# tinycrops/x-transformers-rl

Hardware: AMD Instinct MI355X
Metric: env-steps/s (rollout+update) (higher is better)
Workload: dtype f32; 1 GPU; C3: LunarLander-shaped VecSim (S=8, A=4, hazard 1/64), 1024 episodes x 128 steps per update per GPU, depth-4 d=256 4x16-head gated value-residual world-model policy, batch 128 episodes, 4 epochs, dropout 0.25; no EPO (BASELINE.json configs[2] names no gene pool: one policy, actor / critic heads on [embed | state embed], in = 2d); global_batch=1024, seq_len=128, parallelism=dp1, env_steps=1302236

## Files before the change

include/xtrl_hip.h:

```cpp
#ifndef XTRL_HIP_H
#define XTRL_HIP_H

#include <stdint.h>

#ifdef __cplusplus
extern "C" {
#endif

#define XTRL_OK 0
#define XTRL_E_ARG 1
#define XTRL_E_HIP 2

#define XTRL_ABI_VERSION 27

int xtrl_abi_version(void);
int64_t xtrl_struct_size(const char* name);
const char* xtrl_last_error(void);
const char* xtrl_source_hash(void);

#define XTRL_ACT_NONE 0
#define XTRL_ACT_GELU 1
#define XTRL_ACT_SILU 2
#define XTRL_ACT_RELU 3

int xtrl_gemm_f32(const float* X, int ldx, const float* W, int ldw, const float* bias, const float* ln_gamma,
                  const float* R, int ldr, float* Y, int ldy, const int32_t* t_dev, int64_t y_t_stride, int M,
                  int N, int K, int act, void* stream);

int xtrl_gemm_ex(int trans_a, int trans_b, const float* A, int lda, const float* B, int ldb, const float* bias,
                 float* C, int ldc, int M, int N, int K, float beta, void* stream);

int xtrl_gemm_wgrad(const float* dY, int ldy, const float* X, int ldx, float* dW, int ldw, int M, int N, int K,
                    float beta, float* ws, int64_t ws_floats, void* stream);
int xtrl_gemm_wgrad_db(const float* dY, int ldy, const float* X, int ldx, float* dW, int ldw, int M, int N, int K,
                       float beta, float* ws, int64_t ws_floats, float* db, int db_n0, void* stream);

int xtrl_layernorm_f32(const float* X, int ldx, const float* gamma, float* Y, int ldy, int M, int D, void* stream);

typedef struct XtrlDecodeLayer {
  const float* ln_attn;
  const float* w_qkv;
  const float* b_qkv;
  const float* w_out;
  const float* ln_ff;
  const float* w_ff1;
  const float* b_ff1;
  const float* w_ff2;
  const float* b_ff2;
  float* k_cache;
  float* v_cache;
  const float* w_out_t;
  const uint16_t* w_ff1x;
  const uint16_t* w_ff2x;
  const float* w_qkv_t;
  const float* w_ff1_t;
  const float* w_ff2_t;
  const float* w_ff1f;
  const float* w_ff2f;
  const float* mem_k;
  const float* mem_v;
} XtrlDecodeLayer;

typedef struct XtrlRngState {
  uint64_t seed;
  uint32_t update;
  uint32_t slot_offset;
} XtrlRngState;

typedef struct XtrlDecodeDesc {
  int E, S, A, B, d, L, H, dh, Tmax, G, ff, in_dim, n_qkv;
  int continuous, squash, evolutionary, gate_values, value_residual, learned_mix;
  int rotary_abs;
  int rot_dim;
  int sim_mode;
  int hazard_log2;
  int no_reward_cond;
  int state_only;
  float rs_eps;
  float clamp_lo, clamp_hi; int has_clamp;
  const float* w_pin; const float* b_pin;
  const float* act_emb; const float* act_emb_b;
  const float* reward_embed;
  const float* w_se; const float* b_se;
  const float* ln_final;
  const float* w_h1; const float* b_h1;
  const float* w_h2; const float* b_h2;
  const float* inv_freq;
  const XtrlDecodeLayer* layers;
  const float* rs_mean; const float* rs_var;
  float* state;
  int32_t* prev_action;
  float* prev_action_f;
  float* prev_reward;
  uint8_t* alive;
  int32_t* lens;
  double* cum_reward;
  const int32_t* episode_of_slot;
  const int32_t* slot_of_row;
  const XtrlRngState* rng;
  float* traj_states;
  int32_t* traj_actions;
  float* traj_actions_f;
  float* traj_logp;
  float* traj_rewards;
  uint8_t* traj_bounds;
  float* traj_values;
  float* x;
  float* qkv;
  float* att;
  float* hff;
  float* ac_in;
  float* logits;
  float* v1;
  float* xn;
  int32_t* live_rows;
  int32_t* live_count;
  float* mlp_part;
  uint32_t* mlp_cnt;
  const float* lat_embed;
  void** prof_events;
  const float* w_h1_t;
  const float* w_h2_t;
  const XtrlDecodeLayer* layers_dev;
  const uint16_t* w_h1x;
  float* heads_part;
  uint32_t* heads_cnt;
  float* row_part;
  uint32_t* row_cnt;
  int ff_glu;
  float* hglu;
  int qk_norm;
  float attn_scale;
  float xpos_base;
  int rms_norm;
  void* act_host;
  int attn_window;
  int Hkv;
  const float* alibi_slopes;
  int num_mem_kv;
  int add_zero_kv;
} XtrlDecodeDesc;

int xtrl_rollout_begin(const XtrlDecodeDesc* desc, void* stream);
int xtrl_decode_step(const XtrlDecodeDesc* desc, int t, void* stream);
int xtrl_decode_step_rows(const XtrlDecodeDesc* desc, int t, int max_rows, void* stream);
int xtrl_row_stamps(int on, uint64_t* out, int cap, int64_t* ticks_per_sec);
int xtrl_rollout_env_feedback(const XtrlDecodeDesc* desc, int t, const float* next_state, const float* reward,
                              const uint8_t* terminated, const uint8_t* truncated, int t_limit, int bootstrap,
                              void* stream);
int xtrl_host_decode(const XtrlDecodeDesc* desc, int t, int rows_max, void* act_host, void* stream);
int xtrl_host_feedback(const XtrlDecodeDesc* desc, int t, const void* host_stage, void* dev_stage, int t_limit,
                       int bootstrap, void* stream);
int xtrl_host_row_step(const XtrlDecodeDesc* desc, int t, const void* host_stage, int t_limit, int bootstrap,
                       uint32_t* gate, void* stream);
int xtrl_host_wait(const uint32_t* done, uint32_t value, double timeout_s);

int xtrl_dgemm(const float* A, int lda, const float* Wp, const float* bias, const float* ln_gamma, int ln_k,
               const float* R, int ldr, float* C, int ldc, const int32_t* row_map, const int32_t* m_dev, int M, int N,
               int K, int act, void* stream);
int64_t xtrl_dgemm_packed_floats(int N, int K);
int xtrl_dgemm_pack(const float* W, int ldw, int N, int K, float* Wp, void* stream);
int64_t xtrl_dgemm_packed_x6_elems(int N, int K);
int xtrl_dgemm_pack_x6(const float* W, int ldw, int N, int K, uint16_t* Wp, void* stream);
int64_t xtrl_dgemm_packed_f8_floats(int N, int K);
int xtrl_dgemm_pack_f8(const float* W, int ldw, int N, int K, float* Wp, void* stream);

typedef struct XtrlFractalLevel {
  const float* w_qkv;
  const float* w_out;
  const float* ln1_w; const float* ln1_b;
  const float* w_c;
  const float* ln2_w; const float* ln2_b;
  const float* w_ff1; const float* b_ff1;
  const float* w_ff2; const float* b_ff2;
  const float* ln3_w; const float* ln3_b;
  const float* w_pg; const float* b_pg;
  const float* level_emb;
  float* sums;
} XtrlFractalLevel;

typedef struct XtrlFractalDesc {
  int levels;
  float ln_eps;
  const XtrlFractalLevel* level;
  const float* g_init;
  const float* c0;
  const float* w_fa0; const float* b_fa0;
  const float* w_fa2; const float* b_fa2;
  float* g;
  float* c2;
  float* tmp;
  float* x2;
  float* mean;
  float* allf;
  float* hagg;
} XtrlFractalDesc;

int xtrl_fractal_decode_step(const XtrlDecodeDesc* desc, const XtrlFractalDesc* fd, int t, void* stream);

int xtrl_hlgauss_gae(const float* logits, int64_t ld_row, const float* rewards, const uint8_t* bounds,
                     int64_t ld_seq, const float* centers, float* values, float* returns, int E, int n, int B,
                     float gamma, float gamma_lam, const float* boot, const int32_t* lens, void* stream);

int xtrl_attn_fwd(const float* q, const float* k, const float* v, const int32_t* lens, float* o, float* lse,
                  int b, int H, int n, int dh, float scale, float dropout_p, uint64_t seed, uint32_t offset,
                  uint32_t sub, void* stream);
int xtrl_attn_bwd(const float* q, const float* k, const float* v, const int32_t* lens, const float* o,
                  const float* lse, const float* dout, float* dq, float* dk, float* dv, float* delta_ws, int b,
                  int H, int n, int dh, float scale, float dropout_p, uint64_t seed, uint32_t offset, uint32_t sub,
                  void* stream);
int64_t xtrl_attn_bwd_part_floats(int b, int H, int n, int dh);
int xtrl_attn_bwd_part(const float* q, const float* k, const float* v, const int32_t* lens, const float* o,
                       const float* lse, const float* dout, float* dq, float* dk, float* dv, float* delta_ws,
                       float* dq_part, int64_t dq_part_floats, int b, int H, int n, int dh, float scale,
                       float dropout_p, uint64_t seed, uint32_t offset, uint32_t sub, void* stream);
int xtrl_attn_fwd_win(const float* q, const float* k, const float* v, const int32_t* lens, float* o, float* lse,
                      int b, int H, int n, int dh, float scale, float dropout_p, uint64_t seed, uint32_t offset,
                      uint32_t sub, int window, void* stream);
int xtrl_attn_bwd_win(const float* q, const float* k, const float* v, const int32_t* lens, const float* o,
                      const float* lse, const float* dout, float* dq, float* dk, float* dv, float* delta_ws, int b,
                      int H, int n, int dh, float scale, float dropout_p, uint64_t seed, uint32_t offset,
                      uint32_t sub, int window, void* stream);
int xtrl_attn_bwd_part_win(const float* q, const float* k, const float* v, const int32_t* lens, const float* o,
                           const float* lse, const float* dout, float* dq, float* dk, float* dv, float* delta_ws,
                           float* dq_part, int64_t dq_part_floats, int b, int H, int n, int dh, float scale,
                           float dropout_p, uint64_t seed, uint32_t offset, uint32_t sub, int window, void* stream);
int xtrl_attn_fwd_gqa(const float* q, const float* k, const float* v, const int32_t* lens, float* o, float* lse,
                      int b, int H, int Hkv, int n, int dh, float scale, float dropout_p, uint64_t seed,
                      uint32_t offset, uint32_t sub, int window, void* stream);
int xtrl_attn_bwd_gqa(const float* q, const float* k, const float* v, const int32_t* lens, const float* o,
                      const float* lse, const float* dout, float* dq, float* dk, float* dv, float* delta_ws, int b,
                      int H, int Hkv, int n, int dh, float scale, float dropout_p, uint64_t seed, uint32_t offset,
                      uint32_t sub, int window, void* stream);
int xtrl_attn_bwd_part_gqa(const float* q, const float* k, const float* v, const int32_t* lens, const float* o,
                           const float* lse, const float* dout, float* dq, float* dk, float* dv, float* delta_ws,
                           float* dq_part, int64_t dq_part_floats, int b, int H, int Hkv, int n, int dh, float scale,
                           float dropout_p, uint64_t seed, uint32_t offset, uint32_t sub, int window, void* stream);
int64_t xtrl_attn_sink_ws_floats(int b, int H, int num_mem_kv, int dh);
int xtrl_attn_fwd_sink(const float* q, const float* k, const float* v, const int32_t* lens, float* o, float* lse,
                       const float* mem_k, const float* mem_v, int b, int H, int Hkv, int n, int dh, float scale,
                       float dropout_p, uint64_t seed, uint32_t offset, uint32_t sub, int window, int num_mem_kv,
                       int add_zero_kv, void* stream);
int xtrl_attn_bwd_sink(const float* q, const float* k, const float* v, const int32_t* lens, const float* o,
                       const float* lse, const float* dout, float* dq, float* dk, float* dv, float* delta_ws,
                       const float* mem_k, const float* mem_v, float* dmem_k, float* dmem_v, float* sink_ws,
                       int64_t sink_ws_floats, int b, int H, int Hkv, int n, int dh, float scale, float dropout_p,
                       uint64_t seed, uint32_t offset, uint32_t sub, int window, int num_mem_kv, int add_zero_kv,
                       void* stream);
int xtrl_attn_bwd_part_sink(const float* q, const float* k, const float* v, const int32_t* lens, const float* o,
                            const float* lse, const float* dout, float* dq, float* dk, float* dv, float* delta_ws,
                            float* dq_part, int64_t dq_part_floats, const float* mem_k, const float* mem_v,
                            float* dmem_k, float* dmem_v, float* sink_ws, int64_t sink_ws_floats, int b, int H, int Hkv,
                            int n, int dh, float scale, float dropout_p, uint64_t seed, uint32_t offset, uint32_t sub,
                            int window, int num_mem_kv, int add_zero_kv, void* stream);
int xtrl_attn_fwd_alibi(const float* q, const float* k, const float* v, const int32_t* lens, float* o, float* lse,
                        const float* mem_k, const float* mem_v, int b, int H, int Hkv, int n, int dh, float scale,
                        float dropout_p, uint64_t seed, uint32_t offset, uint32_t sub, int window, int num_mem_kv,
                        int add_zero_kv, const float* alibi_slopes, void* stream);
int xtrl_attn_bwd_alibi(const float* q, const float* k, const float* v, const int32_t* lens, const float* o,
                        const float* lse, const float* dout, float* dq, float* dk, float* dv, float* delta_ws,
                        const float* mem_k, const float* mem_v, float* dmem_k, float* dmem_v, float* sink_ws,
                        int64_t sink_ws_floats, int b, int H, int Hkv, int n, int dh, float scale, float dropout_p,
                        uint64_t seed, uint32_t offset, uint32_t sub, int window, int num_mem_kv, int add_zero_kv,
                        const float* alibi_slopes, void* stream);
int xtrl_attn_bwd_part_alibi(const float* q, const float* k, const float* v, const int32_t* lens, const float* o,
                             const float* lse, const float* dout, float* dq, float* dk, float* dv, float* delta_ws,
                             float* dq_part, int64_t dq_part_floats, const float* mem_k, const float* mem_v,
                             float* dmem_k, float* dmem_v, float* sink_ws, int64_t sink_ws_floats, int b, int H, int Hkv,
                             int n, int dh, float scale, float dropout_p, uint64_t seed, uint32_t offset, uint32_t sub,
                             int window, int num_mem_kv, int add_zero_kv, const float* alibi_slopes, void* stream);

typedef struct XtrlTrainLayer {
  int64_t ln_attn, w_proj, b_proj, w_out, ln_ff, w_ff1, b_ff1, w_ff2, b_ff2;
  int n_qkv;
  int mix;
  float* x_attn;
  float* x_ff;
  float* xn_attn;
  float* xn_ff;
  float* st_attn;
  float* st_ff;
  float* proj;
  float* qkv;
  float* o;
  float* og;
  float* lse;
  float* u;
  float* hd;
  int64_t mem_k, mem_v;
} XtrlTrainLayer;

typedef struct XtrlWimgEntry XtrlWimgEntry;

typedef struct XtrlTrainDesc {
  int b, n, S, A, d, L, H, dh, ff, B, in_dim, n_out, G;
  int continuous, evolutionary, gate_values, rot_dim;
  float dropout, frac_head_grad, reward_keep, attn_scale;
  uint64_t seed;
  uint32_t attn_offset, ff_offset;
  float* flat;
  float* grad;
  int64_t w_pin, act_emb, act_emb_b, reward_embed, w_se, b_se, ln_final;
  int64_t w_pd, b_pd;
  int64_t w_pred2, b_pred2, w_lat, b_lat, w_h1, b_h1, w_a2, b_a2, w_c2, b_c2;
  const float* inv_freq;
  const float* swr;
  const int32_t* prev_action;
  const int32_t* next_action;
  const float* prev_action_f;
  const float* next_action_f;
  const float* latent;
  const int32_t* lens;
  float* raw;
  float* values;
  float* pred;
  float* done;
  float* x_final;
  float* st_final;
  float* ac_in;
  float* ewa;
  float* zp;
  float* hp;
  float* z1;
  float* h1;
  float* lat_e;
  const float* d_raw;
  const float* d_values;
  const float* d_pred;
  const float* d_done;
  float* dx;
  float* dx2;
  float* dxn;
  float* dff;
  float* dproj;
  float* dog;
  float* dvfirst;
  float* dz1;
  float* dac;
  float* dzp;
  float* dewa;
  float* delta;
  float* part;
  int64_t part_floats;
  float* ws;
  int64_t ws_floats;
  const XtrlTrainLayer* layers;
  void** prof_events;
  double* prof_flops;
  int prof_cap;
  int* prof_n;
  void** grad_events;
  int ld_ff;
  int ff_glu;
  int ld_u2;
  float* glu_dh;
  int qk_norm;
  float xpos_base;
  int rms_norm;
  int Tv;
  int32_t* vrows;
  int32_t* vinv;
  float* ewa_v;
  float* hp_v;
  float* zp_v;
  float* pred_v;
  float* d_pred_v;
  float* dzp_v;
  float* dewa_v;
  float* dq_part;
  int64_t dq_part_floats;
  int packed;
  int32_t* ep_off;
  float* pack_ws;
  int64_t pack_ws_floats;
  int attn_window;
  int Hkv;
  void* wimg;
  int64_t wimg_bytes;
  const XtrlWimgEntry* wimg_tab;
  const XtrlWimgEntry* wimg_tab_host;
  int wimg_n;
  const float* alibi_slopes;
  int num_mem_kv;
  int add_zero_kv;
  float* sink_ws;
  int64_t sink_ws_floats;
} XtrlTrainDesc;

struct XtrlWimgEntry {
  int64_t w_off;
  int64_t img_off;
  int N, K, ld, trans_b, BN, blk0;
};
#define XTRL_WIMG_TILE_BYTES(BN) (3 * (BN) * 40 * 2)
int xtrl_train_wimg_plan(const XtrlTrainDesc* desc, XtrlWimgEntry* tab, int cap, int64_t* bytes);
int xtrl_wimg_build(const float* flat, const XtrlWimgEntry* tab_host, const XtrlWimgEntry* tab_dev, int n,
                    void* arena, int64_t arena_bytes, void* stream);

int64_t xtrl_wimg_launch_count(void);

int xtrl_train_forward(const XtrlTrainDesc* desc, void* stream);
int xtrl_train_backward(const XtrlTrainDesc* desc, void* stream);

typedef struct XtrlFractalTrainLevel {
  int64_t w_qkv;
  int64_t w_out, w_gv, w_go;
  int64_t ln1_w, ln1_b, ln2_w, ln2_b, ln3_w, ln3_b;
  int64_t w_ff1, b_ff1, w_ff2, b_ff2, w_proj, b_proj, level_embed;
  float* xin;
  float* qkv;
  float* o;
  float* lse;
  float* s1; float* x1; float* st1;
  float* g;
  float* gv;
  float* s2; float* x2; float* st2;
  float* h; float* u;
  float* s3; float* x3; float* st3;
  float* mean;
} XtrlFractalTrainLevel;

typedef struct XtrlFractalTrainDesc {
  int levels;
  int64_t b_in;
  int64_t g_init, w_gu, b_gu, w_fa0, b_fa0, w_fa2, b_fa2;
  const float* scale_embeds;
  float* le;
  float* bias0;
  float* cat;
  float* hfa;
  float* dxa; float* dxb; float* dmean;
  float* ds;
  float* dga;
  float* dgb;
  float* dgv;
  float* dz;
  float* dqkv;
  float* dob;
  float* dcat;
  float* dhfa;
  const XtrlFractalTrainLevel* level;
} XtrlFractalTrainDesc;

int xtrl_fractal_train_forward(const XtrlTrainDesc* base, const XtrlFractalTrainDesc* f, void* stream);
int xtrl_fractal_train_backward(const XtrlTrainDesc* base, const XtrlFractalTrainDesc* f, void* stream);
int xtrl_linear_gelu_drop(const float* X, int ldx, const float* W, const float* bias, float* Y, int ldy, float* deriv,
                          int ld_deriv, int M, int N, int K, float p, uint64_t seed, uint32_t offset, uint32_t layer,
                          void* stream);
int xtrl_ff_dropout_mask(uint8_t* mask, int M, int N, float p, uint64_t seed, uint32_t offset, uint32_t layer,
                         void* stream);
int xtrl_glu_drop_fwd(const float* u, int ldu, float* h, int ldh, int M, int ff, float p, uint64_t seed,
                      uint32_t offset, uint32_t layer, void* stream);
int xtrl_glu_drop_bwd(const float* dh, int lddh, const float* u, int ldu, float* du, int lddu, int M, int ff, float p,
                      uint64_t seed, uint32_t offset, uint32_t layer, void* stream);
int64_t xtrl_train_part_floats(int T, int b, int d, int A);
int64_t xtrl_train_pack_floats(int T, int S, int A, int n_out, int B);

typedef struct XtrlBatchDesc {
  int N, Tmax, n, b, S, A, B, continuous;
  const float* states;
  const int32_t* actions;
  const float* actions_f;
  const float* rewards;
  const float* logp;
  const uint8_t* bounds;
  const float* values;
  const float* returns;
  const int32_t* lens;
  const int64_t* idx;
  const float* rs_mean;
  const float* rs_var;
  float* swr;
  int32_t* prev_action;
  int32_t* action;
  float* prev_action_f;
  float* action_f;
  float* old_logp;
  float* mb_returns;
  float* old_values;
  uint8_t* dones;
  int32_t* mb_lens;
  float* rs_part;
  float* rs_m;
} XtrlBatchDesc;

int xtrl_minibatch_gather(const XtrlBatchDesc* desc, void* stream);
int xtrl_rsnorm_update(float* mean, float* var, const float* m, int D, int t, void* stream);

typedef struct XtrlLossDesc {
  int b, n, A, B, S1;
  int continuous, squash, hl_reduction_mean;
  float eps_clip, value_clip, entropy_weight, w_actor, w_critic, w_autoreg, lo, hi, sigma;
  const float* raw_actions;
  const float* values;
  const float* pred_raw;
  const float* done_logit;
  const int32_t* actions;
  const float* actions_f;
  const float* old_logp;
  const float* returns;
  const float* old_values;
  const uint8_t* dones;
  const int32_t* lens;
  const float* real;
  const float* support;
  const float* centers;
  float* tok;
  float* stats;
  float* d_raw_actions; float* d_values; float* d_pred_raw; float* d_done_logit;
} XtrlLossDesc;

#define XTRL_LOSS_TOK 30
#define XTRL_LOSS_STATS 32
#define XTRL_LS_LOSS 0
#define XTRL_LS_ACTOR 1
#define XTRL_LS_CRITIC 2
#define XTRL_LS_AUTOREG 3
#define XTRL_LS_DONE 4
#define XTRL_LS_ADV_MEAN 5
#define XTRL_LS_ADV_DEN 6
#define XTRL_LS_L 7
#define XTRL_LS_LC 8
#define XTRL_LS_NMASK 9
#define XTRL_LS_NWM 10
#define XTRL_LS_KCRIT 11
#define XTRL_LS_DL 12
#define XTRL_LS_DLC 13

int xtrl_loss_fwd(const XtrlLossDesc* desc, void* stream);
int xtrl_loss_bwd(const XtrlLossDesc* desc, float grad_scale, void* stream);

int xtrl_grad_norm(const float* g, int64_t n, double* ws, float max_norm, float* out, void* stream);
int xtrl_adopt_atan2(float* p, float* g, float* m, float* v, float* p_init, int64_t n, const int64_t* chunks,
                     int n_chunks, const int64_t* seg_start, int n_seg, int* seg_ws, const float* clip, float lr,
                     float init_lr, float beta1, float beta2, float a, float b, float weight_decay, float regen_rate,
                     float cautious, int first_step, void* stream);
int xtrl_ema_lerp(float* ema, const float* p, int64_t n, float weight, void* stream);

float xtrl_rng_uniform(uint64_t seed, uint32_t update, uint32_t slot, uint32_t t, uint32_t field, uint32_t sub);
float xtrl_rng_normal(uint64_t seed, uint32_t update, uint32_t slot, uint32_t t, uint32_t field, uint32_t sub);

int xtrl_sim_reset(float* state, int E, int S, uint64_t seed, uint32_t update, const int32_t* episode_of_slot,
                   void* stream);

int xtrl_attn_fwd_tokens(const float* q, int ldq, const float* k, int ldk, const float* v, int ldv,
                         const int32_t* lens, float* o, int ldo, float* lse, int b, int H, int n, int dh, float scale,
                         int causal, void* stream);
int xtrl_rows_add(const float* x, int ldx, const float* v, float* y, int ldy, int M, int D, void* stream);
int xtrl_add_layernorm(const float* x, int ldx, const float* r, int ldr, int r_rep, const float* gamma,
                       const float* beta, float* y, int ldy, int M, int D, float eps, void* stream);
int xtrl_seq_mean(const float* x, int ldx, int B, int n, int D, float* y, int ldy, void* stream);
int xtrl_safe_embed(const int32_t* actions, int M, const float* W, int D, float* y, int ldy, void* stream);
// ... 8 lines not shown
```

x-transformers-rl_amd/csrc/cabi.cpp:

```cpp
#include <hip/hip_runtime.h>
#include <stdarg.h>
#include <stdio.h>
#include <string.h>

#include "../../include/xtrl_hip.h"
#include "philox.h"

namespace xtrl {

static thread_local char g_err[512] = "";

void set_error(const char* fmt, ...) {
  va_list ap;
  va_start(ap, fmt);
  vsnprintf(g_err, sizeof(g_err), fmt, ap);
  va_end(ap);
}

int check_launch(const char* what) {
  const hipError_t e = hipGetLastError();
  if (e != hipSuccess) {
    set_error("%s: %s", what, hipGetErrorString(e));
    return XTRL_E_HIP;
  }
  return XTRL_OK;
}

}

extern "C" int xtrl_abi_version(void) { return XTRL_ABI_VERSION; }

#ifndef XTRL_SRC_HASH
#define XTRL_SRC_HASH "unknown"
#endif
extern "C" const char* xtrl_source_hash(void) { return XTRL_SRC_HASH; }

extern "C" int64_t xtrl_struct_size(const char* name) {
  static const struct {
    const char* name;
    int64_t size;
  } sizes[] = {{"XtrlDecodeLayer", sizeof(XtrlDecodeLayer)}, {"XtrlRngState", sizeof(XtrlRngState)},
               {"XtrlDecodeDesc", sizeof(XtrlDecodeDesc)},   {"XtrlTrainLayer", sizeof(XtrlTrainLayer)},
               {"XtrlTrainDesc", sizeof(XtrlTrainDesc)},     {"XtrlBatchDesc", sizeof(XtrlBatchDesc)},
               {"XtrlLossDesc", sizeof(XtrlLossDesc)},       {"XtrlFractalLevel", sizeof(XtrlFractalLevel)},
               {"XtrlFractalDesc", sizeof(XtrlFractalDesc)},     {"XtrlFractalTrainLevel", sizeof(XtrlFractalTrainLevel)},
               {"XtrlFractalTrainDesc", sizeof(XtrlFractalTrainDesc)}, {"XtrlWimgEntry", sizeof(XtrlWimgEntry)}};
  for (const auto& s : sizes)
    if (name && strcmp(name, s.name) == 0) return s.size;
  return -1;
}
extern "C" const char* xtrl_last_error(void) { return xtrl::g_err; }

extern "C" float xtrl_rng_uniform(uint64_t seed, uint32_t update, uint32_t slot, uint32_t t, uint32_t field,
                                  uint32_t sub) {
  return xtrl::rng_uniform(seed, update, slot, t, field, sub);
}
extern "C" float xtrl_rng_normal(uint64_t seed, uint32_t update, uint32_t slot, uint32_t t, uint32_t field,
                                 uint32_t sub) {
  return xtrl::rng_normal(seed, update, slot, t, field, sub);
}
```

x-transformers-rl_amd/csrc/gemm.hip:

```cpp
#include <cstdlib>
#include <type_traits>

#include "kernels.h"
#include "philox.h"
#include "x6.h"

namespace xtrl {

namespace {

__device__ __forceinline__ bool al16(const void* p) { return ((uintptr_t)p & 15u) == 0; }
__device__ __forceinline__ float f4c(const float4& v, int k) {
  return k == 0 ? v.x : (k == 1 ? v.y : (k == 2 ? v.z : v.w));
}

template <int EPI, bool RES>
__device__ __forceinline__ bool epi_v4_ok(const GemmArgs& a, const float* C) {
  constexpr bool AUX1 = (EPI == EPI_MUL_AUX || EPI == EPI_DGATE || EPI == EPI_MASK_POS), AUX2 = (EPI == EPI_DGATE);
  constexpr bool AOUT = (EPI == EPI_GELU_DROP || EPI == EPI_SILU_SAVE || EPI == EPI_DGATE);
  bool ok = (a.N & 3) == 0 && (a.ldc & 3) == 0 && al16(C);
  if constexpr (RES) ok = ok && (a.ldr & 3) == 0 && al16(a.R);
  if constexpr (AUX1) ok = ok && (a.ld_aux_in & 3) == 0 && al16(a.aux_in);
  if constexpr (AUX2) ok = ok && (a.ld_aux_in2 & 3) == 0 && al16(a.aux_in2);
  if constexpr (AOUT) ok = ok && (a.ld_aux_out & 3) == 0 && al16(a.aux_out);
// ... 649 lines not shown
  float4 gam = ld4(a.ln_g);
  if (!cok) gam = z4;
  const float inv_n = 1.0f / (float)N;
  if constexpr (EPI == EPI_RES_LN) {
    float4 bia = z4, beta = z4, add2 = z4;
    if (a.bias) bia = ld4(a.bias);
    if (a.ln_b) beta = ld4(a.ln_b);
    if (a.ln_b2) add2 = ld4(a.ln_b2);
    if (!cok) bia = beta = add2 = z4;
    float4 v[RPW], r[RPW];
#pragma unroll
    for (int rr = 0; rr < RPW; ++rr) {
      const int row = wave + 8 * rr, mc = min(m0 + row, M - 1);
      v[rr] = *reinterpret_cast<const float4*>(tile + row * LDT + cc);
      r[rr] = ld4(a.R + (int64_t)mc * a.ldr);
    }
#pragma unroll
    for (int rr = 0; rr < RPW; ++rr) {
      const int m = m0 + wave + 8 * rr;
      float4 x;
      x.x = (v[rr].x + bia.x) + r[rr].x; x.y = (v[rr].y + bia.y) + r[rr].y;
      x.z = (v[rr].z + bia.z) + r[rr].z; x.w = (v[rr].w + bia.w) + r[rr].w;
      if (!cok) x = z4;
      const float mean = a.ln_rms ? 0.f : wave_sum((x.x + x.y) + (x.z + x.w)) * inv_n;
      float4 dl = make_float4(x.x - mean, x.y - mean, x.z - mean, x.w - mean);
      if (!cok) dl = z4;
      const float sq = wave_sum((dl.x * dl.x + dl.y * dl.y) + (dl.z * dl.z + dl.w * dl.w));
      const float rstd = a.ln_rms ? norm_rstd(sq, (float)N, true) : 1.0f / sqrtf(sq * inv_n + 1e-5f);
      float4 y = make_float4((dl.x * rstd) * gam.x, (dl.y * rstd) * gam.y, (dl.z * rstd) * gam.z,
                             (dl.w * rstd) * gam.w);
      if (a.ln_b) y = make_float4(y.x + beta.x, y.y + beta.y, y.z + beta.z, y.w + beta.w);
      if (m < M) {
        if (cok) {
          *reinterpret_cast<float4*>(a.C + (int64_t)m * a.ldc + c) = x;
          *reinterpret_cast<float4*>(a.ln_y1 + (int64_t)m * a.ln_ld1 + c) = y;
          if (a.ln_y2)
            *reinterpret_cast<float4*>(a.ln_y2 + (int64_t)m * a.ln_ld2 + c) =
                make_float4(y.x + add2.x, y.y + add2.y, y.z + add2.z, y.w + add2.w);
        }
        if (lane == 0) *reinterpret_cast<float2*>(a.ln_stats + 2 * (int64_t)m) = make_float2(mean, rstd);
      }
    }
  } else {
    constexpr bool X = EPI == EPI_LN_BWD2;
    const int ps = X && a.ln_pstride ? a.ln_pstride : N;
    float4 g[RPW], xv[RPW], dr[RPW];
    float2 st[RPW];
#pragma unroll
    for (int rr = 0; rr < RPW; ++rr) {
      const int row = wave + 8 * rr, mc = min(m0 + row, M - 1);
      g[rr] = *reinterpret_cast<const float4*>(tile + row * LDT + cc);
      xv[rr] = ld4(a.ln_x + (int64_t)mc * N);
      if constexpr (X) dr[rr] = a.ln_gpre ? ld4(a.ln_gpre + (int64_t)mc * (a.ln_ldg ? a.ln_ldg : N)) : z4;
      else dr[rr] = a.ln_dres ? ld4(a.ln_dres + (int64_t)mc * N) : z4;
      st[rr] = *reinterpret_cast<const float2*>(a.ln_stats + 2 * (int64_t)mc);
      if constexpr (X) {
        const float gs = a.ln_gscale;
        g[rr] = make_float4(g[rr].x * gs + dr[rr].x, g[rr].y * gs + dr[rr].y, g[rr].z * gs + dr[rr].z,
                            g[rr].w * gs + dr[rr].w);
      }
      if (!cok) g[rr] = z4;
    }
    float4 dg = z4, db = z4;
#pragma unroll
    for (int rr = 0; rr < RPW; ++rr) {
      const int m = m0 + wave + 8 * rr;
      const float mu = st[rr].x, rs = st[rr].y;
      float4 xh = make_float4((xv[rr].x - mu) * rs, (xv[rr].y - mu) * rs, (xv[rr].z - mu) * rs, (xv[rr].w - mu) * rs);
      if (!cok) xh = z4;
      const float4 gm = make_float4(g[rr].x * gam.x, g[rr].y * gam.y, g[rr].z * gam.z, g[rr].w * gam.w);
      if (m < M) {
        dg.x += g[rr].x * xh.x; dg.y += g[rr].y * xh.y; dg.z += g[rr].z * xh.z; dg.w += g[rr].w * xh.w;
        if constexpr (X) { db.x += g[rr].x; db.y += g[rr].y; db.z += g[rr].z; db.w += g[rr].w; }
      }
      const float ma = a.ln_rms ? 0.f : wave_sum((gm.x + gm.y) + (gm.z + gm.w)) * inv_n;
      const float mb = wave_sum((gm.x * xh.x + gm.y * xh.y) + (gm.z * xh.z + gm.w * xh.w)) * inv_n;
      float4 o;
      o.x = rs * (gm.x - ma - xh.x * mb);
      o.y = rs * (gm.y - ma - xh.y * mb);
      o.z = rs * (gm.z - ma - xh.z * mb);
      o.w = rs * (gm.w - ma - xh.w * mb);
      if constexpr (!X) {
        o.x += dr[rr].x; o.y += dr[rr].y; o.z += dr[rr].z; o.w += dr[rr].w;
      }
      if (!cok) o = z4;
      if (m < M && cok) *reinterpret_cast<float4*>(a.C + (int64_t)m * a.ldc + c) = o;
      if constexpr (X) g[rr] = o;
    }
    float* red = tile + BM * LDT;
    const int t = threadIdx.x;
    auto tile_sum = [&](float4 v, float* dst) {
      __syncthreads();
      if (cok) *reinterpret_cast<float4*>(red + wave * BN + c) = v;
      __syncthreads();
      if (t < N) {
        float sum = 0.f;
#pragma unroll
        for (int w = 0; w < 8; ++w) sum += red[w * BN + t];
        dst[(int64_t)row_tile * ps + t] = sum;
      }
    };
    tile_sum(dg, a.ln_part);
    if constexpr (X) {
      if (a.ln_part_b) tile_sum(db, a.ln_part_b);
      if (a.ln2_out) {
        float4 gam2 = ld4(a.ln2_g);
        if (!cok) gam2 = z4;
#pragma unroll
        for (int rr = 0; rr < RPW; ++rr) {
          const int row = wave + 8 * rr, mc = min(m0 + row, M - 1);
          xv[rr] = ld4(a.ln2_x + (int64_t)mc * N);
          st[rr] = *reinterpret_cast<const float2*>(a.ln2_stats + 2 * (int64_t)mc);
        }
        dg = db = z4;
#pragma unroll
        for (int rr = 0; rr < RPW; ++rr) {
          const int m = m0 + wave + 8 * rr;
          const float mu = st[rr].x, rs = st[rr].y;
          float4 xh = make_float4((xv[rr].x - mu) * rs, (xv[rr].y - mu) * rs, (xv[rr].z - mu) * rs, (xv[rr].w - mu) * rs);
          if (!cok) xh = z4;
          const float4 gm = make_float4(g[rr].x * gam2.x, g[rr].y * gam2.y, g[rr].z * gam2.z, g[rr].w * gam2.w);
          if (m < M) {
            dg.x += g[rr].x * xh.x; dg.y += g[rr].y * xh.y; dg.z += g[rr].z * xh.z; dg.w += g[rr].w * xh.w;
            db.x += g[rr].x; db.y += g[rr].y; db.z += g[rr].z; db.w += g[rr].w;
          }
          const float ma = wave_sum((gm.x + gm.y) + (gm.z + gm.w)) * inv_n;
          const float mb = wave_sum((gm.x * xh.x + gm.y * xh.y) + (gm.z * xh.z + gm.w * xh.w)) * inv_n;
          const float4 o = make_float4(rs * (gm.x - ma - xh.x * mb), rs * (gm.y - ma - xh.y * mb),
                                       rs * (gm.z - ma - xh.z * mb), rs * (gm.w - ma - xh.w * mb));
          if (m < M && cok) *reinterpret_cast<float4*>(a.ln2_out + (int64_t)m * N + c) = o;
        }
        tile_sum(dg, a.ln2_part);
        tile_sum(db, a.ln2_part_b);
      }
    }
  }
}

#ifdef XTRL_WS_DIAG
__device__ uint64_t* g_ws_diag;
__device__ int g_ws_mode;
#define WS_STAMP(step, k)                                                                         \
  do {                                                                                            \
    if ((tid & 255) == 0)                                                                         \
      g_ws_diag[((int64_t)(blockIdx.x + gridDim.x * (blockIdx.y + gridDim.y * blockIdx.z)) * 2 +   \
                 (tid >> 8)) * 4096 + (step) * 4 + (k)] = __builtin_amdgcn_s_memtime();           \
  } while (0)
#else
#define WS_STAMP(step, k) do {} while (0)
#endif

typedef __attribute__((address_space(3))) void lds_void_t;

template <bool TA, bool TB, int EPI, bool RES, int BM = 128, int BN = 128, bool KT = false, bool WI = false>
__global__ __launch_bounds__(512, 1) void k_gemm_ws(const GemmArgs a) {
  constexpr int BK = 32, XRS = BK + 8, NP = 256, TM = 2, TN = 2, WN = BN / 64;
  constexpr bool LNE = (EPI == EPI_RES_LN || EPI == EPI_LN_BWD || EPI == EPI_LN_BWD2);
  static_assert(!WI || !TA, "weight images feed B of the A \"N\" launches");
  static_assert(XTRL_WIMG_TILE_BYTES(BN) == 3 * BN * XRS * 2, "image tile = the B part of a piece image");
  constexpr int A_F4 = BM * BK / 4 / NP, B_F4 = BN * BK / 4 / NP;
  constexpr int IMG = 3 * (BM + BN) * XRS;
  static_assert((BM == 128 && BN == 128) || (BM == 64 && BN == 256), "tile 128 x 128 or 64 x 256");
  static_assert(!TA || A_F4 == 4, "A \"T\": one 4 x 4 transposed group per producer thread");
  static_assert(!TB || B_F4 % 4 == 0, "B \"T\": whole 4 x 4 transposed groups per producer thread");
  constexpr int LDT = BN + 4;
  static_assert(!LNE || (BM * LDT + 8 * BN) * 4 <= 2 * IMG * 2, "LN tile exceeds the piece images");
  __shared__ __attribute__((aligned(16))) __bf16 smem[2 * IMG];

  const int tid = threadIdx.x, lane = tid & 63, wave = tid >> 6;
  const bool producer = wave >= 4;
  int bx = blockIdx.x, by = blockIdx.y, bz = blockIdx.z;
  if (a.xcd_remap) {
    const int nx = gridDim.x, ny = gridDim.y;
    const int total = nx * ny * gridDim.z;
    const int lin = bx + nx * (by + ny * bz);
    const int lg = (lin & 7) * (total >> 3) + (lin >> 3);
    bx = lg % nx;
    by = (lg / nx) % ny;
    bz = lg / (nx * ny);
  }
  const int m0 = by * BM, n0 = bx * BN;
  const int M = a.M, N = a.N;
  int K = a.K;
  const float* __restrict__ Ab = a.A;
  const float* __restrict__ Bb = a.B;
  if (a.kspan > 0) {
    const int kb = bz * a.kspan;
    K = min(a.kspan, a.K - kb);
    Ab += TA ? (int64_t)kb * a.lda : kb;
    Bb += TB ? (int64_t)kb * a.ldb : kb;
  }
  const int nk = (K + BK - 1) / BK;
  using I0 = std::integral_constant<int, 0>;
  using I1 = std::integral_constant<int, 1>;

  const int p = tid - 256;
  float4 ra[2][A_F4], rb[2][B_F4];
  const bool do_rs = a.rowsum != nullptr && bx == 0;
  float rs[4] = {0.f, 0.f, 0.f, 0.f};
  auto ld_n = [&](const float* base, int64_t ld, int row, int row_lim, int k) -> float4 {
    return *reinterpret_cast<const float4*>(base + (int64_t)min(row, row_lim - 1) * ld + (KT ? min(k, K - 4) : k));
  };
  auto ld_t = [&](const float* base, int64_t ld, int k, int col, int col_lim) -> float4 {
    return *reinterpret_cast<const float4*>(base + (int64_t)(KT ? min(k, K - 1) : k) * ld +
                                            min(col, ((col_lim + 3) & ~3) - 4));
  };
  auto kmask = [&](float4 f, int k) -> float4 {
    if constexpr (KT) {
      const bool ok = k < K;
      f = make_float4(ok ? f.x : 0.f, ok ? f.y : 0.f, ok ? f.z : 0.f, ok ? f.w : 0.f);
    }
    return f;
  };
  auto load = [&](auto S, int kt) {
    const int k0 = min(kt, nk - 1) * BK;
#pragma unroll
    for (int i = 0; i < A_F4; ++i) {
      if constexpr (!TA) {
        const int e = p + i * NP, r = e / (BK / 4), q = e % (BK / 4);
        ra[S][i] = ld_n(Ab, a.lda, m0 + r, M, k0 + 4 * q);
      } else {
        const int kq = p % (BK / 4), q = p / (BK / 4);
        ra[S][i] = ld_t(Ab, a.lda, k0 + 4 * kq + i, m0 + 4 * q, M);
      }
    }
    if constexpr (!WI) {
#pragma unroll
      for (int i = 0; i < B_F4; ++i) {
        if constexpr (!TB) {
          const int e = p + i * NP, r = e / (BK / 4), q = e % (BK / 4);
          rb[S][i] = ld_n(Bb, a.ldb, n0 + r, N, k0 + 4 * q);
        } else {
          const int kq = p % (BK / 4), q = p / (BK / 4) + 32 * (i >> 2);
          rb[S][i] = ld_t(Bb, a.ldb, k0 + 4 * kq + (i & 3), n0 + 4 * q, N);
        }
      }
    }
  };
  constexpr int WB = XTRL_WIMG_TILE_BYTES(BN), WCH = WB / 1024, WPW = (WCH + 3) / 4;
  static_assert(WB % 1024 == 0 && (3 * BM * XRS * 2) % 16 == 0, "whole wave-instructions, 16-byte aligned B part");
  auto dma_b = [&](int kt, __bf16* img) {
    const char* src = static_cast<const char*>(a.wimg) + ((int64_t)bx * nk + min(kt, nk - 1)) * WB + lane * 16;
    char* dst = reinterpret_cast<char*>(img + 3 * BM * XRS);
#pragma unroll
    for (int i = 0; i < WPW; ++i) {
      const int c = 4 * i + (wave - 4);
      if (WCH % 4 == 0 || c < WCH)
        __builtin_amdgcn_global_load_lds((const void*)(src + c * 1024), (lds_void_t*)(dst + c * 1024), 16, 0, 0);
    }
  };
  auto put = [&](__bf16* img, int rows, int row, int k, float4 v) {
    bf16x4 h, m, l;
#if defined(XTRL_WS_MODE) && XTRL_WS_MODE == 4
    h = __builtin_bit_cast(bf16x4, make_uint2(__float_as_uint(v.x), __float_as_uint(v.y)));
    m = __builtin_bit_cast(bf16x4, make_uint2(__float_as_uint(v.z), __float_as_uint(v.w)));
    l = __builtin_bit_cast(bf16x4, make_uint2(__float_as_uint(v.x), __float_as_uint(v.w)));
#else
    split3(v, h, m, l);
#endif
    __bf16* q = img + row * XRS + k;
    *reinterpret_cast<bf16x4*>(q) = h;
    *reinterpret_cast<bf16x4*>(q + rows * XRS) = m;
    *reinterpret_cast<bf16x4*>(q + 2 * rows * XRS) = l;
  };
  auto convert = [&](auto S, __bf16* img, int kt, bool live) {
    __bf16* xa = img;
    __bf16* xb = img + 3 * BM * XRS;
    const int k0 = min(kt, nk - 1) * BK;
    const int kq = p % (BK / 4), q = p / (BK / 4);
    if constexpr (!TA) {
#pragma unroll
      for (int i = 0; i < A_F4; ++i) {
        const int e = p + i * NP, r = e / (BK / 4), qq = e % (BK / 4);
        put(xa, BM, r, 4 * qq, kmask(ra[S][i], k0 + 4 * qq));
      }
    } else {
      const float4 k0v = kmask(ra[S][0], k0 + 4 * kq), k1v = kmask(ra[S][1], k0 + 4 * kq + 1),
                   k2v = kmask(ra[S][2], k0 + 4 * kq + 2), k3v = kmask(ra[S][3], k0 + 4 * kq + 3);
      put(xa, BM, 4 * q + 0, 4 * kq, make_float4(k0v.x, k1v.x, k2v.x, k3v.x));
      put(xa, BM, 4 * q + 1, 4 * kq, make_float4(k0v.y, k1v.y, k2v.y, k3v.y));
      put(xa, BM, 4 * q + 2, 4 * kq, make_float4(k0v.z, k1v.z, k2v.z, k3v.z));
      put(xa, BM, 4 * q + 3, 4 * kq, make_float4(k0v.w, k1v.w, k2v.w, k3v.w));
      if (do_rs) {
        float s4[4] = {(k0v.x + k1v.x) + (k2v.x + k3v.x), (k0v.y + k1v.y) + (k2v.y + k3v.y),
                       (k0v.z + k1v.z) + (k2v.z + k3v.z), (k0v.w + k1v.w) + (k2v.w + k3v.w)};
#pragma unroll
        for (int c = 0; c < 4; ++c) {
#pragma unroll
          for (int o = 1; o < BK / 4; o <<= 1) s4[c] += __shfl_xor(s4[c], o, kWave);
          rs[c] += live ? s4[c] : 0.f;
        }
      }
    }
    if constexpr (WI) {
    } else if constexpr (!TB) {
#pragma unroll
      for (int i = 0; i < B_F4; ++i) {
        const int e = p + i * NP, r = e / (BK / 4), qq = e % (BK / 4);
        put(xb, BN, r, 4 * qq, kmask(rb[S][i], k0 + 4 * qq));
      }
    } else {
#pragma unroll
      for (int gi = 0; gi < B_F4 / 4; ++gi) {
        const int qg = q + 32 * gi;
        const float4 k0v = kmask(rb[S][4 * gi], k0 + 4 * kq), k1v = kmask(rb[S][4 * gi + 1], k0 + 4 * kq + 1),
                     k2v = kmask(rb[S][4 * gi + 2], k0 + 4 * kq + 2), k3v = kmask(rb[S][4 * gi + 3], k0 + 4 * kq + 3);
        put(xb, BN, 4 * qg + 0, 4 * kq, make_float4(k0v.x, k1v.x, k2v.x, k3v.x));
        put(xb, BN, 4 * qg + 1, 4 * kq, make_float4(k0v.y, k1v.y, k2v.y, k3v.y));
        put(xb, BN, 4 * qg + 2, 4 * kq, make_float4(k0v.z, k1v.z, k2v.z, k3v.z));
        put(xb, BN, 4 * qg + 3, 4 * kq, make_float4(k0v.w, k1v.w, k2v.w, k3v.w));
      }
    }
  };

  const int wm = (wave & 3) / WN, wn = (wave & 3) % WN;
  f32x16 acc[TM][TN];
#pragma unroll
  for (int i = 0; i < TM; ++i)
#pragma unroll
    for (int j = 0; j < TN; ++j)
#pragma unroll
      for (int r = 0; r < 16; ++r) acc[i][j][r] = 0.f;
  auto compute = [&](const __bf16* img) {
    const int xi = wm * 32 * TM + (lane & 31), xj = wn * 32 * TN + (lane & 31), xk = 8 * (lane >> 5);
    const __bf16* xa = img;
    const __bf16* xb = img + 3 * BM * XRS;
    bf16x8 av[2][3][TM], bv[2][3][TN];
    auto rd = [&](int buf, int st) {
      auto ra_ = [&](int pc) {
#pragma unroll
        for (int i = 0; i < TM; ++i)
          av[buf][pc][i] = *reinterpret_cast<const bf16x8*>(xa + (pc * BM + xi + 32 * i) * XRS + 16 * st + xk);
      };
      auto rb_ = [&](int pc) {
#pragma unroll
        for (int j = 0; j < TN; ++j)
          bv[buf][pc][j] = *reinterpret_cast<const bf16x8*>(xb + (pc * BN + xj + 32 * j) * XRS + 16 * st + xk);
      };
      ra_(2); rb_(0); ra_(0); rb_(2); ra_(1); rb_(1);
    };
    rd(0, 0);
#pragma unroll
    for (int st = 0; st < BK / 16; ++st) {
      const int pb = st & 1;
      if (st + 1 < BK / 16) rd(pb ^ 1, st + 1);
      __builtin_amdgcn_sched_barrier(0);
      constexpr int PA[6] = {2, 0, 1, 1, 0, 0}, PB[6] = {0, 2, 1, 0, 1, 0};
#pragma unroll
      for (int t = 0; t < 6; ++t)
#pragma unroll
        for (int i = 0; i < TM; ++i)
#pragma unroll
          for (int j = 0; j < TN; ++j)
            acc[i][j] = __builtin_amdgcn_mfma_f32_32x32x16_bf16(av[pb][PA[t]][i], bv[pb][PB[t]][j], acc[i][j], 0, 0, 0);
      __builtin_amdgcn_sched_barrier(0);
    }
  };

  const int nsteps = 2 * ((nk + 1) / 2);
  auto wi_barrier = [&]() {
    static_assert(A_F4 <= 15, "vmcnt immediate");
    __builtin_amdgcn_sched_barrier(0);
    __builtin_amdgcn_s_waitcnt(A_F4 | 0x70);
    if constexpr (A_F4 == 2) asm volatile("s_waitcnt vmcnt(2) lgkmcnt(0)" ::: "memory");
    else asm volatile("s_waitcnt vmcnt(4) lgkmcnt(0)" ::: "memory");
    static_assert(A_F4 == 2 || A_F4 == 4, "vmcnt immediates above");
    __builtin_amdgcn_s_barrier();
    asm volatile("" ::: "memory");
    __builtin_amdgcn_sched_barrier(0);
  };
  if (producer) {
    load(I0{}, 0);
    load(I1{}, 1);
    convert(I0{}, smem, 0, true);
    if constexpr (WI) {
      __builtin_amdgcn_sched_barrier(0);
      dma_b(0, smem);
      __builtin_amdgcn_sched_barrier(0);
    }
    load(I0{}, 2);
    if constexpr (WI) wi_barrier();
    else __syncthreads();
#ifdef XTRL_WS_DIAG
    const int mode = g_ws_mode;
#elif defined(XTRL_WS_MODE)
    constexpr int mode = XTRL_WS_MODE;
#else
    constexpr int mode = 0;
#endif
    auto pstep = [&](auto C, int t) {
      if constexpr (WI) {
        __bf16* img = smem + ((t + 1) & 1) * IMG;
        convert(C, img, t + 1, t + 1 < nk);
        __builtin_amdgcn_sched_barrier(0);
        dma_b(t + 1, img);
        __builtin_amdgcn_sched_barrier(0);
        load(C, t + 3);
        wi_barrier();
        return;
      }
      WS_STAMP(t, 0);
      if (mode < 2 || mode == 4) convert(C, smem + ((t + 1) & 1) * IMG, t + 1, t + 1 < nk);
      else if (mode == 3) {
        float s = 0.f;
#pragma unroll
        for (int i = 0; i < 4; ++i) s += ra[decltype(C)::value][i % A_F4].x + rb[decltype(C)::value][i].y;
        if (s == 12345.f) smem[tid] = (__bf16)s;
      }
      WS_STAMP(t, 1);
      __builtin_amdgcn_sched_barrier(0);
      if (mode != 2) load(C, t + 3);
      WS_STAMP(t, 2);
      __builtin_amdgcn_sched_barrier(0);
      __syncthreads();
      __builtin_amdgcn_sched_barrier(0);
    };
    for (int t = 0; t < nsteps; t += 2) {
      pstep(I1{}, t);
      pstep(I0{}, t + 1);
    }
    if (TA && do_rs && (p % (BK / 4)) == 0) {
      const int q = p / (BK / 4);
#pragma unroll
      for (int c = 0; c < 4; ++c) {
        const int m = m0 + 4 * q + c;
        if (m < M && m >= a.rowsum_m0) {
          if (a.kspan > 0) a.rowsum_ws[(int64_t)bz * M + m] = rs[c];
          else a.rowsum[m - a.rowsum_m0] += rs[c];
        }
      }
    }
    if constexpr (!LNE) return;
  } else {
    __syncthreads();
    for (int t = 0; t < nsteps; ++t) {
      WS_STAMP(t, 0);
#ifdef XTRL_WS_DIAG
      if (t < nk && g_ws_mode != 1) compute(smem + (t & 1) * IMG);
#elif defined(XTRL_WS_MODE)
      if (t < nk && XTRL_WS_MODE != 1) compute(smem + (t & 1) * IMG);
#else
      if (t < nk) compute(smem + (t & 1) * IMG);
#endif
      WS_STAMP(t, 1);
      __syncthreads();
    }
    WS_STAMP(nsteps, 0);
    if constexpr (!LNE) {
      gemm_epilogue<TM, TN, EPI, RES, EPI == EPI_GELU_DROP>(a, acc, m0, n0, wm, wn, lane, bz);
      return;
    }
  }
  if constexpr (LNE) ln_epilogue<BM, BN, EPI>(a, acc, reinterpret_cast<float*>(smem), producer, m0, wm, wn, lane, wave,
                                              by);
}

__global__ __launch_bounds__(256) void k_layernorm(const float* X, int ldx, const float* gamma, float* Y, int ldy,
                                                   int M, int D) {
  const int lane = threadIdx.x & 63;
  const int m = blockIdx.x * 4 + (threadIdx.x >> 6);
  if (m >= M) return;
  const float* xr = X + (int64_t)m * ldx;
  float s = 0.f;
  for (int k = lane; k < D; k += 64) s += xr[k];
  const float mean = wave_sum(s) / (float)D;
  float q = 0.f;
  for (int k = lane; k < D; k += 64) {
    const float dlt = xr[k] - mean;
    q += dlt * dlt;
  }
  const float rstd = 1.0f / sqrtf(wave_sum(q) / (float)D + 1e-5f);
  for (int k = lane; k < D; k += 64) Y[(int64_t)m * ldy + k] = ((xr[k] - mean) * rstd) * gamma[k];
}

__device__ __forceinline__ float sum_splits(const float* p, int S, int64_t stride) {
  float acc = 0.f;
  int z = 0;
  for (; z + 16 <= S; z += 16) {
    float v[16];
#pragma unroll
    for (int u = 0; u < 16; ++u) v[u] = p[(int64_t)(z + u) * stride];
#pragma unroll
    for (int u = 0; u < 16; ++u) acc += v[u];
  }
  for (; z < S; ++z) acc += p[(int64_t)z * stride];
  return acc;
}

__global__ __launch_bounds__(256) void k_splitk_reduce(const float* ws, int S, int M, int N, float* C, int ldc,
                                                       float beta, const float* rws, float* rowsum, int m0) {
  const int64_t MN = (int64_t)M * N;
  const int64_t gtid = (int64_t)blockIdx.x * 256 + threadIdx.x, gsz = (int64_t)gridDim.x * 256;
  if (rowsum) {
    for (int64_t m = m0 + gtid; m < M; m += gsz) rowsum[m - m0] += sum_splits(rws + m, S, M);
  }
  if ((N & 3) == 0) {
    constexpr int G = 4, U = 8;
    const int64_t Q = MN >> 2;
    const int g = threadIdx.x & (G - 1);
    const float4* w4 = reinterpret_cast<const float4*>(ws);
    for (int64_t q = gtid / G; q < Q; q += gsz / G) {
      float4 a = make_float4(0.f, 0.f, 0.f, 0.f);
      for (int z0 = g; z0 < S; z0 += G * U) {
        float4 p[U];
#pragma unroll
        for (int u = 0; u < U; ++u) {
          const int z = z0 + G * u;
          p[u] = z < S ? w4[(int64_t)z * Q + q] : make_float4(0.f, 0.f, 0.f, 0.f);
        }
#pragma unroll
        for (int u = 0; u < U; ++u) {
          a.x += p[u].x; a.y += p[u].y; a.z += p[u].z; a.w += p[u].w;
        }
      }
      float4 b;
      b.x = __shfl_xor(a.x, 1); b.y = __shfl_xor(a.y, 1); b.z = __shfl_xor(a.z, 1); b.w = __shfl_xor(a.w, 1);
      if (g & 1) { const float4 t = a; a = b; b = t; }
      a.x += b.x; a.y += b.y; a.z += b.z; a.w += b.w;
      b.x = __shfl_xor(a.x, 2); b.y = __shfl_xor(a.y, 2); b.z = __shfl_xor(a.z, 2); b.w = __shfl_xor(a.w, 2);
      if (g & 2) { const float4 t = a; a = b; b = t; }
      a.x += b.x; a.y += b.y; a.z += b.z; a.w += b.w;
      if (g == 0) {
        const int64_t i = q << 2;
        const int m = (int)(i / N), n = (int)(i - (int64_t)m * N);
        float* dst = C + (int64_t)m * ldc + n;
        if (beta != 0.f) {
          a.x += beta * dst[0]; a.y += beta * dst[1]; a.z += beta * dst[2]; a.w += beta * dst[3];
        }
        dst[0] = a.x; dst[1] = a.y; dst[2] = a.z; dst[3] = a.w;
      }
    }
    return;
  }
  for (int64_t i = gtid; i < MN; i += gsz) {
    const float acc = sum_splits(ws + i, S, MN);
    const int m = (int)(i / N), n = (int)(i - (int64_t)m * N);
    float* dst = C + (int64_t)m * ldc + n;
    *dst = (beta != 0.f) ? beta * (*dst) + acc : acc;
  }
}

struct SplitKJobs {
  SplitKJob job[kMaxSplitKJobs];
  int n;
  int64_t total_q, total_r;
};
__global__ __launch_bounds__(256) void k_splitk_reduce_multi(const SplitKJobs J) {
  const int64_t gsz = (int64_t)gridDim.x * 256;
  for (int64_t u = (int64_t)blockIdx.x * 256 + threadIdx.x; u < J.total_q + J.total_r; u += gsz) {
    if (u < J.total_q) {
      int j = 0;
      while (j + 1 < J.n && J.job[j + 1].q0 <= u) ++j;
      const SplitKJob& b = J.job[j];
      const int64_t q = u - b.q0, MN4 = (int64_t)b.M * b.N / 4;
      const float4* w4 = reinterpret_cast<const float4*>(b.ws);
      float4 a = make_float4(0.f, 0.f, 0.f, 0.f);
      int z = 0;
      for (; z + 8 <= b.S; z += 8) {
        float4 p[8];
#pragma unroll
        for (int k = 0; k < 8; ++k) p[k] = w4[(int64_t)(z + k) * MN4 + q];
#pragma unroll
        for (int k = 0; k < 8; ++k) {
          a.x += p[k].x; a.y += p[k].y; a.z += p[k].z; a.w += p[k].w;
        }
      }
      for (; z < b.S; ++z) {
        const float4 p = w4[(int64_t)z * MN4 + q];
        a.x += p.x; a.y += p.y; a.z += p.z; a.w += p.w;
      }
      const int64_t i = q << 2;
      const int m = (int)(i / b.N), n = (int)(i - (int64_t)m * b.N);
      float4* dst = reinterpret_cast<float4*>(b.C + (int64_t)m * b.ldc + n);
      if (b.beta != 0.f) {
        const float4 o = *dst;
        a.x += b.beta * o.x; a.y += b.beta * o.y; a.z += b.beta * o.z; a.w += b.beta * o.w;
      }
      *dst = a;
    } else {
      const int64_t r = u - J.total_q;
      int j = 0;
      while (j + 1 < J.n && J.job[j + 1].r0 <= r) ++j;
      const SplitKJob& b = J.job[j];
      const int m = b.m0 + (int)(r - b.r0);
      b.rowsum[m - b.m0] += sum_splits(b.rws + m, b.S, b.M);
    }
  }
}

template <int WM, int WN, int WK, int TM, int TN, bool TA, bool TB, int EPI, bool LN, bool RES, bool VEC,
          bool X6 = false>
void launch(const GemmArgs& a, hipStream_t s) {
  constexpr int BM = 32 * WM * TM, BN = 32 * WN * TN;
  const int splits = a.kspan > 0 ? (a.K + a.kspan - 1) / a.kspan : 1;
  dim3 grid((a.N + BN - 1) / BN, (a.M + BM - 1) / BM, splits);
  if constexpr (X6) {
    if ((int64_t)grid.x * grid.y * grid.z % 8 == 0) {
      GemmArgs r = a;
      r.xcd_remap = 1;
      hipLaunchKernelGGL((k_gemm<WM, WN, WK, TM, TN, TA, TB, EPI, LN, RES, VEC, X6>), grid, dim3(64 * WM * WN * WK), 0,
                         s, r);
      return;
    }
  }
  hipLaunchKernelGGL((k_gemm<WM, WN, WK, TM, TN, TA, TB, EPI, LN, RES, VEC, X6>), grid, dim3(64 * WM * WN * WK), 0, s,
                     a);
}

bool ws_ok(const GemmArgs& a, bool ta, bool ln) {
  if (!(!ln && (a.K % 32 == 0 || ta) && (a.kspan == 0 || a.kspan % 32 == 0) && (!a.rowsum || ta)))
    return false;
  const int splits = a.kspan > 0 ? (a.K + a.kspan - 1) / a.kspan : 1;
  const int64_t wgs = (int64_t)((a.N + 127) / 128) * ((a.M + 127) / 128) * splits;
  return wgs <= 256 && (a.kspan > 0 ? a.kspan : a.K) >= (ta ? 64 : 512);
}

int64_t g_wimg_launches = 0;

bool wimg_on() {
  static const bool on = [] {
    const char* e = getenv("XTRL_WIMG");
    return !(e && atoi(e) == 0);
  }();
  return on;
}

template <bool TA, bool TB, int EPI, bool RES, int BM = 128, int BN = 128, bool KT = false>
void launch_ws(const GemmArgs& a, hipStream_t s) {
  const int splits = a.kspan > 0 ? (a.K + a.kspan - 1) / a.kspan : 1;
  dim3 grid((a.N + BN - 1) / BN, (a.M + BM - 1) / BM, splits);
  GemmArgs r = a;
  r.xcd_remap = (int64_t)grid.x * grid.y * grid.z % 8 == 0 ? 1 : 0;
  if constexpr (!TA && (EPI == EPI_NONE || EPI == EPI_RES_LN || EPI == EPI_LN_BWD || EPI == EPI_LN_BWD2)) {
    if (a.wimg && a.wimg_bn == BN && a.kspan == 0 && wimg_on()) {
      ++g_wimg_launches;
      hipLaunchKernelGGL((k_gemm_ws<TA, TB, EPI, RES, BM, BN, KT, true>), grid, dim3(512), 0, s, r);
      return;
    }
  }
  hipLaunchKernelGGL((k_gemm_ws<TA, TB, EPI, RES, BM, BN, KT>), grid, dim3(512), 0, s, r);
}

int ln_gemm_run(const GemmArgs& a, int trans_a, int trans_b, int epi, bool vec, hipStream_t s) {
  const bool res = a.R != nullptr;
  XTRL_REQUIRE(!trans_a && vec && a.kspan == 0 && a.N <= 256 && a.N % 4 == 0 && a.K % 4 == 0 && a.ln_g &&
                   a.ln_stats && a.ldc % 4 == 0 && ((uintptr_t)a.C & 15u) == 0 && ((uintptr_t)a.ln_g & 15u) == 0,
               "gemm: LayerNorm epilogue needs one row tile (N=%d <= 256), float4 operands, K %% 4 == 0", a.N);
  const bool kt = a.K % 32 != 0, narrow = a.N <= 128;
  if (epi == EPI_RES_LN) {
    XTRL_REQUIRE(!trans_b && res && a.ln_y1 && a.ldr % 4 == 0 && a.ln_ld1 % 4 == 0 && (!a.ln_y2 || a.ln_ld2 % 4 == 0) &&
                     (!a.bias || ((uintptr_t)a.bias & 15u) == 0) && (!a.ln_b || ((uintptr_t)a.ln_b & 15u) == 0) &&
                     (!a.ln_b2 || (a.ln_y2 && ((uintptr_t)a.ln_b2 & 15u) == 0)),
                 "gemm: residual + LayerNorm epilogue arguments");
    if (narrow) {
      if (kt) launch_ws<false, false, EPI_RES_LN, true, 128, 128, true>(a, s);
      else launch_ws<false, false, EPI_RES_LN, true, 128, 128, false>(a, s);
    } else {
      if (kt) launch_ws<false, false, EPI_RES_LN, true, 64, 256, true>(a, s);
      else launch_ws<false, false, EPI_RES_LN, true, 64, 256, false>(a, s);
    }
  } else if (epi == EPI_LN_BWD) {
    XTRL_REQUIRE(trans_b && !res && a.ln_x && a.ln_part, "gemm: LayerNorm-backward epilogue arguments");
    if (narrow) launch_ws<false, true, EPI_LN_BWD, false, 128, 128, true>(a, s);
    else launch_ws<false, true, EPI_LN_BWD, false, 64, 256, true>(a, s);
  } else {
    XTRL_REQUIRE(trans_b && !res && a.ln_x && a.ln_part && (!a.ln_gpre || ((uintptr_t)a.ln_gpre & 15u) == 0) &&
                     a.ln_ldg % 4 == 0 &&
                     (!a.ln2_out || (a.ln2_g && a.ln2_x && a.ln2_stats && a.ln2_part && a.ln2_part_b &&
                                     ((uintptr_t)a.ln2_out & 15u) == 0 && ((uintptr_t)a.ln2_g & 15u) == 0)) &&
                     a.ldc == a.N,
                 "gemm: post-norm LayerNorm-backward epilogue arguments");
    if (narrow) launch_ws<false, true, EPI_LN_BWD2, false, 128, 128, true>(a, s);
    else launch_ws<false, true, EPI_LN_BWD2, false, 64, 256, true>(a, s);
  }
  XTRL_LAUNCHED("gemm_ln");
  return XTRL_OK;
}

bool use_x6() {
  static const bool x6 = [] {
    const char* e = getenv("XTRL_GEMM_F32");
    return !(e && atoi(e) != 0);
  }();
  return x6;
}

template <bool TA, bool TB, int EPI, bool LN, bool RES>
void dispatch_geom(const GemmArgs& a, bool vec, hipStream_t s) {
  const int64_t tiles128 = (int64_t)((a.M + 127) / 128) * ((a.N + 127) / 128);
  const int64_t tiles64 = (int64_t)((a.M + 63) / 64) * ((a.N + 63) / 64);
  if (!vec) launch<2, 2, 1, 1, 1, TA, TB, EPI, LN, RES, false>(a, s);
  else if (!TA && a.N <= 32 && a.M >= 4096) launch<2, 1, 2, 1, 1, TA, TB, EPI, LN, RES, true>(a, s);
  else if (tiles128 >= 192 && a.K > 64) {
    bool done = false;
    if constexpr (EPI != EPI_DGATE && !LN) {
      if (use_x6() && ws_ok(a, TA, LN) && a.K % 32 == 0) {
        launch_ws<TA, TB, EPI, RES>(a, s);
        done = true;
      }
    }
    if (done) {
    } else if (use_x6()) launch<2, 2, 1, 2, 2, TA, TB, EPI, LN, RES, true, true>(a, s);
    else launch<2, 2, 1, 2, 2, TA, TB, EPI, LN, RES, true>(a, s);
  }
  else if (tiles64 >= 256 && a.K <= 512) {
    bool done = false;
    if constexpr (!TA && !TB && EPI != EPI_DGATE) {
      if (use_x6()) {
        launch<2, 2, 1, 1, 1, TA, TB, EPI, LN, RES, true, true>(a, s);
        done = true;
      }
    }
    if (!done) launch<2, 2, 1, 1, 1, TA, TB, EPI, LN, RES, true>(a, s);
  }
  else if (a.K <= 256) launch<2, 1, 2, 1, 1, TA, TB, EPI, LN, RES, true>(a, s);
  else launch<1, 1, 4, 1, 1, TA, TB, EPI, LN, RES, true>(a, s);
}

bool aligned16(const void* p) { return ((uintptr_t)p & 15u) == 0; }

bool gelu_drop_v4_host(const GemmArgs& a) {
  return (a.N & 3) == 0 && (a.ldc & 3) == 0 && aligned16(a.C) && (a.ld_aux_out & 3) == 0 && aligned16(a.aux_out) &&
         !a.t_dev && a.kspan == 0;
}
int round4(int x) { return (x + 3) & ~3; }

}

int gemm_ln_rows(int N) { return N <= 128 ? 128 : 64; }

int gemm_run(const GemmArgs& a, int trans_a, int trans_b, int epi, hipStream_t s) {
  XTRL_REQUIRE(a.A && a.B && a.C, "gemm: null operand");
  XTRL_REQUIRE(a.M >= 0 && a.N >= 0 && a.K > 0, "gemm: bad shape M=%d N=%d K=%d", a.M, a.N, a.K);
  XTRL_REQUIRE(a.lda >= (trans_a ? a.M : a.K) && a.ldb >= (trans_b ? a.N : a.K) && a.ldc >= a.N,
               "gemm: leading dims too small");
  XTRL_REQUIRE(!(a.gamma && trans_a), "gemm: LayerNorm prologue needs a row-major A");
  XTRL_REQUIRE(!((epi == EPI_GELU_DROP || epi == EPI_SILU_SAVE || epi == EPI_DGATE) && !a.aux_out),
               "gemm: epilogue %d needs aux_out", epi);
  XTRL_REQUIRE(!((epi == EPI_MUL_AUX || epi == EPI_DGATE || epi == EPI_MASK_POS) && !a.aux_in),
               "gemm: epilogue %d needs aux_in", epi);
  XTRL_REQUIRE(!(epi == EPI_DGATE && !a.aux_in2), "gemm: gate epilogue needs aux_in2");
  if (a.M == 0 || a.N == 0) return XTRL_OK;
  const bool vec = aligned16(a.A) && aligned16(a.B) && (a.lda % 4 == 0) && (a.ldb % 4 == 0) &&
                   a.lda >= round4(trans_a ? a.M : a.K) && a.ldb >= round4(trans_b ? a.N : a.K);
  const bool ln = a.gamma != nullptr, res = a.R != nullptr;
  if (epi == EPI_RES_LN || epi == EPI_LN_BWD || epi == EPI_LN_BWD2) return ln_gemm_run(a, trans_a, trans_b, epi, vec, s);
  const bool vec_k = vec && (epi != EPI_GELU_DROP || gelu_drop_v4_host(a));
#define XG(TA_, TB_, E_, L_, R_)                                                                   \
  if (trans_a == TA_ && trans_b == TB_ && epi == E_ && ln == L_ && res == R_) {                    \
    dispatch_geom<TA_, TB_, E_, L_, R_>(a, vec_k, s);                                              \
    XTRL_LAUNCHED("gemm_f32");                                                                     \
    return XTRL_OK;                                                                                \
  }
  XG(0, 0, EPI_NONE, false, false)
  XG(0, 0, EPI_NONE, false, true)
  XG(0, 0, EPI_NONE, true, false)
  XG(0, 0, EPI_GELU, true, false)
  XG(0, 0, EPI_GELU, false, false)
  XG(0, 0, EPI_SILU, false, false)
  XG(0, 0, EPI_RELU, false, false)
  XG(0, 0, EPI_GELU_DROP, false, false)
  XG(0, 0, EPI_SILU_SAVE, false, false)
  XG(0, 1, EPI_NONE, false, false)
  XG(0, 1, EPI_NONE, false, true)
  XG(0, 1, EPI_MASK_POS, false, false)
  XG(0, 1, EPI_MUL_AUX, false, false)
  XG(0, 1, EPI_DGATE, false, false)
  XG(1, 1, EPI_NONE, false, false)
#undef XG
  set_error("gemm: unsupported combination ta=%d tb=%d epi=%d ln=%d residual=%d", trans_a, trans_b, epi, (int)ln,
            (int)res);
  return XTRL_E_ARG;
}

int gemm_ex(int trans_a, int trans_b, const float* A, int lda, const float* B, int ldb, const float* bias,
            const float* ln_gamma, const float* R, int ldr, float* C, int ldc, const int32_t* t_dev,
            int64_t c_t_stride, int M, int N, int K, int act, float beta, hipStream_t s) {
  XTRL_REQUIRE(act >= 0 && act <= 3, "gemm: bad activation %d", act);
  if (act == 3) act = EPI_RELU;
  GemmArgs a;
  a.A = A; a.B = B; a.bias = bias; a.gamma = ln_gamma; a.R = R; a.C = C; a.t_dev = t_dev;
  a.c_t_stride = c_t_stride; a.lda = lda; a.ldb = ldb; a.ldr = ldr; a.ldc = ldc; a.M = M; a.N = N; a.K = K;
  a.beta = beta;
  return gemm_run(a, trans_a, trans_b, act, s);
}

constexpr int SKW_R = 64;
template <bool TALL, int S, int LJ>
__global__ __launch_bounds__(256) void k_wgrad_skinny(const float* __restrict__ dY, int ldy, const float* __restrict__ X,
                                                      int ldx, int M, int N, int K, int bias, int span,
                                                      float* __restrict__ P, float* __restrict__ PR) {
  constexpr int R = SKW_R / LJ;
  extern __shared__ float skw_lds[];
  const int tid = threadIdx.x, Kx = K + bias;
  const int YS = (N + 3) & ~3, XS = (Kx + 3) & ~3;
  float* Ys = skw_lds;
  float* Xs = skw_lds + R * YS + (TALL ? 0 : 256 * LJ);
  const int t_lo = blockIdx.x * span, t_hi = min(M, t_lo + span);
  auto stage = [&](int t0) {
    const float* Lg = TALL ? dY : X;
    const int ldl = TALL ? ldy : ldx, Ln = TALL ? N : Kx, LSd = TALL ? YS : XS;
    float* Ld = TALL ? Ys : Xs;
#pragma unroll
    for (int j = 0; j < LJ; ++j) {
      const int c = tid + 256 * j;
      const bool in = c < Ln, ld = in && (TALL || c < K);
      float v[R];
#pragma unroll
      for (int r = 0; r < R; ++r) v[r] = (t0 + r < t_hi && ld) ? Lg[(int64_t)(t0 + r) * ldl + c] : 0.f;
      if (!TALL && c == K)
#pragma unroll
        for (int r = 0; r < R; ++r) v[r] = t0 + r < t_hi ? 1.f : 0.f;
      if (in)
#pragma unroll
        for (int r = 0; r < R; ++r) Ld[r * LSd + c] = v[r];
    }
    const float* Sg = TALL ? X : dY;
    const int lds_ = TALL ? ldx : ldy, Sn = TALL ? Kx : N, SSd = TALL ? XS : YS;
    float* Sd = TALL ? Xs : Ys;
    for (int e = tid; e < R * Sn; e += 256) {
      const int r = e / Sn, c = e - r * Sn, t = t0 + r;
      float v = 0.f;
      if (t < t_hi) v = (!TALL || c < K) ? Sg[(int64_t)t * lds_ + c] : 1.f;
      Sd[r * SSd + c] = v;
    }
  };
// ... 194 lines not shown
    }
  if (deferred && (defer->n == kMaxSplitKJobs || defer->used + need(splits) > ws_floats)) {
    if (int rc = splitk_flush(*defer, s)) return rc;
  }
  if (defer && !deferred && splits > 1 && defer->n > 0)
    if (int rc = splitk_flush(*defer, s)) return rc;
  if (deferred) {
    ws += defer->used;
    ws_floats -= defer->used;
  }
  while (splits > 1 && need(splits) > ws_floats) {
    splits = std::max(1, splits / 2);
    kspan = ((M + splits - 1) / splits + 31) / 32 * 32;
    splits = (M + kspan - 1) / kspan;
  }
  const bool vec = aligned16(dY) && aligned16(X) && (ldy % 4 == 0) && (ldx % 4 == 0) && ldy >= round4(N) &&
                   ldx >= round4(K);
  GemmArgs a;
  a.A = dY; a.B = X; a.C = dW; a.lda = ldy; a.ldb = ldx; a.ldc = ldw; a.M = N; a.N = K; a.K = M; a.beta = beta;
  a.rowsum = db;
  a.rowsum_m0 = db_n0;
  if (splits > 1) {
    XTRL_REQUIRE(ws && need(splits) <= ws_floats, "gemm_wgrad: workspace too small");
    a.C = ws;
    a.ldc = K;
    a.beta = 0.f;
    a.kspan = kspan;
    a.c_split = (int64_t)N * K;
    a.rowsum_ws = ws + (int64_t)splits * N * K;
  }
  if (!vec) launch<2, 2, 1, 1, 1, true, true, EPI_NONE, false, false, false>(a, s);
  else if (big) {
    const bool timed = prof && prof->events && *prof->n < prof->cap;
    if (timed) (void)hipEventRecord((hipEvent_t)prof->events[2 * *prof->n], s);
    if (use_x6() && ws_ok(a, true, false)) {
      if (a.K % 32 == 0) launch_ws<true, true, EPI_NONE, false>(a, s);
      else launch_ws<true, true, EPI_NONE, false, 128, 128, true>(a, s);
    }
    else if (use_x6()) launch<2, 2, 1, 2, 2, true, true, EPI_NONE, false, false, true, true>(a, s);
    else launch<2, 2, 1, 2, 2, true, true, EPI_NONE, false, false, true>(a, s);
    if (timed) {
      (void)hipEventRecord((hipEvent_t)prof->events[2 * *prof->n + 1], s);
      prof->flops[*prof->n] = 2.0 * (double)M * (double)N * (double)K;
      ++*prof->n;
    }
  } else launch<2, 2, 1, 1, 1, true, true, EPI_NONE, false, false, true>(a, s);
  if (splits > 1 && deferred) {
    SplitKJob& j = defer->job[defer->n++];
    j.ws = ws; j.C = dW; j.rws = a.rowsum_ws; j.rowsum = db; j.S = splits; j.M = N; j.N = K; j.ldc = ldw;
    j.m0 = db_n0; j.beta = beta; j.q0 = j.r0 = 0;
    defer->used += need(splits);
  } else if (splits > 1) {
    const int64_t MN = (int64_t)N * K;
    const int64_t units = MN;
    hipLaunchKernelGGL(k_splitk_reduce, dim3((unsigned)std::max<int64_t>(1, std::min<int64_t>((units + 255) / 256, 4096))),
                       dim3(256), 0, s, ws, splits, N, K, dW, ldw, beta, a.rowsum_ws, db, db_n0);
  }
  XTRL_LAUNCHED("gemm_wgrad");
  return XTRL_OK;
}

int gemm_f32(const float* X, int ldx, const float* W, int ldw, const float* bias, const float* ln_gamma,
             const float* R, int ldr, float* Y, int ldy, const int32_t* t_dev, int64_t y_t_stride, int M, int N,
             int K, int act, hipStream_t s) {
  return gemm_ex(0, 0, X, ldx, W, ldw, bias, ln_gamma, R, ldr, Y, ldy, t_dev, y_t_stride, M, N, K, act, 0.f, s);
}

int layernorm_f32(const float* X, int ldx, const float* gamma, float* Y, int ldy, int M, int D, hipStream_t s) {
  XTRL_REQUIRE(X && gamma && Y && M >= 0 && D > 0, "layernorm: bad arguments");
  if (M == 0) return XTRL_OK;
  hipLaunchKernelGGL(k_layernorm, dim3((M + 3) / 4), dim3(256), 0, s, X, ldx, gamma, Y, ldy, M, D);
  XTRL_LAUNCHED("layernorm_f32");
  return XTRL_OK;
}

namespace {
__global__ __launch_bounds__(256) void k_wimg_build(const float* __restrict__ flat, const XtrlWimgEntry* __restrict__ tab,
                                                    int n, char* __restrict__ arena) {
  constexpr int BK = 32, XRS = BK + 8;
  int e = 0;
  while (e + 1 < n && tab[e + 1].blk0 <= (int)blockIdx.x) ++e;
  const XtrlWimgEntry E = tab[e];
  const int BN = E.BN, nkt = (E.K + BK - 1) / BK, blk = (int)blockIdx.x - E.blk0, j = blk / nkt, s = blk % nkt;
  __bf16* out = reinterpret_cast<__bf16*>(arena + E.img_off + (int64_t)blk * XTRL_WIMG_TILE_BYTES(BN));
  const float* W = flat + E.w_off;
  for (int u = threadIdx.x; u < BN * (BK / 4); u += 256) {
    const int r = E.trans_b ? u % BN : u / (BK / 4), q = E.trans_b ? u / BN : u % (BK / 4);
    const int row = j * BN + r, k0 = s * BK + 4 * q;
    float v[4];
#pragma unroll
    for (int c = 0; c < 4; ++c) {
      const bool ok = row < E.N && k0 + c < E.K;
      const int64_t at = E.trans_b ? (int64_t)(k0 + c) * E.ld + row : (int64_t)row * E.ld + k0 + c;
      const float x = W[ok ? at : 0];
      v[c] = ok ? x : 0.f;
    }
    bf16x4 h, m, l;
    split3(make_float4(v[0], v[1], v[2], v[3]), h, m, l);
    __bf16* o = out + r * XRS + 4 * q;
    *reinterpret_cast<bf16x4*>(o) = h;
    *reinterpret_cast<bf16x4*>(o + BN * XRS) = m;
    *reinterpret_cast<bf16x4*>(o + 2 * BN * XRS) = l;
    if (q == 0) {
#pragma unroll
      for (int pc = 0; pc < 3; ++pc)
        *reinterpret_cast<uint4*>(out + (pc * BN + r) * XRS + BK) = make_uint4(0u, 0u, 0u, 0u);
    }
  }
}
}

bool wimg_enabled() { return wimg_on(); }

int wimg_tile_bn(int N, int epi) {
  const bool lne = epi == EPI_RES_LN || epi == EPI_LN_BWD || epi == EPI_LN_BWD2;
  return lne && N > 128 ? 256 : 128;
}

void wimg_find(GemmArgs& g, int trans_b, int epi, const float* flat, const XtrlWimgEntry* tab, int n,
               const void* arena) {
  if (!tab || !arena || n <= 0 || !wimg_on()) return;
  const int bn = wimg_tile_bn(g.N, epi);
  for (int i = 0; i < n; ++i) {
    const XtrlWimgEntry& E = tab[i];
    if (flat + E.w_off == g.B && E.trans_b == trans_b && E.N == g.N && E.K == g.K && E.ld == g.ldb && E.BN == bn) {
      g.wimg = static_cast<const char*>(arena) + E.img_off;
      g.wimg_bn = bn;
      return;
    }
  }
}

int wimg_build(const float* flat, const XtrlWimgEntry* tab_host, const XtrlWimgEntry* tab_dev, int n, void* arena,
               int64_t arena_bytes, hipStream_t s) {
  XTRL_REQUIRE(flat && tab_host && tab_dev && arena && n > 0, "wimg: null table / arena");
  XTRL_REQUIRE(((uintptr_t)arena & 15u) == 0, "wimg: the arena must be 16-byte aligned");
  int blocks = 0;
  for (int i = 0; i < n; ++i) {
    const XtrlWimgEntry& E = tab_host[i];
    XTRL_REQUIRE((E.BN == 128 || E.BN == 256) && E.N > 0 && E.K > 0 && E.w_off >= 0 && E.img_off >= 0 &&
                     E.img_off % 16 == 0 && E.blk0 == blocks && (E.trans_b == 0 || E.trans_b == 1) &&
                     E.ld >= (E.trans_b ? E.N : E.K),
                 "wimg: bad table entry %d", i);
    const int64_t tiles = (int64_t)((E.N + E.BN - 1) / E.BN) * ((E.K + 31) / 32);
    XTRL_REQUIRE(E.img_off + tiles * XTRL_WIMG_TILE_BYTES(E.BN) <= arena_bytes,
                 "wimg: entry %d ends past the arena (%lld bytes)", i, (long long)arena_bytes);
    blocks += (int)tiles;
  }
  hipLaunchKernelGGL(k_wimg_build, dim3(blocks), dim3(256), 0, s, flat, tab_dev, n, static_cast<char*>(arena));
  XTRL_LAUNCHED("wimg_build");
  return XTRL_OK;
}

}

extern "C" int64_t xtrl_wimg_launch_count(void) { return xtrl::g_wimg_launches; }

extern "C" int xtrl_wimg_build(const float* flat, const XtrlWimgEntry* tab_host, const XtrlWimgEntry* tab_dev, int n,
                               void* arena, int64_t arena_bytes, void* stream) {
  return xtrl::wimg_build(flat, tab_host, tab_dev, n, arena, arena_bytes, xtrl::as_stream(stream));
}

extern "C" int xtrl_gemm_f32(const float* X, int ldx, const float* W, int ldw, const float* bias,
                             const float* ln_gamma, const float* R, int ldr, float* Y, int ldy,
                             const int32_t* t_dev, int64_t y_t_stride, int M, int N, int K, int act, void* stream) {
  return xtrl::gemm_f32(X, ldx, W, ldw, bias, ln_gamma, R, ldr, Y, ldy, t_dev, y_t_stride, M, N, K, act,
                        xtrl::as_stream(stream));
}

extern "C" int xtrl_gemm_ex(int trans_a, int trans_b, const float* A, int lda, const float* B, int ldb,
                            const float* bias, float* C, int ldc, int M, int N, int K, float beta, void* stream) {
  return xtrl::gemm_ex(trans_a, trans_b, A, lda, B, ldb, bias, nullptr, nullptr, 0, C, ldc, nullptr, 0, M, N, K,
                       XTRL_ACT_NONE, beta, xtrl::as_stream(stream));
}

extern "C" int xtrl_gemm_wgrad(const float* dY, int ldy, const float* X, int ldx, float* dW, int ldw, int M, int N,
                               int K, float beta, float* ws, int64_t ws_floats, void* stream) {
  return xtrl::gemm_wgrad(dY, ldy, X, ldx, dW, ldw, M, N, K, beta, ws, ws_floats, xtrl::as_stream(stream), nullptr, 0);
}

extern "C" int xtrl_gemm_wgrad_db(const float* dY, int ldy, const float* X, int ldx, float* dW, int ldw, int M,
                                  int N, int K, float beta, float* ws, int64_t ws_floats, float* db, int db_n0,
                                  void* stream) {
  return xtrl::gemm_wgrad(dY, ldy, X, ldx, dW, ldw, M, N, K, beta, ws, ws_floats, xtrl::as_stream(stream), db, db_n0);
}

extern "C" int xtrl_layernorm_f32(const float* X, int ldx, const float* gamma, float* Y, int ldy, int M, int D,
                                  void* stream) {
  return xtrl::layernorm_f32(X, ldx, gamma, Y, ldy, M, D, xtrl::as_stream(stream));
}
```

x-transformers-rl_amd/csrc/kernels.h:

```cpp
#pragma once
#include "common.h"

namespace xtrl {

enum GemmEpi : int {
  EPI_NONE = 0,
  EPI_GELU = 1,
  EPI_SILU = 2,
  EPI_GELU_DROP = 3,
  EPI_SILU_SAVE = 4,
  EPI_MUL_AUX = 5,
  EPI_RELU = 8,
  EPI_DGATE = 7,
  EPI_RES_LN = 9,
  EPI_LN_BWD = 10,
  EPI_MASK_POS = 11,
  EPI_LN_BWD2 = 12,
};

struct GemmArgs {
  const float* A = nullptr;
  const float* B = nullptr;
  const float* bias = nullptr;
  const float* gamma = nullptr;
  const float* R = nullptr;
  float* C = nullptr;
  const int32_t* t_dev = nullptr;
  int64_t c_t_stride = 0;
  int lda = 0, ldb = 0, ldr = 0, ldc = 0, M = 0, N = 0, K = 0;
  float beta = 0.f;
  int kspan = 0;
  int64_t c_split = 0;
  int bias_col0 = 0;
  int act_cols = 1 << 30;
  const float* aux_in = nullptr;  int ld_aux_in = 0;
  const float* aux_in2 = nullptr; int ld_aux_in2 = 0;
  float* aux_out = nullptr;       int ld_aux_out = 0;
  uint64_t seed = 0;
  uint32_t drop_off = 0;
  uint32_t drop_layer = 0;
  uint32_t drop_thresh = 0;
  uint32_t drop_thresh8 = 0;
  float inv_keep = 1.f;
  const uint8_t* row_mask = nullptr;
  float* rowsum = nullptr;
  int rowsum_m0 = 0;
  float* rowsum_ws = nullptr;
  int xcd_remap = 0;
  const float* ln_g = nullptr;
  int ln_rms = 0;
  const float* ln_b = nullptr;
  const float* ln_b2 = nullptr;
  float* ln_y1 = nullptr; int ln_ld1 = 0;
  float* ln_y2 = nullptr; int ln_ld2 = 0;
  float* ln_stats = nullptr;
  const float* ln_x = nullptr;
  const float* ln_dres = nullptr;
  float* ln_part = nullptr;
  const float* ln_gpre = nullptr;
  int ln_ldg = 0;
  float ln_gscale = 1.f;
  float* ln_part_b = nullptr;
  int ln_pstride = 0;
  const float* ln2_g = nullptr;
  const float* ln2_x = nullptr;
  const float* ln2_stats = nullptr;
  float* ln2_out = nullptr;
  float* ln2_part = nullptr;
  float* ln2_part_b = nullptr;
  const void* wimg = nullptr;
  int wimg_bn = 0;
};
void wimg_find(GemmArgs& g, int trans_b, int epi, const float* flat, const XtrlWimgEntry* tab, int n,
               const void* arena);
int wimg_tile_bn(int N, int epi);
bool wimg_enabled();
int wimg_build(const float* flat, const XtrlWimgEntry* tab_host, const XtrlWimgEntry* tab_dev, int n, void* arena,
               int64_t arena_bytes, hipStream_t s);
int gemm_ln_rows(int N);

int gemm_run(const GemmArgs& a, int trans_a, int trans_b, int epi, hipStream_t s);
struct GemmProfile {
  void** events;
  double* flops;
  int cap;
  int* n;
};
struct SplitKJob {
  const float* ws;
  float* C;
  const float* rws;
  float* rowsum;
  int S, M, N, ldc, m0;
  float beta;
  int64_t q0, r0;
};
constexpr int kMaxSplitKJobs = 24;
struct SplitKQueue {
  SplitKJob job[kMaxSplitKJobs];
  int n = 0;
  int64_t used = 0;
};
int splitk_flush(SplitKQueue& q, hipStream_t s);

int gemm_wgrad(const float* dY, int ldy, const float* X, int ldx, float* dW, int ldw, int M, int N, int K, float beta,
               float* ws, int64_t ws_floats, hipStream_t s, float* db = nullptr, int db_n0 = 0,
               const GemmProfile* prof = nullptr, SplitKQueue* defer = nullptr);
int gemm_f32(const float* X, int ldx, const float* W, int ldw, const float* bias, const float* ln_gamma,
             const float* R, int ldr, float* Y, int ldy, const int32_t* t_dev, int64_t y_t_stride, int M, int N,
             int K, int act, hipStream_t s);
int layernorm_f32(const float* X, int ldx, const float* gamma, float* Y, int ldy, int M, int D, hipStream_t s);

struct DGemmArgs {
  const float* A = nullptr; int lda = 0;
  const float* W = nullptr; int ldw = 0;
  const float* bias = nullptr;
  const float* gamma = nullptr; int ln_k = 0;
  int ln_rms = 0;
  const float* R = nullptr; int ldr = 0;
  float* C = nullptr; int ldc = 0;
  const int32_t* row_map = nullptr;
  const int32_t* m_dev = nullptr;
  int M = 0, N = 0, K = 0;
  int n_split = 1 << 30;
  float* C2 = nullptr; int ldc2 = 0;
  const int32_t* row_map2 = nullptr;
};
int dgemm_run(const DGemmArgs& a, int rows, int epi, hipStream_t s);
int dg_ks(int N, int K);
int64_t dgemm_packed_floats(int N, int K);
int dgemm_pack(const float* W, int ldw, int N, int K, float* Wp, hipStream_t s);

void rows_add_launch(const float* x, int ldx, const float* v, float* y, int ldy, int M, int D, hipStream_t s);
void add_layernorm_launch(const float* x, int ldx, const float* r, int ldr, const float* g, const float* b, float* y,
                          int ldy, int M, int D, float eps, hipStream_t s);

inline uint32_t dropout_thresh8(float p) {
  const double t = (double)p * 256.0;
  return (t >= 1.0 && t <= 255.0 && t == (double)(int)t) ? (uint32_t)t : 0u;
}

inline uint32_t dropout_thresh(float p) {
  if (!(p > 0.f)) return 0u;
  const double th = (double)p * 4294967296.0;
  const uint32_t t = (uint32_t)fmin(th, 4294967295.0);
  return t ? t : 1u;
}

struct AttnLayout {
  int64_t sb, sh;
  int si;
};
inline AttnLayout attn_layout_bhnd(int H, int n, int dh) {
  return AttnLayout{(int64_t)H * n * dh, (int64_t)n * dh, dh};
}
inline AttnLayout attn_layout_tokens(int n, int ld, int dh) {
  return AttnLayout{(int64_t)n * ld, (int64_t)dh, ld};
}

struct AttnProblem {
  int b, H, n, dh;
  const int32_t* lens;
  float scale, dropout;
  uint64_t seed;
  uint32_t offset;
  AttnLayout in, out, grad;
  AttnLayout gate;
  int causal = 1;
  uint32_t sub = 0;
  float* dq_part = nullptr;
  int64_t dq_part_floats = 0;
  const int32_t* ep_off = nullptr;
  int window = 0;
  int Hkv = 0;
  AttnLayout kv = {}, kvgrad = {};
  const float *mem_k = nullptr, *mem_v = nullptr;
  int mem_kv = 0, zero_kv = 0;
  float *dmem_k = nullptr, *dmem_v = nullptr;
  int dmem_accum = 0;
  float* sink_ws = nullptr;
  int64_t sink_ws_floats = 0;
  const float* alibi = nullptr;
};
constexpr int kMaxMemKV = 16;
inline bool attn_has_sinks(const AttnProblem& p) { return p.mem_kv > 0 || p.zero_kv != 0; }
int64_t attn_sink_ws_floats(int b, int H, int mem_kv, int dh);
__host__ __device__ inline int kv_head_of(int h, int Hkv) { return h % Hkv; }
__host__ __device__ inline bool kv_head_owner(int h, int Hkv) {
  for (int x = 0; x < h; ++x)
    if (kv_head_of(x, Hkv) == kv_head_of(h, Hkv)) return false;
  return true;
}
int64_t attn_dq_part_floats(int b, int H, int n, int dh);

int attn_fwd_ex(const AttnProblem& p, const float* q, const float* k, const float* v, float* o, float* lse,
                const float* gate, float* og, hipStream_t s);
int attn_bwd_ex(const AttnProblem& p, const float* q, const float* k, const float* v, const float* o,
                const float* lse, const float* dout, float* dq, float* dk, float* dv, float* delta_ws,
                hipStream_t s);

}
```

x-transformers-rl_amd/csrc/train.hip:

```cpp
#include <cstdlib>
#include <vector>

#include <hip/hip_ext.h>

#include "kernels.h"
#include "philox.h"

namespace xtrl {
namespace {

constexpr int kMaxDPerLane = 8;

__device__ __forceinline__ float ldg(const float* p) { return __builtin_nontemporal_load(p); }

struct EmbedArgs {
  const float *swr, *w_pin, *act_emb, *act_emb_b, *reward_embed, *w_se, *b_se, *lat_e, *prev_af, *next_af;
  const int32_t *prev_a, *next_a;
  float *x0, *ac_in, *ewa;
  int T, n, S, A, d, in_dim, continuous, evolutionary;
  float keep;
  const float* ln_g;
  float *xn, *st;
  int rms;
  const int32_t* rows;
// ... 640 lines not shown
  const int r = blockIdx.x * blockDim.x + threadIdx.x;
  if (r < rows) dst[(int64_t)r * lddst] = src[(int64_t)r * ld];
}

__device__ __forceinline__ bool ff_keep(int m, int n, uint32_t thresh, uint32_t thresh8, uint64_t seed, uint32_t off,
                                        uint32_t layer) {
  if (thresh8) {
    const u32x4_t r = philox4x32_10((uint32_t)n, (uint32_t)(((m >> 5) << 1) | ((m >> 2) & 1)), off,
                                    rng_c3(FIELD_FF_DROPOUT, 2 * layer + 1), seed);
    const int g = (m >> 3) & 3;
    const uint32_t w = g == 0 ? r.x : (g == 1 ? r.y : (g == 2 ? r.z : r.w));
    return ((w >> (8 * (m & 3))) & 0xFFu) >= thresh8;
  }
  if (thresh == 0) return true;
  const u32x4_t r = philox4x32_10((uint32_t)n, (uint32_t)(m >> 2), off, rng_c3(FIELD_FF_DROPOUT, 2 * layer), seed);
  const int q = m & 3;
  const uint32_t w = q == 0 ? r.x : (q == 1 ? r.y : (q == 2 ? r.z : r.w));
  return w >= thresh;
}

__global__ void k_ff_mask(uint8_t* mask, int M, int N, uint32_t thresh, uint32_t thresh8, uint64_t seed,
                          uint32_t off, uint32_t layer) {
  const int64_t i = (int64_t)blockIdx.x * blockDim.x + threadIdx.x;
  if (i >= (int64_t)M * N) return;
  const int m = (int)(i / N), n = (int)(i - (int64_t)m * N);
  mask[i] = (uint8_t)ff_keep(m, n, thresh, thresh8, seed, off, layer);
}

__device__ __forceinline__ float gelu_deriv_erf(float x) {
  const float cdf = 0.5f * (1.0f + erff(x * 0.70710678118654752f));
  return cdf + x * (0.39894228040143268f * expf(-0.5f * x * x));
}
__global__ void k_glu_fwd(const float* u, int ldu, float* h, int ldh, int M, int ff, uint32_t thresh, uint32_t thresh8,
                          float inv_keep, uint64_t seed, uint32_t off, uint32_t layer) {
  const int64_t i = (int64_t)blockIdx.x * blockDim.x + threadIdx.x;
  if (i >= (int64_t)M * ff) return;
  const int m = (int)(i / ff), j = (int)(i - (int64_t)m * ff);
  const float a = u[(int64_t)m * ldu + j], g = u[(int64_t)m * ldu + ff + j];
  const bool keep = ff_keep(m, j, thresh, thresh8, seed, off, layer);
  h[(int64_t)m * ldh + j] = keep ? (a * geluf_(g)) * inv_keep : 0.f;
}
__global__ void k_glu_bwd(const float* dh, int lddh, const float* u, int ldu, float* du, int lddu, int M, int ff,
                          uint32_t thresh, uint32_t thresh8, float inv_keep, uint64_t seed, uint32_t off,
                          uint32_t layer) {
  const int64_t i = (int64_t)blockIdx.x * blockDim.x + threadIdx.x;
  if (i >= (int64_t)M * ff) return;
  const int m = (int)(i / ff), j = (int)(i - (int64_t)m * ff);
  const float a = u[(int64_t)m * ldu + j], g = u[(int64_t)m * ldu + ff + j];
  const bool keep = ff_keep(m, j, thresh, thresh8, seed, off, layer);
  const float dk = keep ? dh[(int64_t)m * lddh + j] * inv_keep : 0.f;
  du[(int64_t)m * lddu + j] = dk * geluf_(g);
  du[(int64_t)m * lddu + ff + j] = (dk * a) * gelu_deriv_erf(g);
}

int glu_fwd(const float* u, int ldu, float* h, int ldh, int M, int ff, float p, uint64_t seed, uint32_t off,
            uint32_t layer, hipStream_t s) {
  if ((int64_t)M * ff == 0) return XTRL_OK;
  hipLaunchKernelGGL(k_glu_fwd, dim3((unsigned)(((int64_t)M * ff + 255) / 256)), dim3(256), 0, s, u, ldu, h, ldh, M, ff,
                     dropout_thresh(p), dropout_thresh8(p), p > 0.f ? 1.f / (1.f - p) : 1.f, seed, off, layer);
  XTRL_LAUNCHED("glu_fwd");
  return XTRL_OK;
}
int glu_bwd(const float* dh, int lddh, const float* u, int ldu, float* du, int lddu, int M, int ff, float p,
            uint64_t seed, uint32_t off, uint32_t layer, hipStream_t s) {
  if ((int64_t)M * ff == 0) return XTRL_OK;
  hipLaunchKernelGGL(k_glu_bwd, dim3((unsigned)(((int64_t)M * ff + 255) / 256)), dim3(256), 0, s, dh, lddh, u, ldu, du,
                     lddu, M, ff, dropout_thresh(p), dropout_thresh8(p), p > 0.f ? 1.f / (1.f - p) : 1.f, seed, off,
                     layer);
  XTRL_LAUNCHED("glu_bwd");
  return XTRL_OK;
}

constexpr int CM_G = 16;
template <int REV>
__global__ __launch_bounds__(64 * CM_G) void k_causal_mean(const float* src, int lds, const float* add, int ldadd,
                                                          float* dst, int ldd, int n, int d) {
  __shared__ float tot[CM_G][64];
  const int e = blockIdx.x, cl = threadIdx.x & 63, grp = threadIdx.x >> 6;
  const int c = blockIdx.y * 64 + cl;
  const int per = (n + CM_G - 1) / CM_G, t0 = min(n, grp * per), t1 = min(n, t0 + per);
  const bool ok = c < d;
  const int64_t base = (int64_t)e * n;
  float s = 0.f;
  if (ok)
    for (int t = t0; t < t1; ++t) {
      const float v = src[(base + t) * lds + c];
      s += REV ? v / (float)(t + 1) : v;
    }
  tot[grp][cl] = s;
  __syncthreads();
  float carry = 0.f;
  if (REV) {
    for (int j = CM_G - 1; j > grp; --j) carry += tot[j][cl];
  } else {
    for (int j = 0; j < grp; ++j) carry += tot[j][cl];
  }
  if (!ok) return;
  if (REV) {
    for (int t = t1 - 1; t >= t0; --t) {
      carry += src[(base + t) * lds + c] / (float)(t + 1);
      dst[(base + t) * ldd + c] = (add ? add[(base + t) * ldadd + c] : 0.f) + carry;
    }
  } else {
    for (int t = t0; t < t1; ++t) {
      carry += src[(base + t) * lds + c];
      dst[(base + t) * ldd + c] = carry / (float)(t + 1);
    }
  }
}

__global__ void k_vec_add(const float* a, const float* b, float* out, int n) {
  const int i = blockIdx.x * 256 + threadIdx.x;
  if (i < n) out[i] = a[i] + b[i];
}

__global__ void k_rows_axpb(const float* a, int lda, float alpha, const float* b, int ldb, float* dst, int ldd,
                            int rows, int cols) {
  const int64_t i = (int64_t)blockIdx.x * 256 + threadIdx.x;
  if (i >= (int64_t)rows * cols) return;
  const int64_t r = i / cols;
  const int c = (int)(i - r * cols);
  float v = alpha * a[r * lda + c];
  if (b) v += b[r * ldb + c];
  dst[r * ldd + c] = v;
}

__global__ void k_action_rows(const int32_t* act, const float* W, int A, float* out, int ldo, int rows, int d) {
  const int64_t i = (int64_t)blockIdx.x * 256 + threadIdx.x;
  if (i >= (int64_t)rows * d) return;
  const int64_t r = i / d;
  const int c = (int)(i - r * d), a = act[r];
  out[r * ldo + c] = (a >= 0 && a < A) ? W[(int64_t)a * d + c] : 0.f;
}

__global__ void k_rows_bcast_ep(const float* src, float* dst, int ldd, int rows, int n, int d) {
  const int64_t i = (int64_t)blockIdx.x * 256 + threadIdx.x;
  if (i >= (int64_t)rows * d) return;
  const int64_t r = i / d;
  const int c = (int)(i - r * d);
  dst[r * ldd + c] = src[(r / n) * d + c];
}

inline unsigned blocks(int64_t n, int per) { return (unsigned)((n + per - 1) / per); }

struct Ctx {
  const XtrlTrainDesc* D;
  hipStream_t s;
  int T;
  SplitKQueue* q = nullptr;
  const float* P(int64_t off) const { return off >= 0 ? D->flat + off : nullptr; }
  float* G(int64_t off) const { return off >= 0 ? D->grad + off : nullptr; }
  void img(GemmArgs& g, int trans_b, int epi) const {
    wimg_find(g, trans_b, epi, D->flat, D->wimg_tab_host, D->wimg_n, D->wimg);
  }
};

inline int ld_ff(const XtrlTrainDesc* D) { return D->ld_ff > 0 ? D->ld_ff : D->ff; }

struct SideStream {
  hipStream_t s = nullptr;
  std::vector<hipEvent_t> ev;
  bool ok = false;
  bool ensure(size_t n) {
    constexpr unsigned flags = hipEventDisableTiming | hipEventReleaseToDevice;
    while (ok && ev.size() < n) {
      hipEvent_t e = nullptr;
      if (hipEventCreateWithFlags(&e, flags) != hipSuccess) return false;
      ev.push_back(e);
    }
    return ok;
  }
};
SideStream& side_stream() {
  static SideStream S = [] {
    SideStream x;
    int least = 0, greatest = 0;
    if (hipDeviceGetStreamPriorityRange(&least, &greatest) != hipSuccess) least = 0;
    x.ok = hipStreamCreateWithPriority(&x.s, hipStreamNonBlocking, least) == hipSuccess;
    return x;
  }();
  return S;
}
constexpr size_t side_events_needed(int L) { return 8 * (size_t)L + 6; }

struct Fork {
  hipStream_t main, side;
  SideStream* S;
  int next = 0;
  bool failed = false;
  bool on() const { return S != nullptr; }
  hipEvent_t take() {
    if ((size_t)next >= S->ev.size()) return nullptr;
    return S->ev[next++];
  }
  int fork() {
    if (!on()) return XTRL_OK;
    hipEvent_t e = take();
    if (!e || hipEventRecord(e, main) != hipSuccess || hipStreamWaitEvent(side, e, 0) != hipSuccess) {
      set_error("train: side-stream fork failed");
      return XTRL_E_HIP;
    }
    return XTRL_OK;
  }
  hipEvent_t mark() {
    if (!on()) return nullptr;
    hipEvent_t e = take();
    if (!e || hipEventRecord(e, side) != hipSuccess) {
      failed = true;
      return nullptr;
    }
    return e;
  }
  int wait(hipEvent_t e) {
    if (!on() || !e) return XTRL_OK;
    if (hipStreamWaitEvent(main, e, 0) != hipSuccess) {
      set_error("train: side-stream join failed");
      return XTRL_E_HIP;
    }
    return XTRL_OK;
  }
};

int linear_fwd(const Ctx& c, const float* A, int lda, const float* W, const float* bias, float* C, int ldc, int M,
               int N, int K, int epi, const float* R = nullptr, float* aux_out = nullptr, int ld_aux = 0,
               int act_cols = 1 << 30, int bias_col0 = 0, uint32_t drop_off = 0, uint32_t drop_layer = 0) {
  GemmArgs g;
  g.A = A; g.lda = lda; g.B = W; g.ldb = K; g.bias = bias; g.C = C; g.ldc = ldc; g.M = M; g.N = N; g.K = K;
  g.R = R; g.ldr = ldc; g.aux_out = aux_out; g.ld_aux_out = ld_aux; g.act_cols = act_cols; g.bias_col0 = bias_col0;
  if (epi == EPI_GELU_DROP) {
    g.seed = c.D->seed;
    g.drop_off = drop_off;
    g.drop_layer = drop_layer;
    g.drop_thresh = dropout_thresh(c.D->dropout);
    g.drop_thresh8 = dropout_thresh8(c.D->dropout);
    g.inv_keep = c.D->dropout > 0.f ? 1.f / (1.f - c.D->dropout) : 1.f;
  }
  c.img(g, 0, epi);
  return gemm_run(g, 0, 0, epi, c.s);
}

int linear_dgrad(const Ctx& c, const float* dY, int ldy, const float* W, float* dX, int ldx, int M, int N, int K,
                 int epi, const float* aux_in = nullptr, int ld_aux = 0, int act_cols = 1 << 30,
                 const float* aux_in2 = nullptr, int ld_aux2 = 0, float* aux_out = nullptr, int ld_aux_out = 0) {
  GemmArgs g;
  g.A = dY; g.lda = ldy; g.B = W; g.ldb = K; g.C = dX; g.ldc = ldx; g.M = M; g.N = K; g.K = N;
  g.aux_in = aux_in; g.ld_aux_in = ld_aux; g.act_cols = act_cols;
  g.aux_in2 = aux_in2; g.ld_aux_in2 = ld_aux2; g.aux_out = aux_out; g.ld_aux_out = ld_aux_out;
  c.img(g, 1, epi);
  return gemm_run(g, 0, 1, epi, c.s);
}

int wgrad(const Ctx& c, const float* dY, int ldy, const float* X, int ldx, float* dW, int M, int N, int K,
          float* db = nullptr, int db_n0 = 0) {
  const GemmProfile prof{c.D->prof_events, c.D->prof_flops, c.D->prof_cap, c.D->prof_n};
  return gemm_wgrad(dY, ldy, X, ldx, dW, K, M, N, K, 1.f, c.D->ws, c.D->ws_floats, c.s, db, db_n0,
                    c.D->prof_events && c.D->prof_n ? &prof : nullptr, c.q);
}

int colsum(const Ctx& c, const float* src, int ld, int rows, int cols, float* dst, const float* rw = nullptr,
           int ld_rw = 0, float rw_scale = 1.f) {
  if (!dst || cols <= 0) return XTRL_OK;
  int chunks = std::min(1024, std::max(1, rows / 16));
  const int chunk_rows = (rows + chunks - 1) / chunks;
  chunks = (rows + chunk_rows - 1) / chunk_rows;
  XTRL_REQUIRE((int64_t)chunks * cols <= c.D->part_floats, "train: partial-sum workspace too small");
  hipLaunchKernelGGL(k_colsum_part, dim3(blocks(cols, 256), chunks), dim3(256), 0, c.s, src, ld, rows, cols,
                     chunk_rows, rw, ld_rw, rw_scale, c.D->part);
  hipLaunchKernelGGL(k_colsum_final, dim3(blocks(cols, CS_COLS)), dim3(64 * CS_WAVES), 0, c.s, c.D->part, chunks, cols, dst);
  XTRL_LAUNCHED("train colsum");
  return XTRL_OK;
}

struct Backward {
  const XtrlTrainDesc* D;
  const char* what;
  size_t events_needed;
  Fork F;
  SplitKQueue skq;
  ColsumQueue csq;
  Ctx c, cw;
  int bucket = 0;
  bool wpin_on_main = false;
  Backward(const Ctx& main, size_t events, const char* what_)
      : D(main.D), what(what_), events_needed(events), F{main.s, nullptr, nullptr}, c(main), cw(main) {
    SideStream& side = side_stream();
    if (side.ok && side.ensure(events)) {
      F.side = side.s;
      F.S = &side;
      cw.s = side.s;
    }
    cw.q = &skq;
  }
  Backward(const Backward&) = delete;
  int bucket_done() {
    if (!D->grad_events) return XTRL_OK;
    if (int rc = csq.flush(c.s)) return rc;
    if (int rc = splitk_flush(skq, cw.s)) return rc;
    if (hipEventRecord((hipEvent_t)D->grad_events[2 * bucket], c.s) != hipSuccess ||
        hipEventRecord((hipEvent_t)D->grad_events[2 * bucket + 1], cw.s) != hipSuccess) {
      set_error("%s: gradient bucket event record failed", what);
      return XTRL_E_HIP;
    }
    ++bucket;
    return XTRL_OK;
  }
  int embed_grad(const float* g1, int ld1, const int32_t* prev, const float* g2, int ld2, const int32_t* next,
// ... 218 lines not shown
  const int cv = cols / V;
  const int64_t i = (int64_t)blockIdx.x * 256 + threadIdx.x;
  if (i >= (int64_t)nr * cv) return;
  const int r = (int)(i / cv), c = V * (int)(i - (int64_t)r * cv);
  const float* sp = src + (int64_t)rows[r] * lds + c;
  float* dp = dst + (int64_t)r * ldd + c;
  if constexpr (V == 4) *reinterpret_cast<float4*>(dp) = *reinterpret_cast<const float4*>(sp);
  else *dp = *sp;
}
template <int V>
__global__ void k_scatter_rows(const float* src, int lds, const int32_t* inv, int T, int cols, float* dst, int ldd) {
  const int cv = cols / V;
  const int64_t i = (int64_t)blockIdx.x * 256 + threadIdx.x;
  if (i >= (int64_t)T * cv) return;
  const int r = (int)(i / cv), c = V * (int)(i - (int64_t)r * cv);
  const int j = inv[r];
  float* dp = dst + (int64_t)r * ldd + c;
  if constexpr (V == 4)
    *reinterpret_cast<float4*>(dp) = j >= 0 ? *reinterpret_cast<const float4*>(src + (int64_t)j * lds + c)
                                            : make_float4(0.f, 0.f, 0.f, 0.f);
  else
    *dp = j >= 0 ? src[(int64_t)j * lds + c] : 0.f;
}
bool vec4_ok(const float* a, int lda, const float* b, int ldb, int cols) {
  return cols % 4 == 0 && lda % 4 == 0 && ldb % 4 == 0 && ((uintptr_t)a % 16) == 0 && ((uintptr_t)b % 16) == 0;
}
void gather_rows(const float* src, int lds, const int32_t* rows, int nr, int cols, float* dst, int ldd, hipStream_t s) {
  const bool v4 = vec4_ok(src, lds, dst, ldd, cols);
  const int64_t units = (int64_t)nr * (v4 ? cols / 4 : cols);
  if (v4) hipLaunchKernelGGL(k_gather_rows<4>, dim3(blocks(units, 256)), dim3(256), 0, s, src, lds, rows, nr, cols, dst, ldd);
  else hipLaunchKernelGGL(k_gather_rows<1>, dim3(blocks(units, 256)), dim3(256), 0, s, src, lds, rows, nr, cols, dst, ldd);
}
void scatter_rows(const float* src, int lds, const int32_t* inv, int T, int cols, float* dst, int ldd, hipStream_t s) {
  const bool v4 = vec4_ok(src, lds, dst, ldd, cols);
  const int64_t units = (int64_t)T * (v4 ? cols / 4 : cols);
  if (v4) hipLaunchKernelGGL(k_scatter_rows<4>, dim3(blocks(units, 256)), dim3(256), 0, s, src, lds, inv, T, cols, dst, ldd);
  else hipLaunchKernelGGL(k_scatter_rows<1>, dim3(blocks(units, 256)), dim3(256), 0, s, src, lds, inv, T, cols, dst, ldd);
}
bool heads_compact(const Ctx& c) {
  const XtrlTrainDesc* D = c.D;
  return D->Tv > 0 && D->Tv < c.T && D->b <= VR_MAXB && D->vrows && D->vinv && D->ewa_v && D->hp_v &&
         D->zp_v && D->pred_v && D->d_pred_v && D->dzp_v && D->dewa_v;
}
}

int heads_forward(const Ctx& c) {
  const XtrlTrainDesc* D = c.D;
  const int T = c.T, d = D->d, ldp = d + 4;
  const hipStream_t s = c.s;
  int rc;
  const int S1x2 = 2 * (D->S + 1);
  if (heads_compact(c)) {
    const int Tv = D->Tv;
    hipLaunchKernelGGL(k_valid_rows, dim3(1), dim3(1024), 0, s, D->lens, D->b, D->n, D->Tv, D->vrows, D->vinv);
    gather_rows(D->ewa, 2 * d, D->vrows, Tv, 2 * d, D->ewa_v, 2 * d, s);
    if ((rc = linear_fwd(c, D->ewa_v, 2 * d, c.P(D->w_pd), c.P(D->b_pd), D->hp_v, ldp, Tv, d + 1, 2 * d, EPI_SILU_SAVE,
                         nullptr, D->zp_v, ldp, d)))
      return rc;
    if ((rc = linear_fwd(c, D->hp_v, ldp, c.P(D->w_pred2), c.P(D->b_pred2), D->pred_v, S1x2, Tv, S1x2, d, EPI_NONE)))
      return rc;
    scatter_rows(D->pred_v, S1x2, D->vinv, T, S1x2, D->pred, S1x2, s);
    scatter_rows(D->hp_v + d, ldp, D->vinv, T, 1, D->done, 1, s);
  } else {
    if ((rc = linear_fwd(c, D->ewa, 2 * d, c.P(D->w_pd), c.P(D->b_pd), D->hp, ldp, T, d + 1, 2 * d, EPI_SILU_SAVE,
                         nullptr, D->zp, ldp, d)))
      return rc;
    if ((rc = linear_fwd(c, D->hp, ldp, c.P(D->w_pred2), c.P(D->b_pred2), D->pred, S1x2, T, S1x2, d, EPI_NONE)))
      return rc;
    hipLaunchKernelGGL(k_copy_col, dim3(blocks(T, 256)), dim3(256), 0, s, D->hp + d, ldp, D->done, 1, T);
  }
  if ((rc = linear_fwd(c, D->ac_in, D->in_dim, c.P(D->w_h1), c.P(D->b_h1), D->h1, 4 * d, T, 4 * d, D->in_dim,
                       EPI_SILU_SAVE, nullptr, D->z1, 4 * d)))
    return rc;
  if ((rc = linear_fwd(c, D->h1, 4 * d, c.P(D->w_a2), c.P(D->b_a2), D->raw, D->n_out, T, D->n_out, 2 * d, EPI_NONE)))
    return rc;
  if ((rc = linear_fwd(c, D->h1 + 2 * d, 4 * d, c.P(D->w_c2), c.P(D->b_c2), D->values, D->B, T, D->B, 2 * d,
                       EPI_NONE)))
    return rc;
  XTRL_LAUNCHED("train heads");
  return XTRL_OK;
}

int heads_backward(const Ctx& c, const Ctx& cw, Fork& F, bool embed_cols = true) {
  const XtrlTrainDesc* D = c.D;
  const int T = c.T, d = D->d, ldp = d + 4, S1x2 = 2 * (D->S + 1);
  const hipStream_t s = c.s;
  int rc;
  const bool cmp = heads_compact(c);
  if (cmp) {
    gather_rows(D->d_pred, S1x2, D->vrows, D->Tv, S1x2, D->d_pred_v, S1x2, s);
    gather_rows(D->d_done, 1, D->vrows, D->Tv, 1, D->dzp_v + d, ldp, s);
  }
  if ((rc = F.fork())) return rc;
  if ((rc = wgrad(cw, D->d_raw, D->n_out, D->h1, 4 * d, c.G(D->w_a2), T, D->n_out, 2 * d, c.G(D->b_a2)))) return rc;
  if ((rc = wgrad(cw, D->d_values, D->B, D->h1 + 2 * d, 4 * d, c.G(D->w_c2), T, D->B, 2 * d, c.G(D->b_c2)))) return rc;
  if ((rc = linear_dgrad(c, D->d_raw, D->n_out, c.P(D->w_a2), D->dz1, 4 * d, T, D->n_out, 2 * d, EPI_MUL_AUX, D->z1,
                         4 * d)))
    return rc;
  if ((rc = linear_dgrad(c, D->d_values, D->B, c.P(D->w_c2), D->dz1 + 2 * d, 4 * d, T, D->B, 2 * d, EPI_MUL_AUX,
                         D->z1 + 2 * d, 4 * d)))
    return rc;
  if ((rc = F.fork())) return rc;
  if ((rc = wgrad(cw, D->dz1, 4 * d, D->ac_in, D->in_dim, c.G(D->w_h1), T, 4 * d, D->in_dim, c.G(D->b_h1)))) return rc;
  if (embed_cols) {
    if ((rc = linear_dgrad(c, D->dz1, 4 * d, c.P(D->w_h1), D->dac, D->in_dim, T, 4 * d, D->in_dim, EPI_NONE))) return rc;
  } else {
    GemmArgs g;
    g.A = D->dz1; g.lda = 4 * d; g.B = c.P(D->w_h1) + d; g.ldb = D->in_dim; g.C = D->dac + d; g.ldc = D->in_dim;
    g.M = T; g.N = D->in_dim - d; g.K = 4 * d;
    c.img(g, 1, EPI_NONE);
    if ((rc = gemm_run(g, 0, 1, EPI_NONE, c.s))) return rc;
  }
  if ((rc = F.fork())) return rc;
  if ((rc = wgrad(cw, D->dac + d, D->in_dim, D->swr, D->S + 1, c.G(D->w_se), T, d, D->S, c.G(D->b_se)))) return rc;
  if (D->evolutionary) {
    XTRL_REQUIRE((int64_t)D->b * d <= D->part_floats, "train: partial-sum workspace too small");
    hipLaunchKernelGGL(k_latent_grad, dim3(D->b, (d + 63) / 64), dim3(64 * LG_G), 0, s, D->dac, D->in_dim, 2 * d,
                       D->b, D->n, d, D->part, D->packed ? D->ep_off : nullptr);
    hipLaunchKernelGGL(k_latent_wgrad, dim3(blocks(d * (D->G + 1), 256)), dim3(256), 0, s, D->part, D->latent, D->b,
                       d, D->G, c.G(D->w_lat), c.G(D->b_lat));
    XTRL_LAUNCHED("train latent grad");
  }
  if (cmp) {
    const int Tv = D->Tv;
    if ((rc = wgrad(cw, D->d_pred_v, S1x2, D->hp_v, ldp, c.G(D->w_pred2), Tv, S1x2, d, c.G(D->b_pred2)))) return rc;
    if ((rc = linear_dgrad(c, D->d_pred_v, S1x2, c.P(D->w_pred2), D->dzp_v, ldp, Tv, S1x2, d, EPI_MUL_AUX, D->zp_v,
                           ldp)))
      return rc;
    if ((rc = F.fork())) return rc;
    if ((rc = wgrad(cw, D->dzp_v, ldp, D->ewa_v, 2 * d, c.G(D->w_pd), Tv, d + 1, 2 * d, c.G(D->b_pd)))) return rc;
    if ((rc = linear_dgrad(c, D->dzp_v, ldp, c.P(D->w_pd), D->dewa_v, 2 * d, Tv, d + 1, 2 * d, EPI_NONE))) return rc;
    scatter_rows(D->dewa_v, 2 * d, D->vinv, T, 2 * d, D->dewa, 2 * d, s);
    XTRL_LAUNCHED("train heads backward (compact)");
    return XTRL_OK;
  }
  if ((rc = wgrad(cw, D->d_pred, S1x2, D->hp, ldp, c.G(D->w_pred2), T, S1x2, d, c.G(D->b_pred2)))) return rc;
  if ((rc = linear_dgrad(c, D->d_pred, S1x2, c.P(D->w_pred2), D->dzp, ldp, T, S1x2, d, EPI_MUL_AUX, D->zp, ldp))) return rc;
  hipLaunchKernelGGL(k_copy_col, dim3(blocks(T, 256)), dim3(256), 0, s, D->d_done, 1, D->dzp + d, ldp, T);
  if ((rc = F.fork())) return rc;
  if ((rc = wgrad(cw, D->dzp, ldp, D->ewa, 2 * d, c.G(D->w_pd), T, d + 1, 2 * d, c.G(D->b_pd)))) return rc;
  if ((rc = linear_dgrad(c, D->dzp, ldp, c.P(D->w_pd), D->dewa, 2 * d, T, d + 1, 2 * d, EPI_NONE))) return rc;
  return XTRL_OK;
}

int train_forward_rows(const XtrlTrainDesc* D, int Trows, hipStream_t s) {
  if (int rc = validate(D)) return rc;
  const Ctx c{D, s, Trows};
  const int32_t* rows = D->packed ? D->vrows : nullptr;
  const int T = c.T, d = D->d, I = D->H * D->dh, ff = D->ff, lf = ld_ff(D);
  const int Ikv = kv_inner(D), nq3 = I + 2 * Ikv;
  int rc;
  if (D->wimg && D->wimg_tab && D->wimg_tab_host && D->wimg_n > 0 && wimg_enabled())
    if ((rc = wimg_build(D->flat, D->wimg_tab_host, D->wimg_tab, D->wimg_n, D->wimg, D->wimg_bytes, s))) return rc;
  if (D->evolutionary) {
    hipLaunchKernelGGL(k_latent_embed, dim3(blocks(D->b * d, 256)), dim3(256), 0, s, D->latent, c.P(D->w_lat),
                       c.P(D->b_lat), D->lat_e, D->b, D->G, d);
  }
  EmbedArgs ea{D->swr, c.P(D->w_pin), c.P(D->act_emb), c.P(D->act_emb_b), c.P(D->reward_embed), c.P(D->w_se),
               c.P(D->b_se), D->lat_e, D->prev_action_f, D->next_action_f, D->prev_action, D->next_action,
               D->layers[0].x_attn, D->ac_in, D->ewa, T, D->n, D->S, D->A, d, D->in_dim, D->continuous,
               D->evolutionary, D->reward_keep, nullptr, nullptr, nullptr, D->rms_norm, rows};
  const bool fuse = ln_fusable(D);
  if (fuse) {
    const XtrlTrainLayer& L0 = D->layers[0];
    ea.ln_g = c.P(L0.ln_attn);
    ea.xn = L0.xn_attn;
    ea.st = L0.st_attn;
    if (D->S == 8) hipLaunchKernelGGL(k_embed_ln<8>, dim3(blocks(T, EMB_LN_TOK)), dim3(256), 0, s, ea);
    else hipLaunchKernelGGL(k_embed_ln<0>, dim3(blocks(T, EMB_LN_TOK)), dim3(256), 0, s, ea);
  } else if (D->S == 8) {
    hipLaunchKernelGGL(k_embed<8>, dim3(blocks(T, EMB_TOK)), dim3(256), 0, s, ea);
  } else {
    hipLaunchKernelGGL(k_embed<0>, dim3(blocks(T, EMB_TOK)), dim3(256), 0, s, ea);
  }
  XTRL_LAUNCHED("train embed");
  for (int li = 0; li < D->L; ++li) {
    const XtrlTrainLayer& Ly = D->layers[li];
    if (!fuse)
      if ((rc = ln_fwd(c, Ly.x_attn, c.P(Ly.ln_attn), Ly.xn_attn, d, nullptr, 0, Ly.st_attn))) return rc;
    if ((rc = linear_fwd(c, Ly.xn_attn, d, c.P(Ly.w_proj), c.P(Ly.b_proj), Ly.proj, Ly.n_qkv, T, Ly.n_qkv, d,
                         EPI_NONE, nullptr, nullptr, 0, 1 << 30, nq3)))
      return rc;
    const int mix_col = Ly.mix ? nq3 + (D->gate_values ? I : 0) : -1;
    PrepArgs pa{Ly.proj, D->layers[0].proj, Ly.qkv, D->inv_freq, T, D->n, D->H, D->dh, I, Ly.n_qkv,
                D->layers[0].n_qkv, D->rot_dim, mix_col, D->qk_norm, D->xpos_base, rows, Ikv};
    const dim3 pg = rows ? dim3(blocks(nq3 / 2, PREP_T), T) : dim3(blocks(nq3 / 2, PREP_T), D->n, D->b);
    hipLaunchKernelGGL(k_qkv_prep, pg, dim3(PREP_T), 0, s, pa);
    XTRL_LAUNCHED("train qkv_prep");
    const AttnProblem ap = attn_problem(c, Ly, li);
    if ((rc = attn_fwd_ex(ap, Ly.qkv, Ly.qkv + I, Ly.qkv + I + Ikv, Ly.o, Ly.lse,
                          D->gate_values ? Ly.proj + nq3 : nullptr, D->gate_values ? Ly.og : nullptr, s)))
      return rc;
    if (fuse) {
      if ((rc = linear_res_ln(c, D->gate_values ? Ly.og : Ly.o, I, c.P(Ly.w_out), nullptr, Ly.x_attn, Ly.x_ff, I,
                              c.P(Ly.ln_ff), Ly.xn_ff, d, nullptr, 0, Ly.st_ff)))
        return rc;
    } else {
      if ((rc = linear_fwd(c, D->gate_values ? Ly.og : Ly.o, I, c.P(Ly.w_out), nullptr, Ly.x_ff, d, T, d, I, EPI_NONE,
                           Ly.x_attn)))
        return rc;
      if ((rc = ln_fwd(c, Ly.x_ff, c.P(Ly.ln_ff), Ly.xn_ff, d, nullptr, 0, Ly.st_ff))) return rc;
    }
    if (D->ff_glu) {
      if ((rc = linear_fwd(c, Ly.xn_ff, d, c.P(Ly.w_ff1), c.P(Ly.b_ff1), Ly.u, D->ld_u2, T, 2 * ff, d, EPI_NONE)))
        return rc;
      if ((rc = glu_fwd(Ly.u, D->ld_u2, Ly.hd, lf, T, ff, D->dropout, D->seed, D->ff_offset, (uint32_t)li, s)))
        return rc;
    } else if ((rc = linear_fwd(c, Ly.xn_ff, d, c.P(Ly.w_ff1), c.P(Ly.b_ff1), Ly.hd, lf, T, ff, d, EPI_GELU_DROP,
                                nullptr, Ly.u, lf, 1 << 30, 0, D->ff_offset, (uint32_t)li))) {
      return rc;
    }
    float* x_out = li + 1 < D->L ? D->layers[li + 1].x_attn : D->x_final;
    if (fuse && li + 1 < D->L) {
      const XtrlTrainLayer& Ln = D->layers[li + 1];
      if ((rc = linear_res_ln(c, Ly.hd, lf, c.P(Ly.w_ff2), c.P(Ly.b_ff2), Ly.x_ff, x_out, ff, c.P(Ln.ln_attn),
                              Ln.xn_attn, d, nullptr, 0, Ln.st_attn)))
        return rc;
    } else if (fuse) {
      if ((rc = linear_res_ln(c, Ly.hd, lf, c.P(Ly.w_ff2), c.P(Ly.b_ff2), Ly.x_ff, x_out, ff, c.P(D->ln_final),
                              D->ac_in, D->in_dim, D->ewa, 2 * d, D->st_final)))
        return rc;
    } else {
      if ((rc = linear_fwd(c, Ly.hd, lf, c.P(Ly.w_ff2), c.P(Ly.b_ff2), x_out, d, T, d, ff, EPI_NONE, Ly.x_ff))) return rc;
    }
  }
  if (!fuse)
    if ((rc = ln_fwd(c, D->x_final, c.P(D->ln_final), D->ac_in, D->in_dim, D->ewa, 2 * d, D->st_final))) return rc;
  if ((rc = heads_forward(c))) return rc;
  XTRL_LAUNCHED("train forward");
  return XTRL_OK;
}

int train_backward_rows(const XtrlTrainDesc* D, int Trows, hipStream_t s) {
  if (int rc = validate(D)) return rc;
  XTRL_REQUIRE(D->d_raw && D->d_values && D->d_pred && D->d_done, "train: missing loss gradients");
  Backward B(Ctx{D, s, Trows}, side_events_needed(D->L), "train");
  const Ctx &c = B.c, &cw = B.cw;
  Fork& F = B.F;
  ColsumQueue& csq = B.csq;
  const int32_t* rows = D->packed ? D->vrows : nullptr;
  const int T = c.T, d = D->d, I = D->H * D->dh, ff = D->ff, lf = ld_ff(D);
  const int Ikv = kv_inner(D), nq3 = I + 2 * Ikv;
  int rc;
  const bool fuse = ln_fusable(D);
  XTRL_REQUIRE(!fuse || D->dx2, "train: fused LayerNorm backward needs dx2");
  if (fuse) {
    csq.base = D->part;
    csq.cap = D->part_floats;
  }
  const int64_t Td = (int64_t)T * d;
  float* dx_top = fuse ? D->dx + D->L * Td : D->dx;
  if ((rc = heads_backward(c, cw, F, !fuse))) return rc;
  if (fuse) {
    const int nb = (T + gemm_ln_rows(d) - 1) / gemm_ln_rows(d);
    XTRL_REQUIRE((int64_t)nb * d <= D->part_floats, "train: partial-sum workspace too small");
    GemmArgs g;
    g.A = D->dz1; g.lda = 4 * d; g.B = c.P(D->w_h1); g.ldb = D->in_dim; g.C = dx_top; g.ldc = d;
    g.M = T; g.N = d; g.K = 4 * d;
    g.ln_g = c.P(D->ln_final); g.ln_x = D->x_final; g.ln_stats = D->st_final; g.ln_rms = D->rms_norm;
    float* P = csq.take_or_flush(nb, d, c.G(D->ln_final), s, &rc);
    if (rc) return rc;
    g.ln_gpre = D->dewa; g.ln_ldg = 2 * d; g.ln_gscale = D->frac_head_grad; g.ln_part = P ? P : D->part;
    c.img(g, 1, EPI_LN_BWD2);
    if ((rc = gemm_run(g, 0, 1, EPI_LN_BWD2, s))) return rc;
    if (!P)
      hipLaunchKernelGGL(k_colsum_final, dim3(blocks(d, CS_COLS)), dim3(64 * CS_WAVES), 0, s, D->part, nb, d,
                         c.G(D->ln_final));
    XTRL_LAUNCHED("train final-norm backward");
  } else if ((rc = ln_bwd(c, D->dac, D->in_dim, D->frac_head_grad, D->dewa, 2 * d, D->x_final, D->st_final,
                          c.P(D->ln_final), nullptr, dx_top, c.G(D->ln_final)))) {
    return rc;
  }
  if ((rc = B.bucket_done())) return rc;
  int maxq = 0;
  for (int li = 0; li < D->L; ++li) maxq = std::max(maxq, D->layers[li].n_qkv);
  auto Gx = [&](int slot) { return fuse ? D->dx + slot * Td : D->dx; };
  auto Gx2 = [&](int li) { return fuse ? D->dx2 + li * Td : D->dx2; };
  const int f1 = D->ff_glu ? 2 * ff : ff, ld_f1 = D->ff_glu ? D->ld_u2 : lf;
  auto Gff = [&](int li) { return fuse ? D->dff + (int64_t)li * T * ld_f1 : D->dff; };
  auto Gpr = [&](int li) { return fuse ? D->dproj + (int64_t)li * T * maxq : D->dproj; };
  const bool any_mix = [&] {
    for (int j = 1; j < D->L; ++j)
      if (D->layers[j].mix) return true;
    return false;
  }();
  hipEvent_t e_ff1 = nullptr, e_proj = nullptr;
  for (int li = D->L - 1; li >= 0; --li) {
    const XtrlTrainLayer& Ly = D->layers[li];
    float* gout = Gx(li + 1);
    float* dff = Gff(li);
    float* dproj = Gpr(li);
    if ((rc = F.fork())) return rc;
    if ((rc = wgrad(cw, gout, d, Ly.hd, lf, c.G(Ly.w_ff2), T, d, ff, c.G(Ly.b_ff2)))) return rc;
    hipEvent_t e_ff2 = F.mark();
    if (!fuse && (rc = F.wait(e_ff1))) return rc;
    if (D->ff_glu) {
      if ((rc = linear_dgrad(c, gout, d, c.P(Ly.w_ff2), D->glu_dh, lf, T, d, ff, EPI_NONE))) return rc;
      if ((rc = glu_bwd(D->glu_dh, lf, Ly.u, D->ld_u2, dff, ld_f1, T, ff, D->dropout, D->seed, D->ff_offset,
                        (uint32_t)li, s)))
        return rc;
    } else if ((rc = linear_dgrad(c, gout, d, c.P(Ly.w_ff2), dff, lf, T, d, ff, EPI_MUL_AUX, Ly.u, lf))) {
      return rc;
    }
    if ((rc = F.fork())) return rc;
    if ((rc = wgrad(cw, dff, ld_f1, Ly.xn_ff, d, c.G(Ly.w_ff1), T, f1, d, c.G(Ly.b_ff1)))) return rc;
    e_ff1 = F.mark();
// ... 327 lines not shown

int fractal_train_backward(const XtrlTrainDesc* D, const XtrlFractalTrainDesc* F, hipStream_t s) {
  if (int rc = validate_fractal(D, F)) return rc;
  XTRL_REQUIRE(D->d_raw && D->d_values && D->d_pred && D->d_done, "fractal train: missing loss gradients");
  XTRL_REQUIRE(F->dxa && F->dxb && F->ds && F->dmean && F->dga && F->dgv && F->dz && F->dqkv && F->dob && F->dcat &&
                   F->dhfa,
               "fractal train: missing backward scratch");
  const int Lv = F->levels;
  Backward B(Ctx{D, s, D->b * D->n}, fractal_events_needed(Lv), "fractal train");
  const Ctx &c = B.c, &cw = B.cw;
  Fork& Fk = B.F;
  const int T = c.T, d = D->d, I = D->H * D->dh, ff = D->ff, lf = ld_ff(D), ldcat = (Lv + 1) * d;
  const int64_t Td = (int64_t)T * d;
  int rc;
  if ((rc = heads_backward(c, cw, Fk))) return rc;
  float* dfeat = F->ds + 3 * (int64_t)Lv * Td;
  if ((rc = rows_axpb(c, D->dac, D->in_dim, D->frac_head_grad, D->dewa, 2 * d, dfeat, d, T, d))) return rc;
  if (D->continuous) {
    if ((rc = Fk.fork())) return rc;
    if ((rc = wgrad(cw, D->dewa + d, 2 * d, D->next_action_f, D->A, c.G(D->act_emb), T, d, D->A, c.G(D->act_emb_b))))
      return rc;
  } else {
    if ((rc = B.embed_grad(nullptr, 0, nullptr, D->dewa + d, 2 * d, D->next_action, c.G(D->act_emb)))) return rc;
    if ((rc = Fk.fork())) return rc;
  }
  if ((rc = wgrad(cw, dfeat, d, F->hfa, 2 * d, c.G(F->w_fa2), T, d, 2 * d, c.G(F->b_fa2)))) return rc;
  if ((rc = linear_dgrad(c, dfeat, d, c.P(F->w_fa2), F->dhfa, 2 * d, T, d, 2 * d, EPI_MASK_POS, F->hfa, 2 * d))) return rc;
  if ((rc = Fk.fork())) return rc;
  if ((rc = wgrad(cw, F->dhfa, 2 * d, F->cat, ldcat, c.G(F->w_fa0), T, 2 * d, ldcat, c.G(F->b_fa0)))) return rc;
  if ((rc = linear_dgrad(c, F->dhfa, 2 * d, c.P(F->w_fa0), F->dcat, ldcat, T, 2 * d, ldcat, EPI_NONE))) return rc;
  if ((rc = B.bucket_done())) return rc;
  const bool post2 = ln_fusable_fractal(D);
  const float* dgn = F->dcat + Lv * d;
  int lddgn = ldcat;
  const float* dxn = nullptr;
  for (int l = Lv - 1; l >= 0; --l) {
    const XtrlFractalTrainLevel& V = F->level[l];
    float* ds1 = F->ds + 3 * (int64_t)l * Td;
    float* ds2 = ds1 + Td;
    float* ds3 = ds1 + 2 * Td;
    float* dz = F->dz + (int64_t)l * T * lf;
    float* dgv = F->dgv + (int64_t)l * T * I;
    float* dqkv = F->dqkv + (int64_t)l * T * 3 * I;
    float* dgc = F->dga + (int64_t)l * Td;
    if ((rc = Fk.fork())) return rc;
    if ((rc = wgrad(cw, dgn, lddgn, V.mean, d, c.G(F->w_gu), T, d, d, c.G(F->b_gu)))) return rc;
    if ((rc = wgrad(cw, F->dcat + l * d, ldcat, V.mean, d, c.G(V.w_proj), T, d, d, c.G(V.b_proj)))) return rc;
    if ((rc = linear_dgrad(c, dgn, lddgn, c.P(F->w_gu), F->dmean, d, T, d, d, EPI_NONE))) return rc;
    if ((rc = dgrad_res(c, F->dcat + l * d, ldcat, c.P(V.w_proj), d, d, F->dmean, d, F->dmean, d))) return rc;
    if ((rc = causal_mean(c, F->dmean, d, dxn, d, F->dxa, d, true))) return rc;
    if ((rc = ln_bwd(c, F->dxa, d, 1.f, nullptr, 0, V.s3, V.st3, c.P(V.ln3_w), nullptr, ds3, c.G(V.ln3_w),
                     c.G(V.ln3_b))))
      return rc;
    if ((rc = Fk.fork())) return rc;
    if ((rc = wgrad(cw, ds3, d, V.h, lf, c.G(V.w_ff2), T, d, ff, c.G(V.b_ff2)))) return rc;
    if ((rc = linear_dgrad(c, ds3, d, c.P(V.w_ff2), dz, lf, T, d, ff, EPI_MUL_AUX, V.u, lf))) return rc;
    if ((rc = Fk.fork())) return rc;
    if ((rc = wgrad(cw, dz, lf, V.x2, d, c.G(V.w_ff1), T, ff, d, c.G(V.b_ff1)))) return rc;
    if (post2) {
      if ((rc = dgrad_post_ln2(c, dz, lf, c.P(V.w_ff1), ds3, V, ds2, ds1))) return rc;
    } else {
      if ((rc = dgrad_res(c, dz, lf, c.P(V.w_ff1), ff, d, ds3, d, F->dxb, d))) return rc;
      if ((rc = ln_bwd(c, F->dxb, d, 1.f, nullptr, 0, V.s2, V.st2, c.P(V.ln2_w), nullptr, ds2, c.G(V.ln2_w),
                       c.G(V.ln2_b))))
        return rc;
      if ((rc = ln_bwd(c, ds2, d, 1.f, nullptr, 0, V.s1, V.st1, c.P(V.ln1_w), nullptr, ds1, c.G(V.ln1_w),
                       c.G(V.ln1_b))))
        return rc;
    }
    if ((rc = Fk.fork())) return rc;
    if ((rc = wgrad(cw, ds2, d, V.gv, I, c.G(V.w_go), T, d, I))) return rc;
    if ((rc = linear_dgrad(c, ds2, d, c.P(V.w_go), dgv, I, T, d, I, EPI_NONE))) return rc;
    if ((rc = Fk.fork())) return rc;
    if ((rc = wgrad(cw, dgv, I, V.g, d, c.G(V.w_gv), T, I, d))) return rc;
    if ((rc = dgrad_res(c, dgv, I, c.P(V.w_gv), I, d, dgn, lddgn, dgc, d))) return rc;
    if ((rc = Fk.fork())) return rc;
    if ((rc = wgrad(cw, ds1, d, V.o, I, c.G(V.w_out), T, d, I))) return rc;
    if ((rc = linear_dgrad(c, ds1, d, c.P(V.w_out), F->dob, I, T, d, I, EPI_NONE))) return rc;
    const AttnProblem ap = fractal_attn(c, l);
    if ((rc = attn_bwd_ex(ap, V.qkv, V.qkv + I, V.qkv + 2 * I, V.o, V.lse, F->dob, dqkv, dqkv + I, dqkv + 2 * I,
                          D->delta, s)))
      return rc;
    if ((rc = Fk.fork())) return rc;
    if ((rc = wgrad(cw, dqkv, 3 * I, V.xin, d, c.G(V.w_qkv), T, 3 * I, d))) return rc;
    if ((rc = dgrad_res(c, dqkv, 3 * I, c.P(V.w_qkv), 3 * I, d, ds1, d, F->dxa, d))) return rc;
    if ((rc = colsum(c, F->dxa, d, T, d, c.G(V.level_embed)))) return rc;
    dxn = F->dxa;
    dgn = dgc;
    lddgn = d;
    if ((rc = B.bucket_done())) return rc;
  }
  if ((rc = B.input_proj_wgrad(F->dxa, c.G(F->b_in), true))) return rc;
  if ((rc = colsum(c, dgn, lddgn, T, d, c.G(F->g_init)))) return rc;
  return B.finish();
}

}

extern "C" int xtrl_train_forward(const XtrlTrainDesc* desc, void* stream) {
  return xtrl::train_forward(desc, xtrl::as_stream(stream));
}

extern "C" int xtrl_train_backward(const XtrlTrainDesc* desc, void* stream) {
  return xtrl::train_backward(desc, xtrl::as_stream(stream));
}

extern "C" int xtrl_fractal_train_forward(const XtrlTrainDesc* base, const XtrlFractalTrainDesc* f, void* stream) {
  return xtrl::fractal_train_forward(base, f, xtrl::as_stream(stream));
}

extern "C" int xtrl_fractal_train_backward(const XtrlTrainDesc* base, const XtrlFractalTrainDesc* f, void* stream) {
  return xtrl::fractal_train_backward(base, f, xtrl::as_stream(stream));
}

extern "C" int64_t xtrl_train_part_floats(int T, int b, int d, int A) {
  if (T <= 0 || d <= 0) return 0;
  const int64_t ln = (int64_t)((T + xtrl::LN_ROWS - 1) / xtrl::LN_ROWS) * d;
  const int64_t cs = (int64_t)std::min(1024, std::max(1, T / 16)) * d;
  const int64_t lat = (int64_t)std::max(b, 1) * d;
  const int64_t emb = (int64_t)std::max(A, 1) * d;
  return std::max(std::max(ln, cs), std::max(lat, emb));
}

extern "C" int xtrl_train_wimg_plan(const XtrlTrainDesc* D, XtrlWimgEntry* tab, int cap, int64_t* bytes) {
  int n = 0, blk = 0;
  int64_t at = 0;
  auto add = [&](int64_t w_off, int trans_b, int N, int K, int ld, int epi) {
    if (w_off < 0 || N <= 0 || K <= 0) return;
    XtrlWimgEntry E{};
    E.w_off = w_off; E.img_off = at; E.N = N; E.K = K; E.ld = ld; E.trans_b = trans_b;
    E.BN = xtrl::wimg_tile_bn(N, epi); E.blk0 = blk;
    const int64_t tiles = (int64_t)((N + E.BN - 1) / E.BN) * ((K + 31) / 32);
    if (tab && n < cap) tab[n] = E;
    ++n;
    blk += (int)tiles;
    at += tiles * XTRL_WIMG_TILE_BYTES(E.BN);
  };
  if (D && D->layers && D->L > 0 && D->d > 0 && xtrl::ln_fusable(D)) {
    const int d = D->d, I = D->H * D->dh, f1 = D->ff_glu ? 2 * D->ff : D->ff;
    for (int li = 0; li < D->L; ++li) {
      const XtrlTrainLayer& Ly = D->layers[li];
      add(Ly.w_out, 0, d, I, I, xtrl::EPI_RES_LN);
      add(Ly.w_ff2, 0, d, D->ff, D->ff, xtrl::EPI_RES_LN);
      add(Ly.w_ff1, 1, d, f1, d, xtrl::EPI_LN_BWD);
      add(Ly.w_proj, 1, d, Ly.n_qkv, d, xtrl::EPI_LN_BWD);
    }
    add(D->w_h1, 1, d, 4 * d, D->in_dim, xtrl::EPI_LN_BWD2);
    if (D->w_h1 >= 0) add(D->w_h1 + d, 1, D->in_dim - d, 4 * d, D->in_dim, xtrl::EPI_NONE);
  }
  if (bytes) *bytes = at;
  return n;
}

extern "C" int64_t xtrl_train_pack_floats(int T, int S, int A, int n_out, int B) {
  if (T <= 0) return 0;
  return xtrl::pack_bufs(nullptr, T, S, A, n_out, B).floats;
}

extern "C" int xtrl_linear_gelu_drop(const float* X, int ldx, const float* W, const float* bias, float* Y, int ldy,
                                     float* deriv, int ld_deriv, int M, int N, int K, float p, uint64_t seed,
                                     uint32_t offset, uint32_t layer, void* stream) {
  XTRL_REQUIRE(layer < (1u << 22), "linear_gelu_drop: layer %u out of range", layer);
  XTRL_REQUIRE(X && W && Y && deriv && M >= 0 && N > 0 && K > 0 && p >= 0.f && p < 1.f && ldx >= K && ldy >= N &&
                   ld_deriv >= N,
               "linear_gelu_drop: bad arguments");
  if (M == 0) return XTRL_OK;
  xtrl::GemmArgs g;
  g.A = X; g.lda = ldx; g.B = W; g.ldb = K; g.bias = bias; g.C = Y; g.ldc = ldy; g.M = M; g.N = N; g.K = K;
  g.aux_out = deriv; g.ld_aux_out = ld_deriv;
  g.seed = seed; g.drop_off = offset; g.drop_layer = layer;
  g.drop_thresh = xtrl::dropout_thresh(p);
  g.drop_thresh8 = xtrl::dropout_thresh8(p);
  g.inv_keep = p > 0.f ? 1.f / (1.f - p) : 1.f;
  return xtrl::gemm_run(g, 0, 0, xtrl::EPI_GELU_DROP, xtrl::as_stream(stream));
}

extern "C" int xtrl_glu_drop_fwd(const float* u, int ldu, float* h, int ldh, int M, int ff, float p, uint64_t seed,
                                 uint32_t offset, uint32_t layer, void* stream) {
  XTRL_REQUIRE(layer < (1u << 22), "glu_drop_fwd: layer %u out of range", layer);
  XTRL_REQUIRE(u && h && M >= 0 && ff > 0 && ldu >= 2 * ff && ldh >= ff && p >= 0.f && p < 1.f,
               "glu_drop_fwd: bad arguments");
  return xtrl::glu_fwd(u, ldu, h, ldh, M, ff, p, seed, offset, layer, xtrl::as_stream(stream));
}

extern "C" int xtrl_glu_drop_bwd(const float* dh, int lddh, const float* u, int ldu, float* du, int lddu, int M, int ff,
                                 float p, uint64_t seed, uint32_t offset, uint32_t layer, void* stream) {
  XTRL_REQUIRE(layer < (1u << 22), "glu_drop_bwd: layer %u out of range", layer);
  XTRL_REQUIRE(dh && u && du && M >= 0 && ff > 0 && lddh >= ff && ldu >= 2 * ff && lddu >= 2 * ff && p >= 0.f && p < 1.f,
               "glu_drop_bwd: bad arguments");
  return xtrl::glu_bwd(dh, lddh, u, ldu, du, lddu, M, ff, p, seed, offset, layer, xtrl::as_stream(stream));
}

extern "C" int xtrl_ff_dropout_mask(uint8_t* mask, int M, int N, float p, uint64_t seed, uint32_t offset,
                                    uint32_t layer, void* stream) {
  XTRL_REQUIRE(layer < (1u << 22), "ff_dropout_mask: layer %u out of range", layer);
  XTRL_REQUIRE(mask && M >= 0 && N >= 0 && p >= 0.f && p < 1.f, "ff_dropout_mask: bad arguments");
  if ((int64_t)M * N == 0) return XTRL_OK;
  hipLaunchKernelGGL(xtrl::k_ff_mask, dim3((unsigned)(((int64_t)M * N + 255) / 256)), dim3(256), 0,
                     xtrl::as_stream(stream), mask, M, N, xtrl::dropout_thresh(p), xtrl::dropout_thresh8(p), seed, offset, layer);
  XTRL_LAUNCHED("ff_dropout_mask");
  return XTRL_OK;
}
```

x-transformers-rl_amd/xtrl_amd/_lib.py:

```python
from __future__ import annotations

import ctypes as C
import os
from pathlib import Path

import torch

LIB_PATH = Path(os.environ.get('XTRL_LIB', Path(__file__).resolve().parent / 'libxtrl_hip.so'))
ABI_VERSION = 27

P = C.c_void_p
I32, I64, U32, U64, F32 = C.c_int, C.c_int64, C.c_uint32, C.c_uint64, C.c_float

ACT_NONE, ACT_GELU, ACT_SILU, ACT_RELU = 0, 1, 2, 3

LS = dict(loss=0, actor=1, critic=2, autoreg=3, done=4, adv_mean=5, adv_den=6, L=7, Lc=8, nmask=9, nwm=10,
          kcrit=11, dL=12, dLc=13)
LOSS_TOK, LOSS_STATS = 30, 32


class DecodeLayer(C.Structure):
    _fields_ = [(n, P) for n in ('ln_attn', 'w_qkv', 'b_qkv', 'w_out', 'ln_ff', 'w_ff1', 'b_ff1', 'w_ff2', 'b_ff2',
                                 'k_cache', 'v_cache', 'w_out_t', 'w_ff1x', 'w_ff2x', 'w_qkv_t', 'w_ff1_t', 'w_ff2_t',
                                 'w_ff1f', 'w_ff2f', 'mem_k', 'mem_v')]


class RngState(C.Structure):
    _fields_ = [('seed', U64), ('update', U32), ('slot_offset', U32)]


class DecodeDesc(C.Structure):
    _fields_ = ([(n, I32) for n in ('E', 'S', 'A', 'B', 'd', 'L', 'H', 'dh', 'Tmax', 'G', 'ff', 'in_dim', 'n_qkv',
                                    'continuous', 'squash', 'evolutionary', 'gate_values', 'value_residual',
                                    'learned_mix', 'rotary_abs', 'rot_dim', 'sim_mode', 'hazard_log2', 'no_reward_cond',
                                    'state_only')]
                + [('rs_eps', F32), ('clamp_lo', F32), ('clamp_hi', F32), ('has_clamp', I32)]
                + [(n, P) for n in ('w_pin', 'b_pin', 'act_emb', 'act_emb_b', 'reward_embed', 'w_se', 'b_se',
                                    'ln_final', 'w_h1', 'b_h1', 'w_h2', 'b_h2', 'inv_freq')]
                + [('layers', C.POINTER(DecodeLayer))]
                + [(n, P) for n in ('rs_mean', 'rs_var', 'state', 'prev_action', 'prev_action_f', 'prev_reward',
                                    'alive', 'lens', 'cum_reward', 'episode_of_slot', 'slot_of_row', 'rng', 'traj_states',
                                    'traj_actions', 'traj_actions_f', 'traj_logp', 'traj_rewards', 'traj_bounds',
                                    'traj_values', 'x', 'qkv', 'att', 'hff', 'ac_in', 'logits', 'v1', 'xn', 'live_rows', 'live_count',
                                    'mlp_part', 'mlp_cnt', 'lat_embed')]
                + [('prof_events', C.POINTER(C.c_void_p))]
                + [(n, P) for n in ('w_h1_t', 'w_h2_t')]
                + [('layers_dev', C.POINTER(DecodeLayer))]
                + [(n, P) for n in ('w_h1x', 'heads_part', 'heads_cnt', 'row_part', 'row_cnt')]
                + [('ff_glu', I32), ('hglu', P), ('qk_norm', I32), ('attn_scale', F32), ('xpos_base', F32),
                   ('rms_norm', I32), ('act_host', P), ('attn_window', I32), ('Hkv', I32),
                   ('alibi_slopes', P), ('num_mem_kv', I32), ('add_zero_kv', I32)])


class FractalLevel(C.Structure):
    _fields_ = [(n, P) for n in ('w_qkv', 'w_out', 'ln1_w', 'ln1_b', 'w_c', 'ln2_w', 'ln2_b', 'w_ff1', 'b_ff1',
                                 'w_ff2', 'b_ff2', 'ln3_w', 'ln3_b', 'w_pg', 'b_pg', 'level_emb', 'sums')]


class FractalDesc(C.Structure):
    _fields_ = ([('levels', I32), ('ln_eps', F32), ('level', C.POINTER(FractalLevel))]
                + [(n, P) for n in ('g_init', 'c0', 'w_fa0', 'b_fa0', 'w_fa2', 'b_fa2', 'g', 'c2', 'tmp', 'x2', 'mean',
                                    'allf', 'hagg')])


class LossDesc(C.Structure):
    _fields_ = ([(n, I32) for n in ('b', 'n', 'A', 'B', 'S1', 'continuous', 'squash', 'hl_reduction_mean')]
                + [(n, F32) for n in ('eps_clip', 'value_clip', 'entropy_weight', 'w_actor', 'w_critic', 'w_autoreg',
                                      'lo', 'hi', 'sigma')]
                + [(n, P) for n in ('raw_actions', 'values', 'pred_raw', 'done_logit', 'actions', 'actions_f',
                                    'old_logp', 'returns', 'old_values', 'dones', 'lens', 'real', 'support', 'centers',
                                    'tok', 'stats', 'd_raw_actions', 'd_values', 'd_pred_raw', 'd_done_logit')])


class TrainLayer(C.Structure):
    _fields_ = ([(n, I64) for n in ('ln_attn', 'w_proj', 'b_proj', 'w_out', 'ln_ff', 'w_ff1', 'b_ff1', 'w_ff2',
                                    'b_ff2')]
                + [('n_qkv', I32), ('mix', I32)]
                + [(n, P) for n in ('x_attn', 'x_ff', 'xn_attn', 'xn_ff', 'st_attn', 'st_ff', 'proj', 'qkv', 'o', 'og',
                                    'lse', 'u', 'hd')]
                + [('mem_k', I64), ('mem_v', I64)])


class WimgEntry(C.Structure):
    _fields_ = [('w_off', I64), ('img_off', I64), ('N', I32), ('K', I32), ('ld', I32), ('trans_b', I32), ('BN', I32),
                ('blk0', I32)]


WIMG_XRS = 40


def wimg_tile_bytes(bn: int) -> int:
    return 3 * bn * WIMG_XRS * 2


class TrainDesc(C.Structure):
    _fields_ = ([(n, I32) for n in ('b', 'n', 'S', 'A', 'd', 'L', 'H', 'dh', 'ff', 'B', 'in_dim', 'n_out', 'G',
                                    'continuous', 'evolutionary', 'gate_values', 'rot_dim')]
                + [(n, F32) for n in ('dropout', 'frac_head_grad', 'reward_keep', 'attn_scale')]
                + [('seed', U64), ('attn_offset', U32), ('ff_offset', U32), ('flat', P), ('grad', P)]
                + [(n, I64) for n in ('w_pin', 'act_emb', 'act_emb_b', 'reward_embed', 'w_se', 'b_se', 'ln_final',
                                      'w_pd', 'b_pd', 'w_pred2', 'b_pred2', 'w_lat', 'b_lat', 'w_h1', 'b_h1', 'w_a2',
                                      'b_a2', 'w_c2', 'b_c2')]
                + [(n, P) for n in ('inv_freq', 'swr', 'prev_action', 'next_action', 'prev_action_f',
                                    'next_action_f', 'latent', 'lens', 'raw', 'values', 'pred', 'done', 'x_final',
                                    'st_final', 'ac_in', 'ewa', 'zp', 'hp', 'z1', 'h1', 'lat_e', 'd_raw', 'd_values',
                                    'd_pred', 'd_done', 'dx', 'dx2', 'dxn', 'dff', 'dproj', 'dog', 'dvfirst', 'dz1', 'dac',
                                    'dzp', 'dewa', 'delta', 'part')]
                + [('part_floats', I64), ('ws', P), ('ws_floats', I64), ('layers', C.POINTER(TrainLayer)),
                   ('prof_events', C.POINTER(C.c_void_p)), ('prof_flops', P), ('prof_cap', I32), ('prof_n', P),
                   ('grad_events', C.POINTER(C.c_void_p)), ('ld_ff', I32),
                   ('ff_glu', I32), ('ld_u2', I32), ('glu_dh', P),
                   ('qk_norm', I32), ('xpos_base', F32), ('rms_norm', I32),
                   ('Tv', I32), ('vrows', P), ('vinv', P), ('ewa_v', P), ('hp_v', P), ('zp_v', P), ('pred_v', P),
                   ('d_pred_v', P), ('dzp_v', P), ('dewa_v', P), ('dq_part', P), ('dq_part_floats', I64),
                   ('packed', I32), ('ep_off', P), ('pack_ws', P), ('pack_ws_floats', I64), ('attn_window', I32),
                   ('Hkv', I32), ('wimg', P), ('wimg_bytes', I64), ('wimg_tab', P),
                   ('wimg_tab_host', C.POINTER(WimgEntry)), ('wimg_n', I32), ('alibi_slopes', P),
                   ('num_mem_kv', I32), ('add_zero_kv', I32), ('sink_ws', P), ('sink_ws_floats', I64)])


class FractalTrainLevel(C.Structure):
    _fields_ = ([(n, I64) for n in ('w_qkv', 'w_out', 'w_gv', 'w_go', 'ln1_w', 'ln1_b', 'ln2_w', 'ln2_b', 'ln3_w',
                                    'ln3_b', 'w_ff1', 'b_ff1', 'w_ff2', 'b_ff2', 'w_proj', 'b_proj', 'level_embed')]
                + [(n, P) for n in ('xin', 'qkv', 'o', 'lse', 's1', 'x1', 'st1', 'g', 'gv', 's2', 'x2', 'st2', 'h', 'u',
                                    's3', 'x3', 'st3', 'mean')])


class FractalTrainDesc(C.Structure):
    _fields_ = ([('levels', I32)]
                + [(n, I64) for n in ('b_in', 'g_init', 'w_gu', 'b_gu', 'w_fa0', 'b_fa0', 'w_fa2', 'b_fa2')]
                + [(n, P) for n in ('scale_embeds', 'le', 'bias0', 'cat', 'hfa', 'dxa', 'dxb', 'dmean', 'ds',
                                    'dga', 'dgb', 'dgv', 'dz', 'dqkv', 'dob', 'dcat', 'dhfa')]
                + [('level', C.POINTER(FractalTrainLevel))])


class BatchDesc(C.Structure):
    _fields_ = ([(n, I32) for n in ('N', 'Tmax', 'n', 'b', 'S', 'A', 'B', 'continuous')]
                + [(n, P) for n in ('states', 'actions', 'actions_f', 'rewards', 'logp', 'bounds', 'values', 'returns',
                                    'lens', 'idx', 'rs_mean', 'rs_var', 'swr', 'prev_action', 'action',
                                    'prev_action_f', 'action_f', 'old_logp', 'mb_returns', 'old_values', 'dones',
                                    'mb_lens', 'rs_part', 'rs_m')])


SIGNATURES = {
    'xtrl_abi_version': (I32, []),
    'xtrl_struct_size': (C.c_int64, [C.c_char_p]),
    'xtrl_last_error': (C.c_char_p, []),
    'xtrl_gemm_f32': (I32, [P, I32, P, I32, P, P, P, I32, P, I32, P, I64, I32, I32, I32, I32, P]),
    'xtrl_gemm_ex': (I32, [I32, I32, P, I32, P, I32, P, P, I32, I32, I32, I32, F32, P]),
    'xtrl_gemm_wgrad': (I32, [P, I32, P, I32, P, I32, I32, I32, I32, F32, P, I64, P]),
    'xtrl_gemm_wgrad_db': (I32, [P, I32, P, I32, P, I32, I32, I32, I32, F32, P, I64, P, I32, P]),
    'xtrl_linear_gelu_drop': (I32, [P, I32, P, P, P, I32, P, I32, I32, I32, I32, F32, U64, U32, U32, P]),
    'xtrl_layernorm_f32': (I32, [P, I32, P, P, I32, I32, I32, P]),
    'xtrl_rollout_begin': (I32, [C.POINTER(DecodeDesc), P]),
    'xtrl_decode_step': (I32, [C.POINTER(DecodeDesc), I32, P]),
    'xtrl_decode_step_rows': (I32, [C.POINTER(DecodeDesc), I32, I32, P]),
    'xtrl_row_stamps': (I32, [I32, P, I32, P]),
    'xtrl_host_decode': (I32, [C.POINTER(DecodeDesc), I32, I32, P, P]),
    'xtrl_host_feedback': (I32, [C.POINTER(DecodeDesc), I32, P, P, I32, I32, P]),
    'xtrl_rollout_env_feedback': (I32, [C.POINTER(DecodeDesc), I32, P, P, P, P, I32, I32, P]),
    'xtrl_host_row_step': (I32, [C.POINTER(DecodeDesc), I32, P, I32, I32, P, P]),
    'xtrl_host_wait': (I32, [P, C.c_uint32, C.c_double]),
    'xtrl_dgemm': (I32, [P, I32, P, P, P, I32, P, I32, P, I32, P, P, I32, I32, I32, I32, P]),
    'xtrl_dgemm_pack': (I32, [P, I32, I32, I32, P, P]),
    'xtrl_fractal_decode_step': (I32, [C.POINTER(DecodeDesc), C.POINTER(FractalDesc), I32, P]),
    'xtrl_dgemm_packed_floats': (I64, [I32, I32]),
    'xtrl_dgemm_pack_x6': (I32, [P, I32, I32, I32, P, P]),
    'xtrl_dgemm_packed_x6_elems': (I64, [I32, I32]),
    'xtrl_dgemm_pack_f8': (I32, [P, I32, I32, I32, P, P]),
    'xtrl_glu_drop_fwd': (I32, [P, I32, P, I32, I32, I32, F32, U64, U32, U32, P]),
    'xtrl_glu_drop_bwd': (I32, [P, I32, P, I32, P, I32, I32, I32, F32, U64, U32, U32, P]),
    'xtrl_dgemm_packed_f8_floats': (I64, [I32, I32]),
    'xtrl_hlgauss_gae': (I32, [P, I64, P, P, I64, P, P, P, I32, I32, I32, F32, F32, P, P, P]),
    'xtrl_attn_fwd': (I32, [P, P, P, P, P, P, I32, I32, I32, I32, F32, F32, U64, U32, U32, P]),
    'xtrl_attn_bwd': (I32, [P, P, P, P, P, P, P, P, P, P, P, I32, I32, I32, I32, F32, F32, U64, U32, U32, P]),
    'xtrl_attn_bwd_part_floats': (I64, [I32, I32, I32, I32]),
    'xtrl_train_pack_floats': (I64, [I32, I32, I32, I32, I32]),
    'xtrl_attn_bwd_part': (I32, [P, P, P, P, P, P, P, P, P, P, P, P, I64, I32, I32, I32, I32, F32, F32, U64, U32, U32,
                                  P]),
    'xtrl_attn_fwd_win': (I32, [P, P, P, P, P, P, I32, I32, I32, I32, F32, F32, U64, U32, U32, I32, P]),
    'xtrl_attn_bwd_win': (I32, [P, P, P, P, P, P, P, P, P, P, P, I32, I32, I32, I32, F32, F32, U64, U32, U32, I32, P]),
    'xtrl_attn_bwd_part_win': (I32, [P, P, P, P, P, P, P, P, P, P, P, P, I64, I32, I32, I32, I32, F32, F32, U64, U32,
                                      U32, I32, P]),
    'xtrl_attn_fwd_gqa': (I32, [P, P, P, P, P, P, I32, I32, I32, I32, I32, F32, F32, U64, U32, U32, I32, P]),
    'xtrl_attn_bwd_gqa': (I32, [P, P, P, P, P, P, P, P, P, P, P, I32, I32, I32, I32, I32, F32, F32, U64, U32, U32, I32,
                                 P]),
    'xtrl_attn_bwd_part_gqa': (I32, [P, P, P, P, P, P, P, P, P, P, P, P, I64, I32, I32, I32, I32, I32, F32, F32, U64,
                                      U32, U32, I32, P]),
    'xtrl_attn_sink_ws_floats': (I64, [I32, I32, I32, I32]),
    'xtrl_attn_fwd_sink': (I32, [P, P, P, P, P, P, P, P, I32, I32, I32, I32, I32, F32, F32, U64, U32, U32, I32, I32, I32,
                                 P]),
    'xtrl_attn_bwd_sink': (I32, [P, P, P, P, P, P, P, P, P, P, P, P, P, P, P, P, I64, I32, I32, I32, I32, I32, F32, F32,
                                 U64, U32, U32, I32, I32, I32, P]),
    'xtrl_attn_bwd_part_sink': (I32, [P, P, P, P, P, P, P, P, P, P, P, P, I64, P, P, P, P, P, I64, I32, I32, I32, I32,
                                      I32, F32, F32, U64, U32, U32, I32, I32, I32, P]),
    'xtrl_attn_fwd_alibi': (I32, [P, P, P, P, P, P, P, P, I32, I32, I32, I32, I32, F32, F32, U64, U32, U32, I32, I32, I32,
                                  P, P]),
    'xtrl_attn_bwd_alibi': (I32, [P, P, P, P, P, P, P, P, P, P, P, P, P, P, P, P, I64, I32, I32, I32, I32, I32, F32, F32,
                                  U64, U32, U32, I32, I32, I32, P, P]),
    'xtrl_attn_bwd_part_alibi': (I32, [P, P, P, P, P, P, P, P, P, P, P, P, I64, P, P, P, P, P, I64, I32, I32, I32, I32,
                                       I32, F32, F32, U64, U32, U32, I32, I32, I32, P, P]),
    'xtrl_loss_fwd': (I32, [C.POINTER(LossDesc), P]),
    'xtrl_loss_bwd': (I32, [C.POINTER(LossDesc), F32, P]),
    'xtrl_grad_norm': (I32, [P, I64, P, F32, P, P]),
    'xtrl_adopt_atan2': (I32, [P, P, P, P, P, I64, P, I32, P, I32, P, P, F32, F32, F32, F32, F32, F32, F32, F32, F32,
                               I32, P]),
    'xtrl_ema_lerp': (I32, [P, P, I64, F32, P]),
    'xtrl_sim_reset': (I32, [P, I32, I32, U64, U32, P, P]),
    'xtrl_train_forward': (I32, [C.POINTER(TrainDesc), P]),
    'xtrl_train_backward': (I32, [C.POINTER(TrainDesc), P]),
    'xtrl_ff_dropout_mask': (I32, [P, I32, I32, F32, U64, U32, U32, P]),
    'xtrl_train_part_floats': (C.c_int64, [I32, I32, I32, I32]),
    'xtrl_train_wimg_plan': (I32, [C.POINTER(TrainDesc), C.POINTER(WimgEntry), I32, C.POINTER(I64)]),
    'xtrl_wimg_launch_count': (I64, []),
    'xtrl_wimg_build': (I32, [P, C.POINTER(WimgEntry), P, I32, P, I64, P]),
    'xtrl_minibatch_gather': (I32, [C.POINTER(BatchDesc), P]),
    'xtrl_rsnorm_update': (I32, [P, P, P, I32, I32, P]),
    'xtrl_attn_fwd_tokens': (I32, [P, I32, P, I32, P, I32, P, P, I32, P, I32, I32, I32, I32, F32, I32, P]),
    'xtrl_rows_add': (I32, [P, I32, P, P, I32, I32, I32, P]),
    'xtrl_add_layernorm': (I32, [P, I32, P, I32, I32, P, P, P, I32, I32, I32, F32, P]),
    'xtrl_seq_mean': (I32, [P, I32, I32, I32, I32, P, I32, P]),
    'xtrl_safe_embed': (I32, [P, I32, P, I32, P, I32, P]),
    'xtrl_wm_post': (I32, [P, I32, I32, I32, P, P, I32, P, P]),
    'xtrl_rng_uniform': (F32, [U64, U32, U32, U32, U32, U32]),
    'xtrl_rng_normal': (F32, [U64, U32, U32, U32, U32, U32]),
    'xtrl_source_hash': (C.c_char_p, []),
    'xtrl_fractal_train_forward': (I32, [C.POINTER(TrainDesc), C.POINTER(FractalTrainDesc), P]),
    'xtrl_fractal_train_backward': (I32, [C.POINTER(TrainDesc), C.POINTER(FractalTrainDesc), P]),
}

STRUCTS = {'XtrlDecodeLayer': DecodeLayer, 'XtrlRngState': RngState, 'XtrlDecodeDesc': DecodeDesc,
           'XtrlTrainLayer': TrainLayer, 'XtrlTrainDesc': TrainDesc, 'XtrlBatchDesc': BatchDesc,
           'XtrlLossDesc': LossDesc, 'XtrlFractalLevel': FractalLevel, 'XtrlFractalDesc': FractalDesc,
           'XtrlFractalTrainLevel': FractalTrainLevel, 'XtrlFractalTrainDesc': FractalTrainDesc,
           'XtrlWimgEntry': WimgEntry}

_lib = None


def load():
    global _lib
    if _lib is None:
        if not LIB_PATH.exists():
            raise RuntimeError(f'{LIB_PATH} is missing: build it with `make -C x-transformers-rl_amd` '
                               f'or __graft_entry__.build() (the MI355X path has no CPU fallback)')
        lib = C.CDLL(str(LIB_PATH))
        for name, (res, args) in SIGNATURES.items():
            fn = getattr(lib, name)
            fn.restype, fn.argtypes = res, args
        if lib.xtrl_abi_version() != ABI_VERSION:
            raise RuntimeError(f'libxtrl_hip ABI {lib.xtrl_abi_version()} != {ABI_VERSION}')
        from ._srchash import source_hash
        built, here = lib.xtrl_source_hash().decode(), source_hash()
        if built != here and 'XTRL_LIB' not in os.environ:
            raise RuntimeError(f'{LIB_PATH} was built from sources {built}, the tree holds {here}: rebuild it '
                               f'with `make -C x-transformers-rl_amd` or __graft_entry__.build()')
        for cname, py in STRUCTS.items():
            got = lib.xtrl_struct_size(cname.encode())
            if got != C.sizeof(py):
                raise RuntimeError(f'libxtrl_hip {cname} is {got} bytes, the binding {C.sizeof(py)}: rebuild')
        _lib = lib
    return _lib


def lib():
    if not torch.cuda.is_available():
        raise RuntimeError('xtrl_amd needs a ROCm GPU (gfx950); no CPU fallback exists by design')
    return load()


def check(rc, what=''):
    if rc != 0:
        msg = load().xtrl_last_error().decode(errors='replace')
        raise RuntimeError(f'libxtrl_hip {what} failed (code {rc}): {msg}')


def ptr(t):
    return None if t is None else C.c_void_p(t.data_ptr())


def stream():
    return C.c_void_p(torch.cuda.current_stream().cuda_stream)


def rng_uniform(seed, update, slot, t, field, sub=0):
    return load().xtrl_rng_uniform(seed & 0xFFFFFFFFFFFFFFFF, update, slot, t, field, sub)


FIELD_STATE, FIELD_REWARD, FIELD_TERM, FIELD_SAMPLE, FIELD_COIN, FIELD_DROPOUT, FIELD_FF_DROPOUT = 1, 2, 3, 4, 5, 6, 7
```

x-transformers-rl_amd/xtrl_amd/train.py:

```python
from __future__ import annotations

import ctypes as C
import os

import torch

from . import _lib as L
from .params import FlatParams


WIMG_DEFAULT = os.environ.get('XTRL_WIMG', '0') == '1'


def ld_ff(ff):
    return ff + 16 if ff % 256 == 0 else ff


def _off(flat, name):
    return flat.index[name][0] if name in flat.index else -1


def _span_off(flat, names):
    flat.span(names)
    return flat.index[names[0]][0]


def _compact_bufs(D, c, T, dev, b_max, n_max):
    d, ldp, S1x2 = c.dim, c.dim + 4, 2 * (c.state_dim + 1)
    f32 = dict(device=dev, dtype=torch.float32)
    bufs = dict(vrows=torch.empty(T, device=dev, dtype=torch.int32), vinv=torch.empty(T, device=dev, dtype=torch.int32),
                ewa_v=torch.empty(T, 2 * d, **f32), hp_v=torch.empty(T, ldp, **f32), zp_v=torch.empty(T, ldp, **f32),
                pred_v=torch.empty(T, S1x2, **f32), d_pred_v=torch.empty(T, S1x2, **f32),
                dzp_v=torch.empty(T, ldp, **f32), dewa_v=torch.empty(T, 2 * d, **f32))
    for k, t in bufs.items():
        setattr(D, k, t.data_ptr())
    D.Tv = 0
    bufs['ep_off'] = torch.zeros(b_max + 1, device=dev, dtype=torch.int32)
    D.ep_off, D.packed, D.pack_ws, D.pack_ws_floats = bufs['ep_off'].data_ptr(), 0, None, 0
    D.dq_part, D.dq_part_floats = None, 0
    if n_max > 128 and c.dim_head == 16:
        nf = int(L.lib().xtrl_attn_bwd_part_floats(b_max, c.heads, n_max, c.dim_head))
        bufs['dq_part'] = torch.empty(nf, **f32)
        D.dq_part, D.dq_part_floats = bufs['dq_part'].data_ptr(), nf
    return bufs


def _alloc_wimg(D, dev):
    nbytes = C.c_int64(0)
    n = int(L.lib().xtrl_train_wimg_plan(C.byref(D), None, 0, C.byref(nbytes)))
    if n <= 0 or nbytes.value <= 0:
        return None
    tab = (L.WimgEntry * n)()
    L.lib().xtrl_train_wimg_plan(C.byref(D), tab, n, C.byref(nbytes))
    arena = torch.empty(nbytes.value, device=dev, dtype=torch.uint8)
    tab_dev = torch.frombuffer(bytearray(bytes(tab)), dtype=torch.uint8).to(dev)
    D.wimg, D.wimg_bytes = arena.data_ptr(), nbytes.value
    D.wimg_tab, D.wimg_tab_host, D.wimg_n = tab_dev.data_ptr(), C.cast(tab, C.POINTER(L.WimgEntry)), n
    return dict(tab=tab, tab_dev=tab_dev, arena=arena)


def _heads_desc(D, c, flat):
    off = lambda n: _off(flat, n)
    if c.continuous:
        D.act_emb, D.act_emb_b = off('action_embeds.weight'), off('action_embeds.bias')
    else:
        D.act_emb, D.act_emb_b = off('action_embeds.embed.weight'), -1
    D.reward_embed, D.w_se, D.b_se = off('reward_embed'), off('to_state_embed.weight'), off('to_state_embed.bias')
    D.w_pd = _span_off(flat, ['to_pred.0.weight', 'to_pred_done.0.weight'])
    D.b_pd = _span_off(flat, ['to_pred.0.bias', 'to_pred_done.0.bias'])
    D.w_pred2, D.b_pred2 = off('to_pred.2.weight'), off('to_pred.2.bias')
    D.w_lat, D.b_lat = off('latent_to_embed.weight'), off('latent_to_embed.bias')
    D.w_h1 = _span_off(flat, ['action_head.0.weight', 'critic_head.0.weight'])
    D.b_h1 = _span_off(flat, ['action_head.0.bias', 'critic_head.0.bias'])
    D.w_a2, D.b_a2 = off('action_head.2.weight'), off('action_head.2.bias')
    D.w_c2, D.b_c2 = off('critic_head.2.weight'), off('critic_head.2.bias')


class FusedTrainStep:
    def __init__(self, model, flat: FlatParams, ws: torch.Tensor, b_max: int, n_max: int):
        c = model.cfg
        self.model, self.flat, self.cfg, self.ws = model, flat, c, ws
        dev = flat.flat.device
        self.dev = dev
        d, H, dh, L_ = c.dim, c.heads, c.dim_head, c.depth
        I, ff, B = H * dh, c.dim * c.ff_mult, c.num_bins
        Ikv = c.kv_inner
        S, A = c.state_dim, c.num_actions
        n_out = A * (2 if c.continuous else 1)
        T = b_max * n_max
        self.b_max, self.n_max, self.T_max = b_max, n_max, T
        self.inv_freq = model.transformer.attn_layers.rotary_pos_emb.inv_freq.to(dev).contiguous()
        rot = 2 * self.inv_freq.numel()
        f32 = dict(device=dev, dtype=torch.float32)
        E = lambda *shape: torch.empty(*shape, **f32)
        off = lambda name: flat.index[name][0] if name in flat.index else -1
        pre = 'transformer.attn_layers.layers.'

        def span_off(names):
            a0 = flat.index[names[0]][0]
            flat.span(names)
            return a0

        self.layers_py = []
        self.ld_ff = lff = ld_ff(ff)
        glu = bool(getattr(c, 'ff_glu', False))
        lu2 = ld_ff(2 * ff) if glu else lff
        layers = (L.TrainLayer * L_)()
        X = [E(T, d) for _ in range(L_ + 1)]
        max_qkv = 0
        nw = 'g' if c.rms_norm else 'gamma'
        for li in range(L_):
            mix = bool(c.value_residual and c.learned_mix and li > 0)
            pa, pf = f'{pre}{2 * li}.', f'{pre}{2 * li + 1}.'
            wn = [pa + '1.to_q.weight', pa + '1.to_k.weight', pa + '1.to_v.weight']
            wn += [pa + '1.to_v_gate.weight'] if c.gate_values else []
            wn += [pa + '1.to_value_residual_mix.0.weight'] if mix else []
            bn = ([pa + '1.to_v_gate.bias'] if c.gate_values else []) + \
                 ([pa + '1.to_value_residual_mix.0.bias'] if mix else [])
            n_qkv = I + 2 * Ikv + (I if c.gate_values else 0) + (c.n_kv_heads if mix else 0)
            max_qkv = max(max_qkv, n_qkv)
            bufs = dict(x_attn=X[li], x_ff=E(T, d), xn_attn=E(T, d), xn_ff=E(T, d), st_attn=E(T, 2), st_ff=E(T, 2),
                        proj=E(T, n_qkv), qkv=E(T, I + 2 * Ikv), o=E(T, I), lse=E(b_max * H * n_max), u=E(T, lu2),
                        hd=E(T, lff))
            bufs['og'] = E(T, I) if c.gate_values else bufs['o']
            self.layers_py.append(bufs)
            Ly = layers[li]
            Ly.ln_attn, Ly.w_proj = off(pa + '0.0.' + nw), span_off(wn)
            Ly.b_proj = span_off(bn) if bn else -1
            Ly.w_out, Ly.ln_ff = off(pa + '1.to_out.weight'), off(pf + '0.0.' + nw)
            f1 = pf + ('1.ff.0.proj.' if glu else '1.ff.0.0.')
            Ly.w_ff1, Ly.b_ff1 = off(f1 + 'weight'), off(f1 + 'bias')
            Ly.w_ff2, Ly.b_ff2 = off(pf + '1.ff.2.weight'), off(pf + '1.ff.2.bias')
            Ly.n_qkv, Ly.mix = n_qkv, int(mix)
            Ly.mem_k, Ly.mem_v = off(pa + '1.mem_k'), off(pa + '1.mem_v')
            for k, t in bufs.items():
                setattr(Ly, k, t.data_ptr())
        self.layers = layers
        self.X = X
        ldp = d + 4
        self.buf = dict(x_final=X[L_], st_final=E(T, 2), ac_in=E(T, c.in_dim), ewa=E(T, 2 * d), zp=E(T, ldp),
                        hp=E(T, ldp), z1=E(T, 4 * d), h1=E(T, 4 * d), lat_e=E(max(b_max, 1), d),
                        raw=E(T, n_out), values=E(T, B), pred=E(T, 2 * (S + 1)), done=E(T),
                        d_raw=E(T, n_out), d_values=E(T, B), d_pred=E(T, 2 * (S + 1)), d_done=E(T),
                        dx=E(L_ + 1, T, d), dx2=E(L_, T, d), dxn=E(T, d), dff=E(L_, T, lu2), dproj=E(L_, T, max_qkv),
                        dog=E(T, I), dvfirst=E(T, Ikv),
                        dz1=E(T, 4 * d), dac=E(T, c.in_dim), dzp=E(T, ldp), dewa=E(T, 2 * d),
                        delta=E(b_max * H * n_max))
        if glu:
            self.buf['glu_dh'] = E(T, lff)
        part = max(256 * max((2 if glu else 1) * ff, 4 * d, B, max_qkv), 1024 * max(A, 1) * d,
                   int(L.lib().xtrl_train_part_floats(T, b_max, d, A)))
        self.buf['part'] = E(part)
        self.tok = torch.empty(b_max, n_max, L.LOSS_TOK, **f32)
        self.stats = torch.zeros(L.LOSS_STATS, **f32)

        D = L.TrainDesc()
        D.S, D.A, D.d, D.L, D.H, D.dh, D.ff, D.B = S, A, d, L_, H, dh, ff, B
        D.in_dim, D.n_out, D.G = c.in_dim, n_out, c.dim_gene if c.evolutionary else 0
        D.continuous, D.evolutionary, D.gate_values, D.rot_dim = int(c.continuous), int(c.evolutionary), \
            int(c.gate_values), rot
        D.frac_head_grad = float(c.frac_head_grad)
        D.attn_scale = float(c.qk_norm_scale) if c.qk_norm else float(dh ** -0.5)
        D.qk_norm, D.xpos_base = int(c.qk_norm), float(c.xpos_scale_base) if c.rotary_xpos else 0.
        D.flat, D.grad = flat.flat.data_ptr(), flat.grad.data_ptr()
        D.w_pin = off('transformer.project_in.weight')
        _heads_desc(D, c, flat)
        D.ln_final = off('transformer.attn_layers.final_norm.' + nw)
        D.rms_norm = int(c.rms_norm)
        D.attn_window = int(c.attn_window)
        D.Hkv = int(c.n_kv_heads)
        D.num_mem_kv, D.add_zero_kv = int(getattr(c, 'num_mem_kv', 0)), int(bool(getattr(c, 'add_zero_kv', False)))
        if D.num_mem_kv:
            self.sink_ws = E(int(L.lib().xtrl_attn_sink_ws_floats(b_max, H, D.num_mem_kv, dh)))
            D.sink_ws, D.sink_ws_floats = self.sink_ws.data_ptr(), self.sink_ws.numel()
        if int(getattr(c, 'alibi_heads', 0)):
            from . import ops
            self.alibi_slopes = ops.alibi_slopes(H, c.alibi_heads).to(dev)
            D.alibi_slopes = self.alibi_slopes.data_ptr()
        D.inv_freq = self.inv_freq.data_ptr()
        for k, t in self.buf.items():
            setattr(D, k, t.data_ptr())
        D.part_floats = self.buf['part'].numel()
        D.ws, D.ws_floats = ws.data_ptr(), ws.numel()
        D.layers = C.cast(layers, C.POINTER(L.TrainLayer))
        D.ld_ff = lff
        D.ff_glu, D.ld_u2 = int(glu), (lu2 if glu else 0)
        self.cbuf = _compact_bufs(D, c, T, dev, b_max, n_max)
        self.D = D
        self.wimg = None
        if WIMG_DEFAULT:
            self.use_weight_images(True)

    def use_weight_images(self, on: bool):
        D = self.D
        if not on or isinstance(self, FractalTrainStep):
            D.wimg, D.wimg_bytes, D.wimg_tab, D.wimg_tab_host, D.wimg_n = None, 0, None, None, 0
            return
        if self.wimg is None:
            self.wimg = _alloc_wimg(D, self.dev)
        w = self.wimg
        if w is not None:
            D.wimg, D.wimg_bytes = w['arena'].data_ptr(), w['arena'].numel()
            D.wimg_tab, D.wimg_tab_host, D.wimg_n = w['tab_dev'].data_ptr(), C.cast(w['tab'], C.POINTER(L.WimgEntry)), \
                len(w['tab'])

    def forward(self, swr, prev_action, next_action, latent, lens, reward_keep, seed, attn_offset, ff_offset,
                dropout, Tv=0, packed=False):
        self._bind_inputs(swr, prev_action, next_action, latent, lens, reward_keep, seed, attn_offset, ff_offset,
                          dropout, Tv)
        D = self.D
        D.packed = 0
        if packed:
            assert 0 < Tv <= D.b * D.n, (Tv, D.b, D.n)
            D.Tv, D.packed = int(Tv), 1
            if self.cbuf.get('pack_ws') is None:
                c = self.cfg
                nf = int(L.lib().xtrl_train_pack_floats(self.T_max, c.state_dim, c.num_actions, D.n_out, c.num_bins))
                self.cbuf['pack_ws'] = torch.empty(nf, device=self.dev, dtype=torch.float32)
                D.pack_ws, D.pack_ws_floats = self.cbuf['pack_ws'].data_ptr(), nf
        L.check(L.lib().xtrl_train_forward(C.byref(self.D), L.stream()), 'train_forward')
        return self._outputs()

    def _bind_inputs(self, swr, prev_action, next_action, latent, lens, reward_keep, seed, attn_offset, ff_offset,
                     dropout, Tv=0):
        c, D = self.cfg, self.D
        b, n = swr.shape[0], swr.shape[1]
        assert b <= self.b_max and n <= self.n_max, (b, n, self.b_max, self.n_max)
        assert 0 <= Tv <= b * n, (Tv, b, n)
        D.Tv = int(Tv) if Tv < b * n else 0
        for t in (swr, prev_action, next_action, lens):
            assert t.is_cuda and t.is_contiguous()
        self._keep = [swr, prev_action, next_action, latent, lens]
        D.b, D.n = b, n
        D.dropout, D.reward_keep = float(dropout), float(reward_keep)
        D.seed, D.attn_offset, D.ff_offset = int(seed) & (2 ** 64 - 1), int(attn_offset) & 0xFFFFFFFF, \
            int(ff_offset) & 0xFFFFFFFF
        D.swr, D.lens = swr.data_ptr(), lens.data_ptr()
        if c.continuous:
            D.prev_action_f, D.next_action_f, D.prev_action, D.next_action = prev_action.data_ptr(), \
                next_action.data_ptr(), None, None
        else:
            assert prev_action.dtype == torch.int32 and next_action.dtype == torch.int32
            D.prev_action, D.next_action, D.prev_action_f, D.next_action_f = prev_action.data_ptr(), \
                next_action.data_ptr(), None, None
        D.latent = latent.contiguous().data_ptr() if latent is not None else None
        if latent is not None:
            self._keep.append(latent.contiguous())
            D.latent = self._keep[-1].data_ptr()

    def _outputs(self):
        b, n = self.D.b, self.D.n
        T = b * n
        bf = self.buf
        return (bf['raw'][:T].view(b, n, -1), bf['values'][:T].view(b, n, -1), bf['pred'][:T].view(b, n, -1),
                bf['done'][:T].view(b, n))

    def loss(self, K, stats=None):
        c, D = self.cfg, self.D
        b, n = D.b, D.n
        T = b * n
        bf = self.buf
        S1 = c.state_dim + 1
        A = c.num_actions
        own = stats is None
        if own:
            self.stats.zero_()
            stats = self.stats
        d = L.LossDesc(b=b, n=n, A=A, B=c.num_bins, S1=S1, continuous=int(K.continuous), squash=int(K.squash),
                       hl_reduction_mean=int(K.hl_mean), eps_clip=K.eps_clip, value_clip=K.value_clip,
                       entropy_weight=K.entropy_weight, w_actor=K.w_actor, w_critic=K.w_critic,
                       w_autoreg=K.w_autoreg, lo=K.lo, hi=K.hi, sigma=K.sigma)
        fields = dict(raw_actions=bf['raw'], values=bf['values'], pred_raw=bf['pred'], done_logit=bf['done'],
                      actions=None if K.continuous else K.actions, actions_f=K.actions if K.continuous else None,
                      old_logp=K.old_logp, returns=K.returns, old_values=K.old_values, dones=K.dones, lens=K.lens,
                      real=K.real, support=K.support, centers=K.centers, tok=self.tok, stats=stats,
                      d_raw_actions=bf['d_raw'], d_values=bf['d_values'], d_pred_raw=bf['d_pred'],
                      d_done_logit=bf['d_done'])
        for name, t in fields.items():
            if t is not None:
                assert t.is_cuda and t.is_contiguous(), name
                setattr(d, name, t.data_ptr())
        lib = L.lib()
        L.check(lib.xtrl_loss_fwd(C.byref(d), L.stream()), 'loss_fwd')
        L.check(lib.xtrl_loss_bwd(C.byref(d), 1.0, L.stream()), 'loss_bwd')
        del T
        return stats.clone() if own else stats

    def backward(self, grad_events=None):
        self.D.grad_events = C.cast(grad_events, C.POINTER(C.c_void_p)) if grad_events is not None else None
        L.check(L.lib().xtrl_train_backward(C.byref(self.D), L.stream()), 'train_backward')


class FractalTrainStep(FusedTrainStep):

    def __init__(self, model, flat: FlatParams, ws: torch.Tensor, b_max: int, n_max: int):
        c = model.cfg
        self.model, self.flat, self.cfg, self.ws = model, flat, c, ws
        dev = flat.flat.device
        self.dev = dev
        d, H, dh, Lv = c.dim, c.heads, c.dim_head, model.levels
        I, ff, B = H * dh, c.dim * c.ff_mult, c.num_bins
        Ikv = c.kv_inner
        S, A = c.state_dim, c.num_actions
        n_out = A * (2 if c.continuous else 1)
        T = b_max * n_max
        self.b_max, self.n_max, self.T_max = b_max, n_max, T
        f32 = dict(device=dev, dtype=torch.float32)
        E = lambda *shape: torch.empty(*shape, **f32)
        off = lambda name: _off(flat, name)
        enc = 'fractal_encoder.'
        le0 = off(enc + 'level_embedding.level_embeds')
        levels = (L.FractalTrainLevel * Lv)()
        self.levels_py = []
        self.ld_ff = lff = ld_ff(ff)
        for li in range(Lv):
            pre = model.block_prefix(li)
            V = levels[li]
            V.w_qkv = _span_off(flat, [pre + 'self_attn.to_q.weight', pre + 'self_attn.to_k.weight',
                                       pre + 'self_attn.to_v.weight'])
            V.w_out, V.w_gv, V.w_go = off(pre + 'self_attn.to_out.weight'), off(pre + 'global_attn.to_v.weight'), \
                off(pre + 'global_attn.to_out.weight')
            for k in (1, 2, 3):
                setattr(V, f'ln{k}_w', off(pre + f'norm{k}.weight'))
                setattr(V, f'ln{k}_b', off(pre + f'norm{k}.bias'))
            V.w_ff1, V.b_ff1 = off(pre + 'ff.ff.0.0.weight'), off(pre + 'ff.ff.0.0.bias')
            V.w_ff2, V.b_ff2 = off(pre + 'ff.ff.2.weight'), off(pre + 'ff.ff.2.bias')
            V.w_proj, V.b_proj = off(enc + f'level_projections.{li}.weight'), off(enc + f'level_projections.{li}.bias')
            V.level_embed = le0 + li * d
            bufs = dict(xin=E(T, d), qkv=E(T, 3 * I), o=E(T, I), lse=E(b_max * H * n_max), s1=E(T, d), x1=E(T, d),
                        st1=E(T, 2), g=E(T, d), gv=E(T, I), s2=E(T, d), x2=E(T, d), st2=E(T, 2), h=E(T, lff),
                        u=E(T, lff), s3=E(T, d), x3=E(T, d), st3=E(T, 2), mean=E(T, d))
            for k, t in bufs.items():
                setattr(V, k, t.data_ptr())
            self.levels_py.append(bufs)
        self.levels = levels
        ldp = d + 4
        self.buf = dict(ac_in=E(T, c.in_dim), ewa=E(T, 2 * d), zp=E(T, ldp), hp=E(T, ldp), z1=E(T, 4 * d),
                        h1=E(T, 4 * d), lat_e=E(max(b_max, 1), d), raw=E(T, n_out), values=E(T, B),
                        pred=E(T, 2 * (S + 1)), done=E(T), d_raw=E(T, n_out), d_values=E(T, B),
                        d_pred=E(T, 2 * (S + 1)), d_done=E(T), dz1=E(T, 4 * d), dac=E(T, c.in_dim), dzp=E(T, ldp),
                        dewa=E(T, 2 * d), delta=E(b_max * H * n_max))
        part = max(256 * max(ff, 4 * d, B, 3 * I), 1024 * max(A, 1) * d,
                   2 * int(L.lib().xtrl_train_part_floats(T, b_max, d, A)))
        self.buf['part'] = E(part)
# ... 118 lines not shown
```

Baseline: 431,100 env-steps/s.

## Prebuild register-fragment weight images for 64x256 LayerNorm GEMM tiles

Adds a per-forward build pass that converts the weights feeding the LayerNorm-fused 64x256 GEMMs (out proj, ff1/ff2, qkv, head) into pre-split 3-piece bf16 fragments, laid out per wave and k-step. The GEMM kernel gains a WF variant that loads these B fragments straight into registers instead of staging B through LDS, so the producer does less work and less shared memory is needed. The cost is an extra build kernel each forward, an extra arena, and higher register pressure in the consumer waves. It is enabled by default but only used when the weight-image path is not already taken for that GEMM.

```diff
diff --git a/include/xtrl_hip.h b/include/xtrl_hip.h
--- a/include/xtrl_hip.h
+++ b/include/xtrl_hip.h
@@ -11,7 +11,7 @@
 #define XTRL_E_ARG 1
 #define XTRL_E_HIP 2
 
-#define XTRL_ABI_VERSION 27
+#define XTRL_ABI_VERSION 28
 
 int xtrl_abi_version(void);
 int64_t xtrl_struct_size(const char* name);
@@ -291,6 +291,7 @@
 } XtrlTrainLayer;
 
 typedef struct XtrlWimgEntry XtrlWimgEntry;
+typedef struct XtrlWfragEntry XtrlWfragEntry;
 
 typedef struct XtrlTrainDesc {
   int b, n, S, A, d, L, H, dh, ff, B, in_dim, n_out, G;
@@ -381,6 +382,11 @@
   const XtrlWimgEntry* wimg_tab_host;
   int wimg_n;
   const float* alibi_slopes;
+  void* wfrag;
+  int64_t wfrag_bytes;
+  const XtrlWfragEntry* wfrag_tab;
+  const XtrlWfragEntry* wfrag_tab_host;
+  int wfrag_n;
   int num_mem_kv;
   int add_zero_kv;
   float* sink_ws;
@@ -398,6 +404,17 @@
                     void* arena, int64_t arena_bytes, void* stream);
 
 int64_t xtrl_wimg_launch_count(void);
+
+struct XtrlWfragEntry {
+  int64_t w_off;
+  int64_t img_off;
+  int N, K, ld, trans_b, blk0, pad_;
+};
+#define XTRL_WFRAG_UNIT_BYTES (12 * 1024)
+int xtrl_train_wfrag_plan(const XtrlTrainDesc* desc, XtrlWfragEntry* tab, int cap, int64_t* bytes);
+int xtrl_wfrag_build(const float* flat, const XtrlWfragEntry* tab_host, const XtrlWfragEntry* tab_dev, int n,
+                     void* arena, int64_t arena_bytes, void* stream);
+int64_t xtrl_wfrag_launch_count(void);
 
 int xtrl_train_forward(const XtrlTrainDesc* desc, void* stream);
 int xtrl_train_backward(const XtrlTrainDesc* desc, void* stream);
diff --git a/x-transformers-rl_amd/csrc/cabi.cpp b/x-transformers-rl_amd/csrc/cabi.cpp
--- a/x-transformers-rl_amd/csrc/cabi.cpp
+++ b/x-transformers-rl_amd/csrc/cabi.cpp
@@ -44,7 +44,8 @@
                {"XtrlTrainDesc", sizeof(XtrlTrainDesc)},     {"XtrlBatchDesc", sizeof(XtrlBatchDesc)},
                {"XtrlLossDesc", sizeof(XtrlLossDesc)},       {"XtrlFractalLevel", sizeof(XtrlFractalLevel)},
                {"XtrlFractalDesc", sizeof(XtrlFractalDesc)},     {"XtrlFractalTrainLevel", sizeof(XtrlFractalTrainLevel)},
-               {"XtrlFractalTrainDesc", sizeof(XtrlFractalTrainDesc)}, {"XtrlWimgEntry", sizeof(XtrlWimgEntry)}};
+               {"XtrlFractalTrainDesc", sizeof(XtrlFractalTrainDesc)}, {"XtrlWimgEntry", sizeof(XtrlWimgEntry)},
+               {"XtrlWfragEntry", sizeof(XtrlWfragEntry)}};
   for (const auto& s : sizes)
     if (name && strcmp(name, s.name) == 0) return s.size;
   return -1;
diff --git a/x-transformers-rl_amd/csrc/gemm.hip b/x-transformers-rl_amd/csrc/gemm.hip
--- a/x-transformers-rl_amd/csrc/gemm.hip
+++ b/x-transformers-rl_amd/csrc/gemm.hip
@@ -825,20 +825,24 @@
 
 typedef __attribute__((address_space(3))) void lds_void_t;
 
-template <bool TA, bool TB, int EPI, bool RES, int BM = 128, int BN = 128, bool KT = false, bool WI = false>
+template <bool TA, bool TB, int EPI, bool RES, int BM = 128, int BN = 128, bool KT = false, bool WI = false,
+          bool WF = false>
 __global__ __launch_bounds__(512, 1) void k_gemm_ws(const GemmArgs a) {
   constexpr int BK = 32, XRS = BK + 8, NP = 256, TM = 2, TN = 2, WN = BN / 64;
   constexpr bool LNE = (EPI == EPI_RES_LN || EPI == EPI_LN_BWD || EPI == EPI_LN_BWD2);
   static_assert(!WI || !TA, "weight images feed B of the A \"N\" launches");
+  static_assert(!WF || (!TA && !WI && LNE && BM == 64 && BN == 256), "fragment images: the 64 x 256 LayerNorm tiles");
   static_assert(XTRL_WIMG_TILE_BYTES(BN) == 3 * BN * XRS * 2, "image tile = the B part of a piece image");
   constexpr int A_F4 = BM * BK / 4 / NP, B_F4 = BN * BK / 4 / NP;
-  constexpr int IMG = 3 * (BM + BN) * XRS;
+  constexpr int IMG = 3 * (BM + (WF ? 0 : BN)) * XRS;
   static_assert((BM == 128 && BN == 128) || (BM == 64 && BN == 256), "tile 128 x 128 or 64 x 256");
   static_assert(!TA || A_F4 == 4, "A \"T\": one 4 x 4 transposed group per producer thread");
   static_assert(!TB || B_F4 % 4 == 0, "B \"T\": whole 4 x 4 transposed groups per producer thread");
   constexpr int LDT = BN + 4;
-  static_assert(!LNE || (BM * LDT + 8 * BN) * 4 <= 2 * IMG * 2, "LN tile exceeds the piece images");
-  __shared__ __attribute__((aligned(16))) __bf16 smem[2 * IMG];
+  static_assert(WF || !LNE || (BM * LDT + 8 * BN) * 4 <= 2 * IMG * 2, "LN tile exceeds the piece images");
+  constexpr int SMEM = WF ? (BM * LDT + 8 * BN) * 2 : 2 * IMG;
+  static_assert(SMEM >= 2 * IMG, "two piece images");
+  __shared__ __attribute__((aligned(16))) __bf16 smem[SMEM];
 
   const int tid = threadIdx.x, lane = tid & 63, wave = tid >> 6;
   const bool producer = wave >= 4;
@@ -897,7 +901,7 @@
         ra[S][i] = ld_t(Ab, a.lda, k0 + 4 * kq + i, m0 + 4 * q, M);
       }
     }
-    if constexpr (!WI) {
+    if constexpr (!WI && !WF) {
 #pragma unroll
       for (int i = 0; i < B_F4; ++i) {
         if constexpr (!TB) {
@@ -965,7 +969,7 @@
         }
       }
     }
-    if constexpr (WI) {
+    if constexpr (WI || WF) {
     } else if constexpr (!TB) {
 #pragma unroll
       for (int i = 0; i < B_F4; ++i) {
@@ -1026,6 +1030,47 @@
 #pragma unroll
           for (int j = 0; j < TN; ++j)
             acc[i][j] = __builtin_amdgcn_mfma_f32_32x32x16_bf16(av[pb][PA[t]][i], bv[pb][PB[t]][j], acc[i][j], 0, 0, 0);
+      __builtin_amdgcn_sched_barrier(0);
+    }
+  };
+
+  bf16x8 bf[2][BK / 16][3][TN];
+  auto ldb = [&](auto S, int kt) {
+    if constexpr (WF) {
+      const int w = __builtin_amdgcn_readfirstlane(wn);
+      const char* src = static_cast<const char*>(a.wfrag) +
+                        ((int64_t)w * nk + min(kt, nk - 1)) * XTRL_WFRAG_UNIT_BYTES + lane * 16;
+#pragma unroll
+      for (int i = 0; i < 12; ++i)
+        bf[decltype(S)::value][i / 6][(i / 2) % 3][i % 2] = *reinterpret_cast<const bf16x8*>(src + i * 1024);
+    }
+  };
+  auto compute_f = [&](const __bf16* xa, auto S) {
+    const int xi = wm * 32 * TM + (lane & 31), xk = 8 * (lane >> 5);
+    bf16x8 av[2][3][TM];
+    auto rd = [&](int buf, int st) {
+      auto ra_ = [&](int pc) {
+#pragma unroll
+        for (int i = 0; i < TM; ++i)
+          av[buf][pc][i] = *reinterpret_cast<const bf16x8*>(xa + (pc * BM + xi + 32 * i) * XRS + 16 * st + xk);
+      };
+      ra_(2); ra_(0); ra_(1);
+    };
+    rd(0, 0);
+#pragma unroll
+    for (int st = 0; st < BK / 16; ++st) {
+      const int pb = st & 1;
+      if (st + 1 < BK / 16) rd(pb ^ 1, st + 1);
+      __builtin_amdgcn_sched_barrier(0);
+      constexpr int PA[6] = {2, 0, 1, 1, 0, 0}, PB[6] = {0, 2, 1, 0, 1, 0};
+#pragma unroll
+      for (int t = 0; t < 6; ++t)
+#pragma unroll
+        for (int i = 0; i < TM; ++i)
+#pragma unroll
+          for (int j = 0; j < TN; ++j)
+            acc[i][j] = __builtin_amdgcn_mfma_f32_32x32x16_bf16(av[pb][PA[t]][i], bf[decltype(S)::value][st][PB[t]][j],
+                                                                acc[i][j], 0, 0, 0);
       __builtin_amdgcn_sched_barrier(0);
     }
   };
@@ -1104,6 +1149,24 @@
       }
     }
     if constexpr (!LNE) return;
+  } else if constexpr (WF) {
+    ldb(I0{}, 0);
+    __syncthreads();
+    auto cstep = [&](auto S, auto Sn, int t) {
+      ldb(Sn, t + 1);
+      __builtin_amdgcn_sched_barrier(0);
+      compute_f(smem + (t & 1) * IMG, S);
+      __syncthreads();
+    };
+    int t = 0;
+    for (; t + 1 < nk; t += 2) {
+      cstep(I0{}, I1{}, t);
+      cstep(I1{}, I0{}, t + 1);
+    }
+    if (t < nk) {
+      cstep(I0{}, I1{}, t);
+      __syncthreads();
+    }
   } else {
     __syncthreads();
     for (int t = 0; t < nsteps; ++t) {
@@ -1288,6 +1351,7 @@
   return wgs <= 256 && (a.kspan > 0 ? a.kspan : a.K) >= (ta ? 64 : 512);
 }
 
+int64_t g_wfrag_launches = 0;
 int64_t g_wimg_launches = 0;
 
 bool wimg_on() {
@@ -1312,6 +1376,23 @@
     }
   }
   hipLaunchKernelGGL((k_gemm_ws<TA, TB, EPI, RES, BM, BN, KT>), grid, dim3(512), 0, s, r);
+}
+
+template <bool TB, int EPI, bool RES, bool KT_PLAIN>
+void launch_ln256(const GemmArgs& a, hipStream_t s) {
+  const bool wi = a.wimg && a.wimg_bn == 256 && wimg_on();
+  if (a.wfrag && !wi && a.kspan == 0) {
+    dim3 grid(1, (a.M + 63) / 64, 1);
+    GemmArgs r = a;
+    r.xcd_remap = grid.y % 8 == 0 ? 1 : 0;
+    ++g_wfrag_launches;
+    if (a.K % 32 != 0)
+      hipLaunchKernelGGL((k_gemm_ws<false, TB, EPI, RES, 64, 256, true, false, true>), grid, dim3(512), 0, s, r);
+    else
+      hipLaunchKernelGGL((k_gemm_ws<false, TB, EPI, RES, 64, 256, false, false, true>), grid, dim3(512), 0, s, r);
+    return;
+  }
+  launch_ws<false, TB, EPI, RES, 64, 256, KT_PLAIN>(a, s);
 }
 
 int ln_gemm_run(const GemmArgs& a, int trans_a, int trans_b, int epi, bool vec, hipStream_t s) {
@@ -1329,13 +1410,13 @@
       if (kt) launch_ws<false, false, EPI_RES_LN, true, 128, 128, true>(a, s);
       else launch_ws<false, false, EPI_RES_LN, true, 128, 128, false>(a, s);
     } else {
-      if (kt) launch_ws<false, false, EPI_RES_LN, true, 64, 256, true>(a, s);
-      else launch_ws<false, false, EPI_RES_LN, true, 64, 256, false>(a, s);
+      if (kt) launch_ln256<false, EPI_RES_LN, true, true>(a, s);
+      else launch_ln256<false, EPI_RES_LN, true, false>(a, s);
     }
   } else if (epi == EPI_LN_BWD) {
     XTRL_REQUIRE(trans_b && !res && a.ln_x && a.ln_part, "gemm: LayerNorm-backward epilogue arguments");
     if (narrow) launch_ws<false, true, EPI_LN_BWD, false, 128, 128, true>(a, s);
-    else launch_ws<false, true, EPI_LN_BWD, false, 64, 256, true>(a, s);
+    else launch_ln256<true, EPI_LN_BWD, false, true>(a, s);
   } else {
     XTRL_REQUIRE(trans_b && !res && a.ln_x && a.ln_part && (!a.ln_gpre || ((uintptr_t)a.ln_gpre & 15u) == 0) &&
                      a.ln_ldg % 4 == 0 &&
@@ -1344,7 +1425,7 @@
                      a.ldc == a.N,
                  "gemm: post-norm LayerNorm-backward epilogue arguments");
     if (narrow) launch_ws<false, true, EPI_LN_BWD2, false, 128, 128, true>(a, s);
-    else launch_ws<false, true, EPI_LN_BWD2, false, 64, 256, true>(a, s);
+    else launch_ln256<true, EPI_LN_BWD2, false, true>(a, s);
   }
   XTRL_LAUNCHED("gemm_ln");
   return XTRL_OK;
@@ -1845,6 +1926,82 @@
   return XTRL_OK;
 }
 
+namespace {
+__global__ __launch_bounds__(256) void k_wfrag_build(const float* __restrict__ flat, const XtrlWfragEntry* __restrict__ tab,
+                                                     int n, char* __restrict__ arena) {
+  int e = 0;
+  while (e + 1 < n && tab[e + 1].blk0 <= (int)blockIdx.x) ++e;
+  const XtrlWfragEntry E = tab[e];
+  const int nkt = (E.K + 31) / 32, blk = (int)blockIdx.x - E.blk0, w = blk / nkt, s = blk % nkt;
+  const int t = threadIdx.x, l = t & 63, j = (t >> 6) & 1, st = t >> 7;
+  const int col = 64 * w + 32 * j + (l & 31), k0 = 32 * s + 16 * st + 8 * (l >> 5);
+  const float* W = flat + E.w_off;
+  float v[8];
+#pragma unroll
+  for (int c = 0; c < 8; ++c) {
+    const bool ok = col < E.N && k0 + c < E.K;
+    const int64_t at = E.trans_b ? (int64_t)(k0 + c) * E.ld + col : (int64_t)col * E.ld + k0 + c;
+    const float x = W[ok ? at : 0];
+    v[c] = ok ? x : 0.f;
+  }
+  bf16x4 h[2], m[2], lo[2];
+  split3(make_float4(v[0], v[1], v[2], v[3]), h[0], m[0], lo[0]);
+  split3(make_float4(v[4], v[5], v[6], v[7]), h[1], m[1], lo[1]);
+  char* out = arena + E.img_off + (int64_t)blk * XTRL_WFRAG_UNIT_BYTES + l * 16;
+  auto store = [&](int pc, const bf16x4 (&x)[2]) {
+    bf16x4* q = reinterpret_cast<bf16x4*>(out + ((st * 3 + pc) * 2 + j) * 1024);
+    q[0] = x[0];
+    q[1] = x[1];
+  };
+  store(0, h);
+  store(1, m);
+  store(2, lo);
+}
+}
+
+bool wfrag_applies(int N, int epi) {
+  return (epi == EPI_RES_LN || epi == EPI_LN_BWD || epi == EPI_LN_BWD2) && N > 128 && N <= 256;
+}
+
+void wfrag_find(GemmArgs& g, int trans_b, int epi, const float* flat, const XtrlWfragEntry* tab, int n,
+                const void* arena) {
+  if (!tab || !arena || n <= 0 || !wfrag_applies(g.N, epi)) return;
+  for (int i = 0; i < n; ++i) {
+    const XtrlWfragEntry& E = tab[i];
+    if (flat + E.w_off == g.B && E.trans_b == trans_b && E.N == g.N && E.K == g.K && E.ld == g.ldb) {
+      g.wfrag = static_cast<const char*>(arena) + E.img_off;
+      return;
+    }
+  }
+}
+
+int wfrag_build(const float* flat, const XtrlWfragEntry* tab_host, const XtrlWfragEntry* tab_dev, int n, void* arena,
+                int64_t arena_bytes, hipStream_t s) {
+  XTRL_REQUIRE(flat && tab_host && tab_dev && arena && n > 0, "wfrag: null table / arena");
+  XTRL_REQUIRE(((uintptr_t)arena & 15u) == 0, "wfrag: the arena must be 16-byte aligned");
+  int blocks = 0;
+  for (int i = 0; i < n; ++i) {
+    const XtrlWfragEntry& E = tab_host[i];
+    XTRL_REQUIRE(E.N > 0 && E.N <= 256 && E.K > 0 && E.w_off >= 0 && E.img_off >= 0 && E.img_off % 16 == 0 &&
+                     E.blk0 == blocks && (E.trans_b == 0 || E.trans_b == 1) && E.ld >= (E.trans_b ? E.N : E.K),
+                 "wfrag: bad table entry %d", i);
+    const int64_t units = 4 * (int64_t)((E.K + 31) / 32);
+    XTRL_REQUIRE(E.img_off + units * XTRL_WFRAG_UNIT_BYTES <= arena_bytes,
+                 "wfrag: entry %d ends past the arena (%lld bytes)", i, (long long)arena_bytes);
+    blocks += (int)units;
+  }
+  hipLaunchKernelGGL(k_wfrag_build, dim3(blocks), dim3(256), 0, s, flat, tab_dev, n, static_cast<char*>(arena));
+  XTRL_LAUNCHED("wfrag_build");
+  return XTRL_OK;
+}
+
+}
+
+extern "C" int64_t xtrl_wfrag_launch_count(void) { return xtrl::g_wfrag_launches; }
+
+extern "C" int xtrl_wfrag_build(const float* flat, const XtrlWfragEntry* tab_host, const XtrlWfragEntry* tab_dev, int n,
+                                void* arena, int64_t arena_bytes, void* stream) {
+  return xtrl::wfrag_build(flat, tab_host, tab_dev, n, arena, arena_bytes, xtrl::as_stream(stream));
 }
 
 extern "C" int64_t xtrl_wimg_launch_count(void) { return xtrl::g_wimg_launches; }
diff --git a/x-transformers-rl_amd/csrc/kernels.h b/x-transformers-rl_amd/csrc/kernels.h
--- a/x-transformers-rl_amd/csrc/kernels.h
+++ b/x-transformers-rl_amd/csrc/kernels.h
@@ -70,7 +70,13 @@
   float* ln2_part_b = nullptr;
   const void* wimg = nullptr;
   int wimg_bn = 0;
-};
+  const void* wfrag = nullptr;
+};
+void wfrag_find(GemmArgs& g, int trans_b, int epi, const float* flat, const XtrlWfragEntry* tab, int n,
+                const void* arena);
+bool wfrag_applies(int N, int epi);
+int wfrag_build(const float* flat, const XtrlWfragEntry* tab_host, const XtrlWfragEntry* tab_dev, int n, void* arena,
+                int64_t arena_bytes, hipStream_t s);
 void wimg_find(GemmArgs& g, int trans_b, int epi, const float* flat, const XtrlWimgEntry* tab, int n,
                const void* arena);
 int wimg_tile_bn(int N, int epi);
diff --git a/x-transformers-rl_amd/csrc/train.hip b/x-transformers-rl_amd/csrc/train.hip
--- a/x-transformers-rl_amd/csrc/train.hip
+++ b/x-transformers-rl_amd/csrc/train.hip
@@ -816,6 +816,7 @@
   float* G(int64_t off) const { return off >= 0 ? D->grad + off : nullptr; }
   void img(GemmArgs& g, int trans_b, int epi) const {
     wimg_find(g, trans_b, epi, D->flat, D->wimg_tab_host, D->wimg_n, D->wimg);
+    wfrag_find(g, trans_b, epi, D->flat, D->wfrag_tab_host, D->wfrag_n, D->wfrag);
   }
 };
 
@@ -1340,6 +1341,8 @@
   int rc;
   if (D->wimg && D->wimg_tab && D->wimg_tab_host && D->wimg_n > 0 && wimg_enabled())
     if ((rc = wimg_build(D->flat, D->wimg_tab_host, D->wimg_tab, D->wimg_n, D->wimg, D->wimg_bytes, s))) return rc;
+  if (D->wfrag && D->wfrag_tab && D->wfrag_tab_host && D->wfrag_n > 0)
+    if ((rc = wfrag_build(D->flat, D->wfrag_tab_host, D->wfrag_tab, D->wfrag_n, D->wfrag, D->wfrag_bytes, s))) return rc;
   if (D->evolutionary) {
     hipLaunchKernelGGL(k_latent_embed, dim3(blocks(D->b * d, 256)), dim3(256), 0, s, D->latent, c.P(D->w_lat),
                        c.P(D->b_lat), D->lat_e, D->b, D->G, d);
@@ -1973,6 +1976,34 @@
   return n;
 }
 
+extern "C" int xtrl_train_wfrag_plan(const XtrlTrainDesc* D, XtrlWfragEntry* tab, int cap, int64_t* bytes) {
+  int n = 0, blk = 0;
+  int64_t at = 0;
+  auto add = [&](int64_t w_off, int trans_b, int N, int K, int ld) {
+    if (w_off < 0 || N <= 0 || K <= 0) return;
+    XtrlWfragEntry E{};
+    E.w_off = w_off; E.img_off = at; E.N = N; E.K = K; E.ld = ld; E.trans_b = trans_b; E.blk0 = blk;
+    const int units = 4 * ((K + 31) / 32);
+    if (tab && n < cap) tab[n] = E;
+    ++n;
+    blk += units;
+    at += (int64_t)units * XTRL_WFRAG_UNIT_BYTES;
+  };
+  if (D && D->layers && D->L > 0 && xtrl::ln_fusable(D) && xtrl::wfrag_applies(D->d, xtrl::EPI_RES_LN)) {
+    const int d = D->d, I = D->H * D->dh, f1 = D->ff_glu ? 2 * D->ff : D->ff;
+    for (int li = 0; li < D->L; ++li) {
+      const XtrlTrainLayer& Ly = D->layers[li];
+      add(Ly.w_out, 0, d, I, I);
+      add(Ly.w_ff2, 0, d, D->ff, D->ff);
+      add(Ly.w_ff1, 1, d, f1, d);
+      add(Ly.w_proj, 1, d, Ly.n_qkv, d);
+    }
+    add(D->w_h1, 1, d, 4 * d, D->in_dim);
+  }
+  if (bytes) *bytes = at;
+  return n;
+}
+
 extern "C" int64_t xtrl_train_pack_floats(int T, int S, int A, int n_out, int B) {
   if (T <= 0) return 0;
   return xtrl::pack_bufs(nullptr, T, S, A, n_out, B).floats;
diff --git a/x-transformers-rl_amd/xtrl_amd/_lib.py b/x-transformers-rl_amd/xtrl_amd/_lib.py
--- a/x-transformers-rl_amd/xtrl_amd/_lib.py
+++ b/x-transformers-rl_amd/xtrl_amd/_lib.py
@@ -7,7 +7,7 @@
 import torch
 
 LIB_PATH = Path(os.environ.get('XTRL_LIB', Path(__file__).resolve().parent / 'libxtrl_hip.so'))
-ABI_VERSION = 27
+ABI_VERSION = 28
 
 P = C.c_void_p
 I32, I64, U32, U64, F32 = C.c_int, C.c_int64, C.c_uint32, C.c_uint64, C.c_float
@@ -91,6 +91,14 @@
 
 def wimg_tile_bytes(bn: int) -> int:
     return 3 * bn * WIMG_XRS * 2
+
+
+class WfragEntry(C.Structure):
+    _fields_ = [('w_off', I64), ('img_off', I64), ('N', I32), ('K', I32), ('ld', I32), ('trans_b', I32), ('blk0', I32),
+                ('pad_', I32)]
+
+
+WFRAG_UNIT_BYTES = 12 * 1024
 
 
 class TrainDesc(C.Structure):
@@ -116,6 +124,8 @@
                    ('packed', I32), ('ep_off', P), ('pack_ws', P), ('pack_ws_floats', I64), ('attn_window', I32),
                    ('Hkv', I32), ('wimg', P), ('wimg_bytes', I64), ('wimg_tab', P),
                    ('wimg_tab_host', C.POINTER(WimgEntry)), ('wimg_n', I32), ('alibi_slopes', P),
+                   ('wfrag', P), ('wfrag_bytes', I64), ('wfrag_tab', P), ('wfrag_tab_host', C.POINTER(WfragEntry)),
+                   ('wfrag_n', I32),
                    ('num_mem_kv', I32), ('add_zero_kv', I32), ('sink_ws', P), ('sink_ws_floats', I64)])
 
 
@@ -213,6 +223,9 @@
     'xtrl_train_part_floats': (C.c_int64, [I32, I32, I32, I32]),
     'xtrl_train_wimg_plan': (I32, [C.POINTER(TrainDesc), C.POINTER(WimgEntry), I32, C.POINTER(I64)]),
     'xtrl_wimg_launch_count': (I64, []),
+    'xtrl_train_wfrag_plan': (I32, [C.POINTER(TrainDesc), C.POINTER(WfragEntry), I32, C.POINTER(I64)]),
+    'xtrl_wfrag_launch_count': (I64, []),
+    'xtrl_wfrag_build': (I32, [P, C.POINTER(WfragEntry), P, I32, P, I64, P]),
     'xtrl_wimg_build': (I32, [P, C.POINTER(WimgEntry), P, I32, P, I64, P]),
     'xtrl_minibatch_gather': (I32, [C.POINTER(BatchDesc), P]),
     'xtrl_rsnorm_update': (I32, [P, P, P, I32, I32, P]),
@@ -233,7 +246,7 @@
            'XtrlTrainLayer': TrainLayer, 'XtrlTrainDesc': TrainDesc, 'XtrlBatchDesc': BatchDesc,
            'XtrlLossDesc': LossDesc, 'XtrlFractalLevel': FractalLevel, 'XtrlFractalDesc': FractalDesc,
            'XtrlFractalTrainLevel': FractalTrainLevel, 'XtrlFractalTrainDesc': FractalTrainDesc,
-           'XtrlWimgEntry': WimgEntry}
+           'XtrlWimgEntry': WimgEntry, 'XtrlWfragEntry': WfragEntry}
 
 _lib = None
 
diff --git a/x-transformers-rl_amd/xtrl_amd/train.py b/x-transformers-rl_amd/xtrl_amd/train.py
--- a/x-transformers-rl_amd/xtrl_amd/train.py
+++ b/x-transformers-rl_amd/xtrl_amd/train.py
@@ -56,6 +56,18 @@
     tab_dev = torch.frombuffer(bytearray(bytes(tab)), dtype=torch.uint8).to(dev)
     D.wimg, D.wimg_bytes = arena.data_ptr(), nbytes.value
     D.wimg_tab, D.wimg_tab_host, D.wimg_n = tab_dev.data_ptr(), C.cast(tab, C.POINTER(L.WimgEntry)), n
+    return dict(tab=tab, tab_dev=tab_dev, arena=arena)
+
+
+def _alloc_wfrag(D, dev):
+    nbytes = C.c_int64(0)
+    n = int(L.lib().xtrl_train_wfrag_plan(C.byref(D), None, 0, C.byref(nbytes)))
+    if n <= 0 or nbytes.value <= 0:
+        return None
+    tab = (L.WfragEntry * n)()
+    L.lib().xtrl_train_wfrag_plan(C.byref(D), tab, n, C.byref(nbytes))
+    arena = torch.empty(nbytes.value, device=dev, dtype=torch.uint8)
+    tab_dev = torch.frombuffer(bytearray(bytes(tab)), dtype=torch.uint8).to(dev)
     return dict(tab=tab, tab_dev=tab_dev, arena=arena)
 
 
@@ -190,6 +202,21 @@
         self.wimg = None
         if WIMG_DEFAULT:
             self.use_weight_images(True)
+        self.wfrag = None
+        self.use_weight_fragments(True)
+
+    def use_weight_fragments(self, on: bool):
+        D = self.D
+        if not on or isinstance(self, FractalTrainStep):
+            D.wfrag, D.wfrag_bytes, D.wfrag_tab, D.wfrag_tab_host, D.wfrag_n = None, 0, None, None, 0
+            return
+        if self.wfrag is None:
+            self.wfrag = _alloc_wfrag(D, self.dev)
+        w = self.wfrag
+        if w is not None:
+            D.wfrag, D.wfrag_bytes = w['arena'].data_ptr(), w['arena'].numel()
+            D.wfrag_tab, D.wfrag_tab_host, D.wfrag_n = w['tab_dev'].data_ptr(), \
+                C.cast(w['tab'], C.POINTER(L.WfragEntry)), len(w['tab'])
 
     def use_weight_images(self, on: bool):
         D = self.D
```

Measured after the change: 441,100 env-steps/s (median of 6 runs). +2.3%, better.
